# sourcedennis/wasm-pathtracer

Hardware: AMD Instinct MI355X
Metric: Mray/s (primary+shadow+bounce) at 1920x1080, 1/2/4/8 GPU; L2 vs CPU ref (higher is better)
Workload: dtype f32; 1 GPU; C3 bunny scene (scene id 2), 1920x1080, 64 spp per GPU share (64 spp frame), depth 8, NormalNEE; rays=25682600955, parallelism=single GPU

## Files before the change

include/wpt.h:

```cpp
#ifndef WPT_H
#define WPT_H

#include <stddef.h>
#include <stdint.h>

#ifdef __cplusplus
extern "C" {
#endif

#define WPT_OK 0
#define WPT_ERR_NOT_INIT (-1)
#define WPT_ERR_ALREADY_INIT (-2)
#define WPT_ERR_INVALID_SCENE (-3)
#define WPT_ERR_INVALID_ARG (-4)
#define WPT_ERR_UNSUPPORTED (-5)
#define WPT_ERR_DEVICE (-6)
#define WPT_ERR_NO_MESH (-7)

#define WPT_NO_NEE 0
#define WPT_NORMAL_NEE 1
#define WPT_PNEE 2


int wpt_init(uint32_t width, uint32_t height, uint32_t scene_id, float cam_x, float cam_y, float cam_z,
// ... 45 lines not shown

int wpt_copy_partition(void* device_dst);

typedef int (*wpt_exchange_fn)(void* user);
int wpt_set_exchange(wpt_exchange_fn fn, void* user, void* local_dev, void* gathered_dev, uint64_t slot);
int64_t wpt_exchange_slot(void);

int wpt_comm_unique_id(void* out128);
int wpt_set_comm(uint32_t rank, uint32_t nranks, uint32_t tile, const void* unique_id128);
int wpt_gather_frame(uint32_t root);
int wpt_comm_destroy(void);
#define WPT_XFER_GATHER 0
#define WPT_XFER_ALLGATHER 1
typedef int (*wpt_transport_fn)(void* user, int32_t op, uint32_t root);
int wpt_set_transport(wpt_transport_fn fn, void* user, void* send_dev, void* recv_dev, uint64_t slot);
int64_t wpt_gather_plan(uint32_t rank, uint32_t nranks, uint32_t root, uint64_t slot, uint64_t* out);
float wpt_seq_sum(const float* v, uint64_t n);
float wpt_seq_sum_chunks(const float* v, uint64_t n);
int wpt_seq_sum_device(const float* v, uint64_t n, float* out);

int wpt_stats(uint64_t* out, size_t n);
int wpt_kernel_times(double* out, size_t n);
int wpt_set_counting(int on);
int wpt_set_profiling(int on);
int wpt_set_lanes(int32_t n);
#define WPT_OPT_DEFAULTS 0
#define WPT_OPT_TRAVERSAL 1
#define WPT_OPT_TRAVERSAL_SH 2
#define WPT_OPT_FUSED 3
#define WPT_OPT_FUSED_BELOW 4
#define WPT_OPT_SMALL_LANES 5
#define WPT_OPT_PIXEL_TILE 6
#define WPT_OPT_GRID_PCT 7
#define WPT_OPT_REFILL 8
#define WPT_OPT_REFILL_SH 9
#define WPT_OPT_TREELET 10
#define WPT_OPT_BVH_BUILD 11
#define WPT_OPT_LANES 12
#define WPT_OPT_FINISH_BELOW 13
#define WPT_OPT_TRACE_GRID_PCT 14
#define WPT_OPT_FINISH_EVERY 20
#define WPT_OPT_PROBE 22
#define WPT_OPT_STOCK 23
#define WPT_OPT_STOCK_LANES 24
#define WPT_OPT_FILL 25
#define WPT_OPT_ASYNC_PRIO 26
#define WPT_OPT_ASYNC_GRID_PCT 27
#define WPT_OPT_STOCK_AHEAD 30
#define WPT_OPT_STOCK_EVERY 32
#define WPT_OPT_STOCK_EXTRA 33
#define WPT_OPT_ASYNC_ONESHOT 31
#define WPT_OPT_STOCK_PREFILL 35
#define WPT_OPT_ASYNC_FUSED_BELOW 36
#define WPT_OPT_LOG 34
#define WPT_OPT_SCENE_TRAVERSAL 28
#define WPT_OPT_SCENE_TRI_ONLY 29
int wpt_set_option(int32_t option, int64_t value);
int64_t wpt_probe_read(uint32_t* meta, uint32_t* rec, uint64_t* rec_entries, double* ticks_per_us);
int wpt_get_option(int32_t option, int64_t* value);
int wpt_scene_build_info(double* out);
int wpt_clear_stats(void);
int wpt_sync(void);
int wpt_bvh_depth(void);

int wpt_trace_rays(size_t n, const float* rays, float* t_out, int32_t* id_out);
int wpt_shadow_rays(size_t n, const float* pq, const int32_t* light, uint8_t* occluded);

int wpt_shutdown(void);

void* wpt_debug_scene_new(int32_t scene_id, const float* mesh_vertices, size_t num_vertices);
int wpt_debug_scene_info(void* h, uint64_t* out);
int wpt_debug_scene_nodes4(void* h, uint32_t* out);
int wpt_debug_scene_nodes(void* h, uint32_t* out);
int wpt_debug_scene_shapes(void* h, float* out);
int wpt_debug_scene_lights(void* h, uint32_t* out);
void wpt_debug_scene_free(void* h);
void* wpt_debug_scene_new_gpu(int32_t scene_id, const float* mesh_vertices, size_t num_vertices);
int wpt_debug_scene_build_info(void* h, double* out);

#ifdef __cplusplus
}
#endif

#endif
```

wasm-pathtracer_amd/_lib.py:

```python
import ctypes
import os

HERE = os.path.dirname(os.path.abspath(__file__))
_VARIANT = os.environ.get("WPT_LIB_VARIANT", "")
LIB_PATH = os.path.join(HERE, f"libwpt_{_VARIANT}.so" if _VARIANT else "libwpt.so")

_lib = None

c_u32, c_i32, c_f32, c_sz = ctypes.c_uint32, ctypes.c_int32, ctypes.c_float, ctypes.c_size_t
c_p = ctypes.c_void_p

_SIGS = {
    "wpt_init": (ctypes.c_int, [c_u32, c_u32, c_u32, c_f32, c_f32, c_f32, c_f32, c_f32]),
    "wpt_results": (ctypes.POINTER(ctypes.c_uint8), [c_u32]),
    "wpt_update_scene": (ctypes.c_int, [c_u32]),
    "wpt_update_settings": (ctypes.c_int, [c_u32, c_u32, c_u32, c_u32, c_u32]),
    "wpt_update_viewport": (ctypes.c_int, [c_u32, c_u32]),
    "wpt_update_camera": (ctypes.c_int, [c_f32, c_f32, c_f32, c_f32, c_f32]),
    "wpt_allocate_mesh": (ctypes.c_int, [c_u32, c_u32]),
    "wpt_mesh_vertices": (ctypes.POINTER(ctypes.c_float), [c_u32]),
    "wpt_notify_mesh_loaded": (ctypes.c_int, [c_u32]),
    "wpt_load_obj": (ctypes.c_int, [c_u32, ctypes.c_char_p, c_sz, c_p, c_p]),
    "wpt_parse_obj": (ctypes.c_int, [ctypes.c_char_p, c_sz, c_p, c_p, ctypes.c_uint64, c_p]),
    "wpt_allocate_texture": (ctypes.POINTER(ctypes.c_uint8), [c_u32, c_u32, c_u32]),
    "wpt_notify_texture_loaded": (ctypes.c_int, [c_u32]),
    "wpt_compute": (ctypes.c_int, [c_sz]),
    "wpt_last_error": (ctypes.c_char_p, []),
    "wpt_set_device": (ctypes.c_int, [ctypes.c_int]),
    "wpt_set_render_options": (ctypes.c_int, [c_i32, c_u32, ctypes.c_uint64]),
    "wpt_set_partition": (ctypes.c_int, [c_u32, c_u32, c_u32]),
    "wpt_partition_pixels": (ctypes.c_int64, [c_p]),
    "wpt_tile_partition": (ctypes.c_int64, [c_u32, c_u32, c_u32, c_u32, c_u32, c_p]),
    "wpt_photon_tree": (ctypes.c_int64, [c_p, c_p, c_p]),
    "wpt_read_radiance": (ctypes.c_int, [c_p, c_p]),
    "wpt_copy_partition": (ctypes.c_int, [c_p]),
    "wpt_set_exchange": (ctypes.c_int, [c_p, c_p, c_p, c_p, ctypes.c_uint64]),
    "wpt_exchange_slot": (ctypes.c_int64, []),
    "wpt_stats": (ctypes.c_int, [c_p, c_sz]),
    "wpt_kernel_times": (ctypes.c_int, [c_p, c_sz]),
    "wpt_set_counting": (ctypes.c_int, [ctypes.c_int]),
    "wpt_set_profiling": (ctypes.c_int, [ctypes.c_int]),
    "wpt_set_lanes": (ctypes.c_int, [ctypes.c_int32]),
    "wpt_set_option": (ctypes.c_int, [ctypes.c_int32, ctypes.c_int64]),
    "wpt_get_option": (ctypes.c_int, [ctypes.c_int32, c_p]),
    "wpt_probe_read": (ctypes.c_int64, [c_p, c_p, c_p, c_p]),
    "wpt_scene_build_info": (ctypes.c_int, [c_p]),
    "wpt_clear_stats": (ctypes.c_int, []),
    "wpt_sync": (ctypes.c_int, []),
    "wpt_bvh_depth": (ctypes.c_int, []),
    "wpt_trace_rays": (ctypes.c_int, [c_sz, c_p, c_p, c_p]),
    "wpt_shadow_rays": (ctypes.c_int, [c_sz, c_p, c_p, c_p]),
    "wpt_shutdown": (ctypes.c_int, []),
    "wpt_debug_scene_new": (c_p, [c_i32, c_p, c_sz]),
    "wpt_debug_scene_info": (ctypes.c_int, [c_p, c_p]),
    "wpt_debug_scene_nodes": (ctypes.c_int, [c_p, c_p]),
    "wpt_debug_scene_shapes": (ctypes.c_int, [c_p, c_p]),
    "wpt_debug_scene_nodes4": (ctypes.c_int, [c_p, c_p]),
    "wpt_comm_unique_id": (ctypes.c_int, [c_p]),
    "wpt_set_comm": (ctypes.c_int, [c_u32, c_u32, c_u32, c_p]),
    "wpt_gather_frame": (ctypes.c_int, [c_u32]),
    "wpt_comm_destroy": (ctypes.c_int, []),
    "wpt_set_transport": (ctypes.c_int, [c_p, c_p, c_p, c_p, ctypes.c_uint64]),
    "wpt_gather_plan": (ctypes.c_int64, [c_u32, c_u32, c_u32, ctypes.c_uint64, c_p]),
    "wpt_seq_sum": (ctypes.c_float, [c_p, ctypes.c_uint64]),
    "wpt_seq_sum_chunks": (ctypes.c_float, [c_p, ctypes.c_uint64]),
    "wpt_seq_sum_device": (ctypes.c_int, [c_p, ctypes.c_uint64, c_p]),
    "wpt_debug_scene_lights": (ctypes.c_int, [c_p, c_p]),
    "wpt_debug_scene_free": (None, [c_p]),
    "wpt_debug_scene_new_gpu": (c_p, [c_i32, c_p, c_sz]),
    "wpt_debug_scene_build_info": (ctypes.c_int, [c_p, c_p]),
}

EXPORTED = tuple(_SIGS)


def header_symbols():
    import re
    hdr = os.path.join(os.path.dirname(HERE), "include", "wpt.h")
    txt = open(hdr).read()
    return sorted(set(re.findall(r"\b(wpt_[a-z_0-9]+)\s*\(", txt)))


def lib():
    global _lib
    if _lib is not None:
        return _lib
    try:
        import torch
    except ImportError:
        pass
    if not os.path.exists(LIB_PATH):
        raise RuntimeError(f"{LIB_PATH} is missing: run __graft_entry__.build() (make -C wasm-pathtracer_amd/csrc)")
    L = ctypes.CDLL(LIB_PATH)
    for name, (res, args) in _SIGS.items():
        f = getattr(L, name)
        f.restype = res
        f.argtypes = args
    _lib = L
    return L
```

wasm-pathtracer_amd/csrc/wpt_api.cpp:

```cpp
#include <cstring>
#include <map>
#include <memory>
#include <string>
#include <vector>

#include "../../include/wpt.h"
#include "wpt_bvh_gpu.h"
#include "wpt_comm.h"
#include "wpt_obj.h"
#include "wpt_partition.h"
#include "wpt_render.h"
#include "wpt_seqsum.h"

using namespace wpt;

namespace {

struct Session {
  std::map<uint32_t, std::vector<float>> preload;
  std::map<uint32_t, std::vector<float>> meshes;
  std::map<uint32_t, std::vector<uint8_t>> textures;
  uint32_t scene_id = 0;
  HostScene scene;
  Renderer renderer;
// ... 441 lines not shown
  if (slot < s.renderer.exchange_slot() || slot < s.renderer.part_pixels())
    return fail(WPT_ERR_INVALID_ARG, "transport slot smaller than the largest partition");
  s.drop_comm();
  s.xfer = fn;
  s.xfer_user = user;
  s.xfer_send = (float4*)send_dev;
  s.xfer_recv = (float4*)recv_dev;
  s.xfer_slot = slot;
  s.renderer.set_exchange(xfer_exchange, &s, send_dev, recv_dev, slot);
  return WPT_OK;
}

int64_t wpt_gather_plan(uint32_t rank, uint32_t nranks, uint32_t root, uint64_t slot, uint64_t* out) {
  if (nranks == 0 || rank >= nranks || root >= nranks) return fail(WPT_ERR_INVALID_ARG, "bad rank");
  std::vector<XferOp> ops;
  gather_plan(rank, nranks, root, slot, ops);
  if (out)
    for (size_t i = 0; i < ops.size(); i++) {
      out[4 * i] = ops[i].peer;
      out[4 * i + 1] = ops[i].offset;
      out[4 * i + 2] = ops[i].count;
      out[4 * i + 3] = ops[i].recv ? 1u : 0u;
    }
  return (int64_t)ops.size();
}

float wpt_seq_sum(const float* v, uint64_t n) { return wpt::seq_sum_f32(v, (size_t)n); }

float wpt_seq_sum_chunks(const float* v, uint64_t n) {
  std::vector<wpt::ChunkEff> eff(2 * ((size_t)n / wpt::kSumChunk + 1));
  wpt::seq_sum_effects(v, (size_t)n, eff.data());
  return wpt::seq_sum_walk(v, (size_t)n, eff.data());
}

int wpt_seq_sum_device(const float* v, uint64_t n, float* out) {
  if (!g_session) return fail(WPT_ERR_NOT_INIT, "init not called");
  if (!out || (n && !v)) return fail(WPT_ERR_INVALID_ARG, "null pointer");
  std::string err;
  if (!g_session->renderer.seq_sum_device(v, n, *out, err)) return fail(WPT_ERR_DEVICE, err);
  return WPT_OK;
}

int wpt_comm_destroy(void) {
  if (!g_session) return fail(WPT_ERR_NOT_INIT, "init not called");
  g_session->drop_comm();
  return WPT_OK;
}

int wpt_stats(uint64_t* out, size_t n) {
  if (!g_session) return fail(WPT_ERR_NOT_INIT, "init not called");
  std::string err;
  if (!g_session->renderer.flush_counts(err)) return fail(WPT_ERR_DEVICE, err);
  const Stats& st = g_session->renderer.stats();
  uint64_t v[40] = {st.paths,          st.rays,           st.shadow_rays,    st.node_visits,  st.prim_tests,
                    st.bounces,        st.ext_visits,     st.ext_tests,      st.ext_node_bytes, st.sh_visits,
                    st.sh_tests,       st.sh_node_bytes,  st.fallback_ext,   st.fallback_sh,  st.ext_lane_iters,
                    st.ext_live_iters, st.sh_lane_iters,  st.sh_live_iters,  st.photon_rays,  st.photons,
                    st.sum_chunks,     st.sum_resummed,   st.sum_fetched,    st.stock_consumed, st.fill_paths,
                    st.trace_bytes,    st.finish_paths,   st.finish_max_bounces, st.max_ray_visits,
                    st.ex_body_lanes,  st.ex_bodies,      st.lf_body_lanes,  st.lf_bodies,    st.stock_traced,
                    st.stock_deficit,  st.stock_waits,    st.plan_us,        st.stock_us,
                    st.stock_rays,     st.stock_rays_used};
  for (size_t i = 0; i < n && i < 40; i++) out[i] = v[i];
  return WPT_OK;
}

int wpt_kernel_times(double* out, size_t n) {
  if (!g_session) return fail(WPT_ERR_NOT_INIT, "init not called");
  const KernelTimes& t = g_session->renderer.times();
  double v[28] = {t.generate, (double)t.n_generate, t.extend, (double)t.n_extend, t.shade, (double)t.n_shade,
                  t.shadow, (double)t.n_shadow, t.accumulate, (double)t.n_accumulate, t.trace, (double)t.n_trace};
  for (int k = 0; k < 6; k++) {
    v[12 + 2 * k] = t.busy[k];
    v[13 + 2 * k] = (double)t.logical[k];
  }
  v[24] = t.retrace;
  v[25] = (double)t.n_retrace;
  v[26] = t.busy[6];
  v[27] = (double)t.logical[6];
  for (size_t i = 0; i < n && i < 28; i++) out[i] = v[i];
  return WPT_OK;
}

int wpt_set_counting(int on) {
  if (!g_session) return fail(WPT_ERR_NOT_INIT, "init not called");
  g_session->renderer.set_counting(on != 0);
  return WPT_OK;
}

int wpt_scene_build_info(double* out) {
  if (!g_session) return fail(WPT_ERR_NOT_INIT, "init not called");
  if (!out) return fail(WPT_ERR_INVALID_ARG, "null argument");
  out[0] = g_session->scene.bvh_ms;
  out[1] = g_session->scene.bvh_on_gpu ? 1.0 : 0.0;
  return WPT_OK;
}

int wpt_set_lanes(int32_t n) {
  if (!g_session) return fail(WPT_ERR_NOT_INIT, "init not called");
  if (!g_session->renderer.set_lanes(n)) return fail(WPT_ERR_INVALID_ARG, "lanes out of range");
  return WPT_OK;
}

int wpt_set_option(int32_t option, int64_t value) {
  if (option == WPT_OPT_BVH_BUILD) {
    if (value < 0 || value > 2) return fail(WPT_ERR_INVALID_ARG, "option value out of range");
    g_bvh_build = (int)value;
    return WPT_OK;
  }
  std::string err;
  if (!g_session) {
    if (option == WPT_OPT_DEFAULTS) {
      g_default_opts.clear();
      g_bvh_build = 0;
      return WPT_OK;
    }
// ... 46 lines not shown
  std::memcpy(meta, s.probe_meta.data(), s.probe_meta.size() * sizeof(uint32_t));
  std::memcpy(rec, s.probe_rec.data(), s.probe_rec.size() * sizeof(uint4));
  *rec_entries = s.probe_rec.size();
  if (ticks_per_us) *ticks_per_us = s.probe_tpu;
  const int64_t n = (int64_t)(s.probe_meta.size() / 5);
  s.probe_meta.clear();
  s.probe_rec.clear();
  s.probe_taken = false;
  return n;
}

int wpt_get_option(int32_t option, int64_t* value) {
  if (!value) return fail(WPT_ERR_INVALID_ARG, "null argument");
  if (option == WPT_OPT_BVH_BUILD) { *value = g_bvh_build; return WPT_OK; }
  if (!g_session) {
    auto it = g_default_opts.find(option);
    if (it != g_default_opts.end()) { *value = it->second; return WPT_OK; }
    Renderer probe;
    if (!probe.get_option(option, *value)) return fail(WPT_ERR_INVALID_ARG, "unknown option");
    return WPT_OK;
  }
  if (!g_session->renderer.get_option(option, *value)) return fail(WPT_ERR_INVALID_ARG, "unknown option");
  return WPT_OK;
}

int wpt_set_profiling(int on) {
  if (!g_session) return fail(WPT_ERR_NOT_INIT, "init not called");
  g_session->renderer.set_profiling(on != 0);
  return WPT_OK;
}

int wpt_clear_stats(void) {
  if (!g_session) return fail(WPT_ERR_NOT_INIT, "init not called");
  g_session->renderer.clear_stats();
  return WPT_OK;
}

int wpt_sync(void) {
  if (!g_session) return fail(WPT_ERR_NOT_INIT, "init not called");
  std::string err;
  if (!g_session->renderer.sync(err)) return fail(WPT_ERR_DEVICE, err);
  return WPT_OK;
}

int wpt_bvh_depth(void) {
  if (!g_session) return fail(WPT_ERR_NOT_INIT, "init not called");
  return (int)g_session->renderer.bvh_depth();
}

int wpt_trace_rays(size_t n, const float* rays, float* t_out, int32_t* id_out) {
  if (!g_session) return fail(WPT_ERR_NOT_INIT, "init not called");
  std::string err;
  if (!g_session->renderer.trace_rays(n, rays, t_out, id_out, err)) return fail(WPT_ERR_DEVICE, err);
  return WPT_OK;
}

int wpt_shadow_rays(size_t n, const float* pq, const int32_t* light, uint8_t* occluded) {
  if (!g_session) return fail(WPT_ERR_NOT_INIT, "init not called");
  std::string err;
  if (!g_session->renderer.shadow_rays(n, pq, light, occluded, err)) return fail(WPT_ERR_INVALID_ARG, err);
  return WPT_OK;
}

int wpt_shutdown(void) {
  if (!g_session) return fail(WPT_ERR_NOT_INIT, "init not called");
  delete g_session;
  g_session = nullptr;
  return WPT_OK;
}

void* wpt_debug_scene_new(int32_t scene_id, const float* mesh_vertices, size_t num_vertices) {
  std::vector<float> mesh;
  if (mesh_vertices && num_vertices) mesh.assign(mesh_vertices, mesh_vertices + ((num_vertices / 3) * 9));
  HostScene* sc = new HostScene();
  std::string err;
  if (!build_scene(scene_id, mesh, *sc, err)) {
    delete sc;
    fail(WPT_ERR_INVALID_SCENE, err);
    return nullptr;
  }
  return sc;
}

void* wpt_debug_scene_new_gpu(int32_t scene_id, const float* mesh_vertices, size_t num_vertices) {
  static BvhGpu* gpu = nullptr;
  const hipError_t he = hipSetDevice(g_device);
  if (he != hipSuccess) {
    fail(WPT_ERR_DEVICE, std::string("hipSetDevice failed: ") + hipGetErrorString(he));
    return nullptr;
  }
  if (!gpu) gpu = new BvhGpu();
  gpu->min_shapes = 0;
  std::vector<float> mesh;
  if (mesh_vertices && num_vertices) mesh.assign(mesh_vertices, mesh_vertices + ((num_vertices / 3) * 9));
  HostScene* sc = new HostScene();
  std::string err;
  if (!build_scene(scene_id, mesh, *sc, err, gpu)) {
    delete sc;
    fail(err.rfind("HIP error", 0) == 0 || err.rfind("GPU BVH", 0) == 0 ? WPT_ERR_DEVICE : WPT_ERR_INVALID_SCENE,
         err);
    return nullptr;
  }
  return sc;
}

int wpt_debug_scene_build_info(void* h, double* out) {
// ... 30 lines not shown
  const HostScene* sc = (const HostScene*)h;
  if (!sc) return fail(WPT_ERR_INVALID_ARG, "null scene");
  for (size_t i = 0; i < sc->nodes4.size(); i++) {
    const Node4& n = sc->nodes4[i];
    uint32_t* o = out + 37 * i;
    memset(o, 0, 37 * sizeof(uint32_t));
    for (int k = 0; k < 4; k++) {
      const uint32_t c = n.child[k];
      if (c == kChildEmpty) continue;
      o[0]++;
      uint32_t* e = o + 1 + 9 * k;
      if (!(c & 0x80000000u)) {
        e[0] = 1;
        e[1] = c;
      } else {
        e[0] = 2;
        if ((c & 0xC0000000u) == 0xC0000000u) {
          e[1] = sc->leaf_table[2 * (c & 0x3FFFFFFFu)];
          e[2] = sc->leaf_table[2 * (c & 0x3FFFFFFFu) + 1];
        } else {
          e[1] = c & 0xFFFFFFu;
          e[2] = (c >> 24) & 0x3Fu;
        }
      }
      const float b[6] = {n.xmin[k], n.ymin[k], n.zmin[k], n.xmax[k], n.ymax[k], n.zmax[k]};
      memcpy(e + 3, b, sizeof b);
    }
  }
  return WPT_OK;
}

int wpt_debug_scene_shapes(void* h, float* out) {
  const HostScene* sc = (const HostScene*)h;
  if (!sc) return fail(WPT_ERR_INVALID_ARG, "null scene");
  for (size_t i = 0; i < sc->shapes.size(); i++) {
    const Shape& s = sc->shapes[i];
    float* o = out + 16 * i;
    memcpy(o, s.g, sizeof s.g);
    o[12] = (float)s.kind;
    o[13] = s.emissive ? 1.0f : 0.0f;
    o[14] = 0.0f;
    o[15] = 0.0f;
  }
  return WPT_OK;
}

int wpt_debug_scene_lights(void* h, uint32_t* out) {
  const HostScene* sc = (const HostScene*)h;
  if (!sc) return fail(WPT_ERR_INVALID_ARG, "null scene");
  for (size_t i = 0; i < sc->lights.size(); i++) out[i] = sc->lights[i];
  return WPT_OK;
}

void wpt_debug_scene_free(void* h) { delete (HostScene*)h; }

}
```

wasm-pathtracer_amd/csrc/wpt_render.h:

```cpp
#pragma once
#include <hip/hip_runtime.h>
#include <stdint.h>
#include <string>
#include <algorithm>
#include <deque>
#include <vector>

#include "wpt_scene.h"
#include "wpt_seqsum.h"

namespace wpt {

constexpr int kMaxInf = 16;
constexpr int kMaxBvhDepth = 4096;
constexpr int kMaxBounces = 512;

struct DevScene {
  const float4* nodes;
  const float4* tree;
  uint32_t tree_pairs, tree_root_lf;
  const float4* prims;
  const uint32_t* kinds;
  const float4* all;
  const uint32_t* all_kinds;
  const float4* mats;
  const float4* lights;
  const float4* nodes4;
  const uint32_t* leaf_table;
  uint32_t num_inf, num_finite, num_shapes, num_lights;
  uint32_t use_bvh, tri_only;
  uint32_t refill_lanes;
  uint32_t refill_lanes_sh;
  int stack_cap;
  uint32_t* overflow;
  const uint32_t* oct_child;
  const float* oct_cum;
  const uint32_t* oct_corners;
  uint32_t oct_nodes;
  uint32_t oct_lds_words;
  float bg[3];
  float4 planes[kMaxInf];
  uint4* probe;
};

struct Stats {
  uint64_t paths = 0;
  uint64_t rays = 0;
  uint64_t shadow_rays = 0;
  uint64_t node_visits = 0;
  uint64_t prim_tests = 0;
  uint64_t bounces = 0;
  uint64_t ext_visits = 0, ext_tests = 0, ext_node_bytes = 0;
  uint64_t sh_visits = 0, sh_tests = 0, sh_node_bytes = 0;
  uint64_t fallback_ext = 0, fallback_sh = 0;
  uint64_t ex_body_lanes = 0, ex_bodies = 0, lf_body_lanes = 0, lf_bodies = 0;
  uint64_t ext_lane_iters = 0, ext_live_iters = 0, sh_lane_iters = 0, sh_live_iters = 0;
  uint64_t photon_rays = 0, photons = 0;
  uint64_t trace_bytes = 0;
  uint64_t max_ray_visits = 0;
  uint64_t sum_chunks = 0, sum_resummed = 0, sum_fetched = 0;
  uint64_t finish_paths = 0, finish_max_bounces = 0;
  uint64_t stock_traced = 0, stock_consumed = 0, fill_paths = 0;
  uint64_t stock_deficit = 0, stock_waits = 0, plan_us = 0, stock_us = 0;
  uint64_t stock_rays = 0;
  uint64_t stock_rays_used = 0;
};

constexpr int kTimedKernels = 7;
struct KernelTimes {
  double generate = 0, extend = 0, shade = 0, shadow = 0, accumulate = 0, trace = 0, retrace = 0;
  uint64_t n_extend = 0, n_shadow = 0, n_shade = 0, n_generate = 0, n_accumulate = 0, n_trace = 0, n_retrace = 0;
  double busy[kTimedKernels] = {0, 0, 0, 0, 0, 0, 0};
  uint64_t logical[kTimedKernels] = {0, 0, 0, 0, 0, 0, 0};
};

constexpr int kMaxLanes = 8;
constexpr uint64_t kMinLanePaths = 1024;
constexpr size_t kFinishWord = 2 + 2 * (size_t)kMaxBounces;
constexpr size_t kCountWords = kFinishWord + 4;
constexpr uint32_t kWorkWords = 16;
constexpr uint32_t kWorkCopies = 64;
struct PathSet {
  hipStream_t stream = nullptr;
  hipStream_t lo = nullptr;
  hipEvent_t done = nullptr;
  uint64_t cap = 0;
  uint32_t* pixel = nullptr;
  float4* col = nullptr;
  float4* ro[2] = {nullptr, nullptr};
  float4* rd[2] = {nullptr, nullptr};
  float4* thr[2] = {nullptr, nullptr};
  float* t = nullptr;
  int32_t* id = nullptr;
  float4 *so = nullptr, *sd = nullptr, *sc = nullptr;
  uint32_t* counts = nullptr;
  uint32_t* h_counts = nullptr;
  uint2* spill = nullptr;
  size_t spill_cap = 0;
};

constexpr int kAsyncLane0 = 2;
struct Batch {
  enum State { kNew, kBouncing, kCountWait, kIssued };
  uint64_t k0 = 0, n = 0;
  int half = -1;
  const uint32_t* part = nullptr;
  uint32_t npix = 0;
  const uint32_t* moff = nullptr;
  const uint32_t* mbase = nullptr;
  const uint32_t* mlist = nullptr;
  uint32_t nent = 0;
  bool stock = false;
  bool async = false;
  int queue = 0;
  int lane0 = 0, nl = 1;
  uint64_t off[kMaxLanes + 1] = {};
  bool fused = false, pnee = false;
  int maxb = 0, b = 0;
  bool finished = false;
  State state = kNew;
  hipEvent_t done[kMaxLanes] = {};
  hipEvent_t live[kMaxLanes] = {};
  uint32_t* hc = nullptr;
  uint32_t* hl = nullptr;
};

class Renderer {
 public:
  Renderer();
  ~Renderer();
  bool set_device(int dev, std::string& err);
  bool upload_scene(const HostScene& sc, std::string& err);
  bool set_viewport(uint32_t w, uint32_t h, std::string& err);
  void set_camera(const float cam[5]);
  void set_types(int left, int right, int debug) { left_type_ = left; right_type_ = right; debug_ = debug; }
  void set_adaptive(bool left, bool right) { adaptive_[0] = left; adaptive_[1] = right; }
  bool adaptive() const { return adaptive_[0] || adaptive_[1]; }
  bool fill_sampling_blue(std::string& err);
  bool sampling_rgba(uint8_t* out, std::string& err);
  void set_options(int max_depth, uint32_t seed, uint64_t batch) {
    if (seed != seed_) photons_ok_ = false;
    max_depth_ = max_depth; seed_ = seed; if (batch) batch_ = batch;
  }
  bool build_photons(std::string& err);
  bool photon_tree(std::vector<uint32_t>& child, std::vector<float>& cum, uint64_t& shot, uint64_t& stored,
                   std::string& err);
  bool set_partition(uint32_t rank, uint32_t nranks, uint32_t tile, std::string& err);
  bool reset(std::string& err);
  bool compute(uint64_t num_paths, std::string& err);
  bool sync(std::string& err);
  bool results_rgba(uint8_t* host_out, std::string& err);
  bool read_radiance(float* acc3, uint32_t* cnt, std::string& err);
  bool copy_partition(float* dev_dst, std::string& err);
  using ExchangeFn = int (*)(void*);
  void set_exchange(ExchangeFn fn, void* user, void* local_dev, void* gathered_dev, uint64_t slot) {
    xfn_ = fn; xuser_ = user; xlocal_ = (float4*)local_dev; xall_ = (float4*)gathered_dev; xslot_ = slot;
  }
  uint64_t exchange_slot() const { return maxpart_; }
  uint32_t rank() const { return rank_; }
  uint32_t nranks() const { return nranks_; }
  uint32_t tile() const { return tile_; }
  bool unpack_ranks(const float4* gathered, uint64_t slot, std::string& err);
  bool trace_rays(size_t n, const float* rays, float* t_out, int32_t* id_out, std::string& err);
  bool shadow_rays(size_t n, const float* pq, const int32_t* light, uint8_t* occ, std::string& err);
  bool probe_read(std::vector<uint32_t>& meta, std::vector<uint4>& rec, double& ticks_per_us, std::string& err);
  void set_counting(bool on) { counting_ = on; }
  void set_profiling(bool on) { profiling_ = on; }
  bool set_lanes(int n) {
    if (n < 1 || n > lanes_made_) return false;
    nlanes_ = n;
    return true;
  }
  int lanes() const { return nlanes_; }
  static bool scene_option(int opt) { return opt == 1 || opt == 2 || opt == 10; }
  bool set_option(int opt, int64_t v, std::string& err);
  bool get_option(int opt, int64_t& v) const;
  int wants_bvh4() const {
    return (traversal_ == 1 || traversal_sh_ == 1) ? 1 : (traversal_ == 3 || traversal_sh_ == 3) ? 2 : 0;
  }
  bool seq_sum_device(const float* v, uint64_t n, float& out, std::string& err);
  const Stats& stats() const { return stats_; }
  const KernelTimes& times() const { return times_; }
  void clear_stats() {
    std::string e;
    (void)flush_counts(e);
    stats_ = Stats();
    times_ = KernelTimes();
  }
  bool flush_counts(std::string& err);
  uint32_t width() const { return w_; }
  uint32_t height() const { return h_; }
  uint32_t part_pixels() const { return (uint32_t)part_pix_.size(); }
  const std::vector<uint32_t>& part_list() const { return part_pix_; }
  hipStream_t stream() const { return stream_; }
  uint32_t bvh_depth() const { return depth_; }

 private:
  bool ensure_paths(uint64_t n, std::string& err);
  bool ensure_lane(int i, uint64_t n, std::string& err);
  void free_lane_paths(PathSet& L);
  void bind_lane(int i);
  bool run_batch(uint64_t k0, uint64_t n, int half, std::string& err, const uint32_t* part_pix = nullptr,
                 uint32_t part_n = 0, const Batch* map = nullptr);
  bool batch_begin(Batch& B, std::string& err);
  bool batch_advance(Batch& B, bool block, std::string& err);
  bool batch_tail(Batch& B, std::string& err);
  void batch_counts(const Batch& B, const uint32_t* hc);
  bool pump(bool block, std::string& err);
  bool wait_issued(Batch* B, std::string& err);
  bool drain_async(std::string& err);
  bool host_wait(hipEvent_t e, std::string& err);
  bool host_wait_stream(hipStream_t s, std::string& err);
  hipEvent_t ev_sync_ = nullptr;
  uint64_t batch_cap() const;
  int main_lanes() const;
  bool compute_half(int h, uint64_t n, std::string& err);
// ... 38 lines not shown
  ChunkEff* h_eff_ = nullptr;
  uint32_t* d_need_ = nullptr;
  uint32_t* d_list_ = nullptr;
  float* d_fb_ = nullptr;
  uint32_t* h_list_ = nullptr;
  float* h_fb_ = nullptr;
  uint32_t stock_slots_ = 1024;
  int stock_lanes_ = 2;
  uint32_t stock_ahead_ = 40;
  uint32_t stock_extra_ = 8;
  uint32_t stock_every_ = 3;
  float4* d_stock_ = nullptr;
  uint32_t* d_stock_id_ = nullptr;
  size_t stock_bytes_[2] = {0, 0};
  uint32_t* d_front_ = nullptr;
  uint32_t* d_def_ = nullptr;
  uint32_t* d_bmax_ = nullptr;
  unsigned long long* d_rays_ = nullptr;
  uint64_t stock_cap_ = 0;
  uint32_t stock_used_slots_ = 0;
  static constexpr int kMaxRefill = 8;
  static constexpr uint64_t kStockBytes = 48ull << 30;
  static constexpr int kRefillChunks = 8;
  static constexpr uint64_t kRefillChunk = 1ull << 25;
  struct Refill {
    uint32_t id = 0;
    bool live = false;
    bool counted = false;
    uint32_t* off = nullptr;
    uint32_t* base = nullptr;
    std::deque<Batch> chunks;
  };
  Refill refills_[kMaxRefill];
  hipEvent_t refill_ev_[kMaxRefill][2 * kRefillChunks] = {};
  uint32_t* h_refill_cnt_ = nullptr;
  uint32_t refill_id_ = 0;
  int refill_lane_ = 0;
  uint32_t round_need_[2] = {0, 0};
  bool stock_redo_[2] = {false, false};
  int log_ = 0;
  bool stock_active(int h) const { return stock_slots_ != 0 && nranks_ == 1 && adaptive_[h]; }
  bool stock_alloc(std::string& err);
  void stock_drop();
  bool stock_round(int h, uint64_t left, std::string& err);
  bool stock_consume(int h, uint64_t a, uint64_t b, std::string& err);
  bool stock_flush(std::string& err);
  bool refill_count(Refill& f, bool block, std::string& err);
  uint32_t refill_scale(int h, uint32_t ahead, uint64_t after) const;
  Refill* refill_slot(std::string& err);
  void refill_plan(Refill& F, int h, uint32_t ahead, uint32_t q);
  bool refill_issue(Refill& F, int h, uint64_t wt, std::string& err);
  bool stock_prefill(int h, uint64_t budget, std::string& err);
  bool stock_prefill_ = true;
  bool pend_stock_ = false;
  std::deque<Batch*> aq_[2];
  bool fill_on_ = false;
  int async_prio_ = 0;
  int async_grid_pct_ = 100;
  uint64_t async_fused_below_ = 1ull << 26;
  bool async_launch_ = false;
  uint32_t* d_seam_pix_[2] = {nullptr, nullptr};
  uint32_t* d_rest_pix_[2] = {nullptr, nullptr};
  uint32_t seam_npix_[2] = {0, 0}, rest_npix_[2] = {0, 0};
  static constexpr int kMaxFill = 8;
  Batch fill_[kMaxFill];
  int nfill_ = 0;
  hipEvent_t fill_ev_[kMaxFill][2] = {};
  uint32_t* h_fill_cnt_ = nullptr;
  bool async_pending() const { return !aq_[0].empty() || !aq_[1].empty(); }
  int fill_lane() const { return kAsyncLane0 + stock_lanes_; }
  bool issue_fill(int h, uint64_t k0, uint64_t n, std::string& err);
  bool drain_fill(std::string& err);
  bool compute_halves(uint64_t nl, uint64_t nr, std::string& err);
  uint32_t async_grid(uint32_t g, int base_pct, uint32_t rays_per_path = 1) const {
    if (!async_launch_) return g;
    if (async_oneshot_) return std::max<uint32_t>(1u, (uint32_t)((async_paths_ * rays_per_path + 255) / 256));
    return async_grid_pct_ > 0 ? std::max<uint32_t>(1u, (uint32_t)((uint64_t)g * async_grid_pct_ / base_pct)) : g;
  }
  bool async_oneshot_ = false;
  uint64_t async_paths_ = 0;
  void bind_batch_lane(const Batch& B, int l);
  bool time_launches_ = false;
  uint8_t* d_samp_ = nullptr;
  ExchangeFn xfn_ = nullptr;
  void* xuser_ = nullptr;
  float4* xlocal_ = nullptr;
  float4* xall_ = nullptr;
  uint64_t xslot_ = 0;
  uint64_t maxpart_ = 0;
  uint32_t* d_xidx_ = nullptr;
  bool photons_ok_ = false;
  uint64_t photons_shot_ = 0, photons_stored_ = 0;
  std::vector<uint32_t> oct_child_;
  std::vector<float> oct_cum_;
  uint32_t* d_oct_child_ = nullptr;
  float* d_oct_cum_ = nullptr;
  uint32_t* d_oct_corners_ = nullptr;

  int device_ = -1;
  int ncu_ = 256;
  uint2* d_spill_ = nullptr;
  size_t spill_cap_ = 0;
  static constexpr int kTravVariants = 8;
  uint32_t grid_ext_[2 * kTravVariants] = {};
  uint32_t grid_sh_[2 * kTravVariants] = {};
  uint32_t grid_tr_[4] = {};
  uint32_t grid_shade_ = 512;
  uint32_t shade_occ_[16] = {};
  size_t shade_occ_smem_[16] = {};
  bool fused_ = false;
  uint64_t fused_below_ = 1ull << 24;
  int small_lanes_ = 2;
  int traversal_ = 3, traversal_sh_ = 3;
  int trav_ext_ = 0, trav_sh_ = 0;
  bool treelet_ = true;
  uint32_t pixel_tile_ = 8;
  int grid_pct_ = 50;
#ifndef WPT_TRACE_GRID_PCT
#define WPT_TRACE_GRID_PCT 75
#endif
  int trace_grid_pct_ = WPT_TRACE_GRID_PCT;
  uint32_t refill_ = 12, refill_sh_ = 16;
  uint64_t finish_below_ = 1u << 18;
  int finish_every_ = 4;
  int batch_lanes_ = 1;
  uint32_t probe_cap_ = 0, probe_waves_ = 0, probe_used_ = 0;
  uint4* d_probe_ = nullptr;
  std::vector<uint32_t> probe_meta_;
  int cur_bounce_ = 0;
  uint4* probe_slot(int kernel, uint32_t grid);
  uint32_t* d_fallback_ = nullptr;
  hipStream_t stream_ = nullptr;
  hipStream_t ks_ = nullptr;
  PathSet lanes_[kMaxLanes];
  int lanes_made_ = 0;
  bool stats_pending_ = false;
  int pend_nl_ = 0, pend_b_ = 0;
  int nlanes_ = 4;
  int bound_ = 0;
  hipEvent_t ev_main_ = nullptr;
  hipEvent_t ev_ref_ = nullptr;
  std::vector<void*> scene_bufs_;
  DevScene ds_{};
  uint32_t depth_ = 0;
  bool scene_ok_ = false;

  uint32_t w_ = 0, h_ = 0;
  float cam_[5] = {0, 0, 0, 0, 0};
  int left_type_ = 1, right_type_ = 1, debug_ = 0;
  int max_depth_ = 0;
  uint32_t seed_ = 0xBABABEBEu;
  uint64_t batch_ = 1ull << 27;

  uint32_t rank_ = 0, nranks_ = 1, tile_ = 16;
  std::vector<uint32_t> part_pix_;
  uint32_t* d_part_pix_ = nullptr;
  uint32_t* d_half_pix_[2] = {nullptr, nullptr};
  uint32_t* d_frame_pix_ = nullptr;
  uint32_t half_npix_[2] = {0, 0};
  uint64_t next_path_ = 0;

  float4* d_acc_ = nullptr;
  uint32_t* d_cnt_ = nullptr;
  uint8_t* d_rgba_ = nullptr;

  uint64_t cap_ = 0;
  uint32_t* p_pixel_ = nullptr;
  float4* p_col_ = nullptr;
  float4* p_ro_[2] = {nullptr, nullptr};
  float4* p_rd_[2] = {nullptr, nullptr};
  float4* p_thr_[2] = {nullptr, nullptr};
  float* p_t_ = nullptr;
  int32_t* p_id_ = nullptr;
  float4* s_o_ = nullptr;
  float4* s_d_ = nullptr;
  float4* s_c_ = nullptr;
  uint32_t* d_counts_ = nullptr;
  unsigned long long* d_work_ = nullptr;
  uint32_t* h_counts_ = nullptr;
  uint32_t* h_word_ = nullptr;
  uint32_t* ext_count(int b) const { return b == 0 ? d_counts_ : d_counts_ + 2 + 2 * (b - 1); }
  uint32_t* sh_count(int b) const { return d_counts_ + 3 + 2 * b; }
  unsigned long long* append_ctr(int b) const { return reinterpret_cast<unsigned long long*>(d_counts_ + 2 + 2 * b); }

  bool counting_ = false;
  bool profiling_ = false;
  Stats stats_;
  KernelTimes times_;
  struct PendingTiming {
    hipEvent_t a, b;
    int slot;
  };
  bool next_event(hipEvent_t* e, std::string& err);
  bool resolve_timings(std::string& err);
  std::vector<hipEvent_t> ev_pool_;
  size_t ev_used_ = 0;
  std::vector<PendingTiming> pending_;
};

}
```

wasm-pathtracer_amd/csrc/wpt_render.hip:

```cpp
#include "wpt_render.h"
#include "wpt_partition.h"
#include "wpt_photon.h"
#include "wpt_quartic.h"
#include "wpt_seqsum.h"

#include <algorithm>
#include <chrono>
#include <cstdlib>
#include <cmath>
#include <cstdio>
#include <cstring>
#include <deque>
#include <mutex>
#include <unordered_map>
#include <thread>
#include <type_traits>

#define HIP_OK(expr)                                                     \
  do {                                                                   \
    hipError_t e_ = (expr);                                              \
    if (e_ != hipSuccess) {                                              \
      err = std::string(#expr " failed: ") + hipGetErrorString(e_);      \
      return false;                                                      \
    }                                                                    \
// ... 616 lines not shown
__device__ __forceinline__ bool begin_shadow(const DevScene& S, const Hot& H, Lane& L, V3 o, V3 d, float dir_len,
                                             int32_t light, float& early, bool& occluded, uint32_t& visits,
                                             uint32_t& tests, uint32_t& nbytes) {
  L.o = o;
  L.d = d;
  L.inv = inv_dir(d);
  L.best_id = -1;
  occluded = false;
  if (!S.use_bvh) {
    L.best = 0.0f;
    linear_closest<TRI_ONLY>(S, o, d, L.best, L.best_id, tests);
    return false;
  }
  early = dir_len;
  float tl;
  bool lhit;
  uint32_t k = 0;
  if (H.lrec)
    while (k < S.num_lights && H.lid[k] != light) k++;
  if (H.lrec && k < S.num_lights) {
    lhit = tri_hit_r(H.lq(k, 0), H.lq(k, 1), H.lq(k, 2), H.lq(k, 3), o, d, tl);
  } else {
    const uint32_t lk = (uint32_t)light - S.num_inf;
    const float4* lp = S.prims + 4 * (size_t)lk;
    lhit = TRI_ONLY ? tri_hit(lp, o, d, tl) : prim_hit(S.kinds[lk], lp, o, d, tl);
  }
  if (lhit) early = fminf(tl, dir_len);
  float pt = __int_as_float(0x7f800000);
  int32_t pid = -1;
  if (planes_closest(S, o, d, pt, pid) && pt < early) {
    occluded = true;
    return false;
  }
  if (pid >= 0 && pt < dir_len) { L.best = pt; L.best_id = pid; }
  else { L.best = dir_len; L.best_id = -1; }
  if (!S.num_finite) return false;
  return FAST ? enter_root4<COUNT>(H, L, visits, nbytes) : enter_root<COUNT>(S, H, L, visits, nbytes);
}

__device__ __forceinline__ bool shadow_verdict(const Lane& L, float dir_len, int32_t light, bool occluded) {
  return occluded || (L.best_id >= 0 && L.best < dir_len && L.best_id != light);
}

struct GenParams {
  uint32_t W, H, npix;
  float w_inv, h_inv, ar;
  float cam[3];
  float cx, sx, cy, sy;
  uint32_t seed;
  uint32_t half;
  uint32_t left_type, right_type;
};

__global__ void __launch_bounds__(kBlock) k_generate(GenParams P, const uint32_t* __restrict__ part_pix, uint64_t k0,
                                                     uint32_t n, uint32_t* __restrict__ pix_out,
                                                     float4* __restrict__ thr,
                                                     float4* __restrict__ col, float4* __restrict__ ro,
                                                     float4* __restrict__ rd, uint32_t* __restrict__ count0,
                                                     const uint32_t* __restrict__ rnd_off,
                                                     const uint32_t* __restrict__ rnd_base,
                                                     const uint32_t* __restrict__ rnd_list, uint32_t stock_slots) {
  const uint32_t i = blockIdx.x * kBlock + threadIdx.x;
  if (i == 0) *count0 = n;
  if (i >= n) return;
  const uint64_t k = k0 + i;
  uint32_t pl, sample;
  if (rnd_off) {
    uint32_t lo = 0, hi = P.npix;
    while (lo + 1u < hi) {
      const uint32_t mid = (lo + hi) >> 1;
      if ((uint64_t)rnd_off[mid] <= k) lo = mid;
      else hi = mid;
    }
    pl = lo;
    sample = rnd_base[lo] + (uint32_t)(k - rnd_off[lo]);
  } else {
    pl = (uint32_t)(k % P.npix);
    sample = (uint32_t)(k / P.npix);
  }
  const uint32_t pixel = rnd_list ? rnd_list[pl] : part_pix ? part_pix[pl] : pl;
  const uint32_t x = pixel % P.W, y = pixel / P.W;
  uint32_t s = path_seed(P.seed, pixel, sample);
  const float fx = (((float)x + xs_next(s)) * P.w_inv - 0.5f) * P.ar;
  const float fy = 0.5f - ((float)y + xs_next(s)) * P.h_inv;
  V3 v = normalize(mk(fx, fy, 0.8f));
  v = mk(v.x, P.cx * v.y - P.sx * v.z, P.sx * v.y + P.cx * v.z);
  v = mk(P.cy * v.x + P.sy * v.z, v.y, (-P.sy) * v.x + P.cy * v.z);
  const uint32_t type = x < P.half ? P.left_type : P.right_type;
  pix_out[i] = stock_slots ? pixel * stock_slots + (sample & (stock_slots - 1u)) : rnd_off ? pl : pixel;
  thr[i] = make_float4(1.0f, 1.0f, 1.0f, __uint_as_float(type << kTypeShift));
  col[i] = make_float4(0.0f, 0.0f, 0.0f, 0.0f);
  ro[i] = make_float4(P.cam[0], P.cam[1], P.cam[2], __uint_as_float(s));
  rd[i] = make_float4(v.x, v.y, v.z, __uint_as_float(i));
}

template <bool TRI_ONLY>
__device__ __forceinline__ const float4* shape_rec(const DevScene& S, int32_t id, uint32_t& kind) {
  if (!S.use_bvh) { kind = S.all_kinds[id]; return S.all + 4 * (size_t)id; }
  if ((uint32_t)id < S.num_inf) { kind = kPlane; return nullptr; }
  kind = TRI_ONLY ? (uint32_t)kTri : S.kinds[id - S.num_inf];
  return S.prims + 4 * (size_t)(id - S.num_inf);
}

template <class CP, class FP>
struct OctViewT {
  CP child;
  FP cum;
};
using OctG = OctViewT<const uint32_t*, const float*>;
using OctL1 = OctViewT<const lds_u32*, const float*>;
using OctL2 = OctViewT<const lds_u32*, const lds_f32*>;

template <class OV>
__device__ uint32_t oct_find(const DevScene& S, const OV& O, V3 v, int max_depth, float b[6], int& depth) {
  b[0] = b[1] = b[2] = -kPhotonTreeSize;
  b[3] = b[4] = b[5] = kPhotonTreeSize;
  uint32_t node = 0;
  depth = 0;
  while (O.child[node] != 0u && (max_depth < 0 || depth < max_depth)) {
    float nb[6];
    const uint32_t ci = octant(b, v, nb);
    for (int k = 0; k < 6; k++) b[k] = nb[k];
    node = O.child[node] + ci;
    depth++;
  }
  return node;
}

template <class OV>
__device__ __forceinline__ float oct_bin_prob(const DevScene& S, const OV& O, uint32_t node, uint32_t i) {
  const auto c = O.cum + (size_t)node * S.num_lights;
  return i + 1u == S.num_lights ? 1.0f - c[i] : c[i + 1] - c[i];
}

template <class OV>
__device__ __forceinline__ float oct_node_prob(const DevScene& S, const OV& O, V3 v, int depth, uint32_t res) {
  float b[6];
  int d;
  return oct_bin_prob(S, O, oct_find(S, O, v, depth, b, d), res);
}

__device__ __forceinline__ void oct_axis(float v, float lo, float hi, float& w, float& wadj, float& off) {
  const float size = hi - lo;
  if (v > 0.5f * (lo + hi)) {
    const float left = (hi - (v - size * 0.5f)) / size;
    w = left;
// ... 226 lines not shown
    } else {
      const float4* L = S.lights + 5 * (size_t)li;
      L0 = L[0];
      L1 = L[1];
      L2 = L[2];
      L3 = L[3];
      L4 = L[4];
    }
    const float q1 = xs_next(s);
    const float q2 = xs_next(s);
    const float q1s = sqrtf(q1);
    const V3 pt = add(add(scale(ld3(L0), 1.0f - q1s), scale(ld3(L1), q1s * (1.0f - q2))), scale(ld3(L2), q2 * q1s));
    V3 ln = ld3(L3);
    if (xs_next(s) > 0.5f) ln = neg(ln);
    const V3 inten = ld3(L4);
    V3 tl = sub(pt, hp);
    const float d2 = dot(tl, tl);
    const float dl = sqrtf(d2);
    tl = divs(tl, dl);
    const float ci = dot(tl, nrm);
    const float co = dot(neg(tl), ln);
    if (ci > 0.0f && co > 0.0f) {
      if (P.debug) {
        const float4 c4 = col[path];
        const V3 c = add(ld3(c4), mulv(thr, inten));
        col[path] = make_float4(c.x, c.y, c.z, c4.w);
      } else {
        const float solid = (L0.w * co) / d2;
        const V3 contrib = scale(scale(scale(mulv(thr, inten), solid), ci), 1.0f / light_chance);
        const V3 sorig = add(hp, scale(tl, kEpsilon));
        R.so = make_float4(sorig.x, sorig.y, sorig.z, dl);
        R.sd = make_float4(tl.x, tl.y, tl.z, L1.w);
        R.sc = make_float4(contrib.x, contrib.y, contrib.z, d4.w);
        R.shadow = true;
      }
    }
  }
  const bool capped = P.max_depth > 0 && (int)depth >= P.max_depth;
  if (!capped && depth < (uint32_t)kMaxBounces) {
    const float keep = fmaxf(fminf(fmaxf(fmaxf(thr.x, thr.y), thr.z), 0.9f), 0.1f);
    if (xs_next(s) < keep) {
      thr = scale(thr, 1.0f / keep);
      const uint32_t nsh = (flags >> kShadowShift) + (R.shadow ? 1u : 0u);
      flags = (flags & ~((~0u) << kDepthShift)) | (depth << kDepthShift) | (nsh << kShadowShift) | kFlagBounced;
      R.ro = make_float4(no.x, no.y, no.z, __uint_as_float(s));
      R.rd = make_float4(wi.x, wi.y, wi.z, d4.w);
      R.th = make_float4(thr.x, thr.y, thr.z, __uint_as_float(flags));
      R.alive = true;
    }
  }
  if (!R.alive) end_counts((flags >> kShadowShift) + (R.shadow ? 1u : 0u));
}

template <bool TRI_ONLY, bool PNEE, int OCT, bool CR = false>
__global__ void WPT_SHADE_BOUNDS k_shade(DevScene S, ShadeParams P, RayStream in, RayStream out,
                                                       ShadowStream sh, float4* __restrict__ col,
                                                       const uint32_t* __restrict__ count, const float* __restrict__ t_in,
                                                       const int32_t* __restrict__ id_in,
                                                       unsigned long long* __restrict__ append) {
  constexpr uint32_t kWaves = kShadeBlock / 64;
  __shared__ uint32_t s_off[2][kWaves];
  __shared__ f4v s_light[5 * kShadeLights];
  const uint32_t n = *count;
  const bool lds_lights = S.num_lights <= kShadeLights;
  if (lds_lights) {
    for (uint32_t k = threadIdx.x; k < 5 * S.num_lights; k += kShadeBlock) {
      const float4 v = S.lights[k];
      s_light[k] = f4v{v.x, v.y, v.z, v.w};
    }
  }
  extern __shared__ uint32_t s_oct[];
  if (PNEE && OCT != 0) {
    const uint32_t nc = S.oct_nodes, nw = S.oct_lds_words;
    for (uint32_t k = threadIdx.x; k < nw; k += kShadeBlock)
      s_oct[k] = k < nc ? S.oct_child[k] : __float_as_uint(S.oct_cum[k - nc]);
  }
  __syncthreads();
  using OV = std::conditional_t<OCT == 2, OctL2, std::conditional_t<OCT == 1, OctL1, OctG>>;
  OV O;
  if constexpr (OCT == 2) {
    O.child = (const lds_u32*)s_oct;
    O.cum = (const lds_f32*)(s_oct + S.oct_nodes);
  } else if constexpr (OCT == 1) {
    O.child = (const lds_u32*)s_oct;
    O.cum = S.oct_cum;
  } else {
    O.child = S.oct_child;
    O.cum = S.oct_cum;
  }
  const uint32_t lane = threadIdx.x & 63u, wid = threadIdx.x >> 6;
  const uint64_t below = (1ull << lane) - 1ull;
  for (uint32_t i0 = blockIdx.x * kShadeBlock; i0 < n; i0 += gridDim.x * kShadeBlock) {
    const uint32_t i = i0 + threadIdx.x;
    ShadeOut R;
    R.alive = R.shadow = false;
    if (i < n)
      shade_path<TRI_ONLY, PNEE, OV, CR>(S, O, P, col, t_in[i], id_in[i], in.o[i], in.d[i], in.thr[i], R,
                                     lds_lights ? (const lds_f4v*)s_light : nullptr);
    const uint64_t am = __ballot(R.alive), sm = __ballot(R.shadow);
    if (lane == 0) {
      s_off[0][wid] = (uint32_t)__popcll(am);
      s_off[1][wid] = (uint32_t)__popcll(sm);
    }
    __syncthreads();
    if (wid == 0) {
      const uint32_t a = lane < kWaves ? s_off[0][lane] : 0u, b = lane < kWaves ? s_off[1][lane] : 0u;
      uint32_t ia = a, ib = b;
#pragma unroll
      for (uint32_t k = 1; k < kWaves; k <<= 1) {
        const uint32_t ya = __shfl_up(ia, k, 64), yb = __shfl_up(ib, k, 64);
        if (lane >= k) { ia += ya; ib += yb; }
      }
      unsigned long long base = 0ull;
      if (lane == kWaves - 1) base = atomicAdd(append, (unsigned long long)ia | ((unsigned long long)ib << 32));
      const uint32_t ba = (uint32_t)__shfl((int)(uint32_t)base, (int)(kWaves - 1), 64);
      const uint32_t bb = (uint32_t)__shfl((int)(uint32_t)(base >> 32), (int)(kWaves - 1), 64);
      if (lane < kWaves) {
        s_off[0][lane] = ba + ia - a;
        s_off[1][lane] = bb + ib - b;
      }
    }
    __syncthreads();
    if (R.alive) {
      const uint32_t p = s_off[0][wid] + (uint32_t)__popcll(am & below);
      st_stream(out.o + p, R.ro);
      st_stream(out.d + p, R.rd);
      st_stream(out.thr + p, R.th);
    }
    if (R.shadow) {
      const uint32_t p = s_off[1][wid] + (uint32_t)__popcll(sm & below);
      st_stream(sh.o + p, R.so);
      st_stream(sh.d + p, R.sd);
      st_stream(sh.c + p, R.sc);
    }
    __syncthreads();
  }
}

struct WaveFeed {
  uint32_t n, v, wave, nwaves;
  __device__ WaveFeed(uint32_t n_) : n(n_), v(0) {
    wave = (blockIdx.x * kTBlock + threadIdx.x) >> 6;
    nwaves = (gridDim.x * kTBlock) >> 6;
  }
  static constexpr uint32_t K = kFeedChunk;
  __device__ uint32_t pos(uint32_t k) const { return ((k / K) * nwaves + wave) * K + (k % K); }
  __device__ bool more() const { return pos(v) < n; }
  __device__ uint32_t taken() const { return taken_below(n); }
  __device__ uint32_t taken_below(uint32_t m) const {
    const uint32_t C = m / K, rem = m % K;
    const uint32_t full = C > wave ? (C - wave - 1u) / nwaves + 1u : 0u;
    const uint32_t part = (rem != 0u && C % nwaves == wave) ? rem : 0u;
    return min(v, full * K + part);
  }
  __device__ uint32_t take(uint64_t take_m) {
    const uint32_t rank = (uint32_t)__popcll(take_m & ((1ull << (threadIdx.x & 63)) - 1ull));
    const uint32_t p = pos(v + rank);
    v += (uint32_t)__popcll(take_m);
    return p;
  }
};

__global__ void __launch_bounds__(kBlock) k_photon_gen(DevScene S, uint32_t seed, uint32_t k0, uint32_t n,
                                                       float4* __restrict__ ro, float4* __restrict__ rd,
                                                       float4* __restrict__ rec) {
  const uint32_t i = blockIdx.x * kBlock + threadIdx.x;
  if (i >= n) return;
  uint32_t s = photon_seed(seed, k0 + i);
  const uint32_t li = xs_next_in_range(s, S.num_lights);
  const float4* L = S.lights + 5 * (size_t)li;
  const float4 L0 = L[0], L1 = L[1], L2 = L[2], L3 = L[3], L4 = L[4];
  const float q1 = xs_next(s);
  const float q2 = xs_next(s);
  const float q1s = sqrtf(q1);
  const V3 pt = add(add(scale(ld3(L0), 1.0f - q1s), scale(ld3(L1), q1s * (1.0f - q2))), scale(ld3(L2), q2 * q1s));
  V3 ln = ld3(L3);
  if (xs_next(s) > 0.5f) ln = neg(ln);
  float x, y, z;
  do {
    x = xs_next(s) * 2.0f - 1.0f;
// ... 357 lines not shown
  __shared__ float s_lrec[16 * kLdsLights];
  __shared__ int32_t s_lid[kLdsLights];
  __shared__ f4v s_tree[4 * kTreePairs + 1];
  const Hot H = load_hot(S, (lds_f32h*)s_lrec, (lds_i32*)s_lid, (lds_f4v*)s_tree, (const float4*)s_tree);
  const uint32_t n = *count;
  const uint32_t G = gridDim.x * kTBlock;
  const Stack stk{(lds_u32*)(s_code + threadIdx.x), (lds_f32*)(s_h + threadIdx.x),
                  spill + blockIdx.x * kTBlock + threadIdx.x, G, S.stack_cap, S.overflow};
  const OctG O{S.oct_child, S.oct_cum};
  const float inf = __int_as_float(0x7f800000);
  uint32_t nrays = 0, nshadow = 0, npaths = 0, longest = 0, dummy = 0;
  for (uint32_t i = blockIdx.x * kTBlock + threadIdx.x; i < n; i += G) {
    float4 o4 = in.o[i], d4 = in.d[i], th4 = in.thr[i];
    const uint32_t r0 = nrays;
    npaths++;
    for (;;) {
      Lane L;
      bool occ = false;
      nrays++;
      if (begin_extend<TRI_ONLY, false, false>(S, H, L, ld3(o4), ld3(d4), dummy, dummy, dummy))
        while (step<false, TRI_ONLY, false, false>(S, H, L, stk, -1, 0.0f, occ, dummy, dummy, dummy)) {
        }
      ShadeOut R;
      R.alive = R.shadow = false;
      shade_path<TRI_ONLY, PNEE, OctG, CR>(S, O, P, col, L.best_id >= 0 ? L.best : inf, L.best_id, o4, d4, th4, R);
      if (R.shadow) {
        nshadow++;
        const float dir_len = R.so.w, early0 = 0.0f;
        const int32_t light = (int32_t)__float_as_uint(R.sd.w);
        float early = early0;
        bool occluded = false;
        Lane Ls;
        if (begin_shadow<TRI_ONLY, false, false>(S, H, Ls, ld3(R.so), ld3(R.sd), dir_len, light, early, occluded,
                                                 dummy, dummy, dummy))
          while (step<true, TRI_ONLY, false, false>(S, H, Ls, stk, light, early, occluded, dummy, dummy, dummy)) {
          }
        if (!shadow_verdict(Ls, dir_len, light, occluded)) add_contribution(col, R.sc);
      }
      if (!R.alive) break;
      o4 = R.ro;
      d4 = R.rd;
      th4 = R.th;
    }
    longest = max(longest, nrays - r0);
  }
  if (nrays) atomicAdd(counters, nrays);
  if (nshadow) atomicAdd(counters + 1, nshadow);
  if (npaths) {
    atomicAdd(counters + 2, npaths);
    atomicMax(counters + 3, longest);
  }
}

__global__ void __launch_bounds__(kBlock) k_accumulate(const uint32_t* __restrict__ part_pix, uint64_t k0, uint32_t n,
                                                       uint32_t npix, const float4* __restrict__ col,
                                                       float4* __restrict__ acc, uint32_t* __restrict__ cnt) {
  const uint32_t i = blockIdx.x * kBlock + threadIdx.x;
  const uint32_t lim = n < npix ? n : npix;
  if (i >= lim) return;
  const uint32_t pl = (uint32_t)((k0 + i) % npix);
  const uint32_t pixel = part_pix ? part_pix[pl] : pl;
  float4 a = acc[pixel];
  uint32_t c = cnt[pixel];
  for (uint32_t j = i; j < n; j += npix) {
    const float4 v = col[j];
    a.x += v.x;
    a.y += v.y;
    a.z += v.z;
    c += 1;
  }
  acc[pixel] = a;
  cnt[pixel] = c;
}

__global__ void k_rgba(const float4* __restrict__ acc, const uint32_t* __restrict__ cnt, uint32_t npix,
                       uint8_t* __restrict__ out) {
  const uint32_t i = blockIdx.x * kBlock + threadIdx.x;
  if (i >= npix) return;
  const float4 a = acc[i];
  const uint32_t c = cnt[i];
  uchar4 r = make_uchar4(0, 0, 0, 255);
  if (c > 0) {
    const float fc = (float)c;
    r.x = (uint8_t)(fmaxf(fminf(a.x / fc, 1.0f), 0.0f) * 255.0f);
    r.y = (uint8_t)(fmaxf(fminf(a.y / fc, 1.0f), 0.0f) * 255.0f);
    r.z = (uint8_t)(fmaxf(fminf(a.z / fc, 1.0f), 0.0f) * 255.0f);
  }
  reinterpret_cast<uchar4*>(out)[i] = r;
}

__global__ void k_pack_partition(const uint32_t* __restrict__ part_pix, uint32_t n, const float4* __restrict__ acc,
                                 const uint32_t* __restrict__ cnt, float4* __restrict__ out) {
  const uint32_t i = blockIdx.x * kBlock + threadIdx.x;
  if (i >= n) return;
  const uint32_t p = part_pix ? part_pix[i] : i;
  float4 a = acc[p];
  a.w = __uint_as_float(cnt[p]);
  out[i] = a;
}

inline uint32_t blocks_for(uint64_t n) { return (uint32_t)((n + kBlock - 1) / kBlock); }

}

namespace {
struct RingBlock {
// ... 113 lines not shown
    if (d_rest_pix_[k]) (void)hipFree(d_rest_pix_[k]);
  }
  if (h_fill_cnt_) (void)hipHostFree(h_fill_cnt_);
  for (auto& fe : fill_ev_)
    for (hipEvent_t e : fe)
      if (e) (void)hipEventDestroy(e);
  if (ev_main_) (void)hipEventDestroy(ev_main_);
  if (ev_sync_) (void)hipEventDestroy(ev_sync_);
  if (ev_ref_) (void)hipEventDestroy(ev_ref_);
  if (h_word_) (void)hipHostFree(h_word_);
  for (auto& e : ev_pool_)
    if (e) (void)hipEventDestroy(e);
  if (stream_) (void)hipStreamDestroy(stream_);
}

bool Renderer::set_device(int dev, std::string& err) {
  if (device_ == dev && stream_) return true;
  if (stream_) {
    err = "device already selected";
    return false;
  }
  HIP_OK(hipSetDevice(dev));
  device_ = dev;
  HIP_OK(hipStreamCreateWithFlags(&stream_, hipStreamNonBlocking));
  HIP_OK(hipDeviceGetAttribute(&ncu_, hipDeviceAttributeMultiprocessorCount, dev));
  HIP_OK(hipEventCreateWithFlags(&ev_main_, hipEventDisableTiming));
  HIP_OK(hipEventCreateWithFlags(&ev_sync_, hipEventDisableTiming));
  HIP_OK(hipEventCreate(&ev_ref_));
  HIP_OK(hipHostMalloc(&h_word_, sizeof(uint32_t) * 4));
  lanes_made_ = kMaxLanes;
  for (int i = 0; i < kMaxLanes; i++) {
    PathSet& L = lanes_[i];
    if (i == 0) L.stream = stream_;
    else HIP_OK(hipStreamCreateWithFlags(&L.stream, hipStreamNonBlocking));
    HIP_OK(hipEventCreateWithFlags(&L.done, hipEventDisableTiming));
    HIP_OK(hipMalloc(&L.counts, sizeof(uint32_t) * kCountWords));
    HIP_OK(hipHostMalloc(&L.h_counts, sizeof(uint32_t) * kCountWords));
  }
  bind_lane(0);
  HIP_OK(hipMalloc(&d_work_, sizeof(unsigned long long) * kWorkWords * kWorkCopies));
  HIP_OK(hipMalloc(&d_fallback_, sizeof(uint32_t) * 4));
  HIP_OK(hipMemset(d_fallback_, 0, sizeof(uint32_t) * 4));
  HIP_OK(hipMemset(d_work_, 0, sizeof(unsigned long long) * kWorkWords * kWorkCopies));
  return true;
}

void Renderer::free_scene() {
  for (void* p : scene_bufs_) (void)hipFree(p);
  scene_bufs_.clear();
  scene_ok_ = false;
}

void Renderer::free_lane_paths(PathSet& L) {
  void* bufs[] = {L.pixel, L.col, L.ro[0], L.rd[0], L.thr[0], L.ro[1], L.rd[1], L.thr[1], L.t, L.id, L.so, L.sd, L.sc};
  for (void* p : bufs)
    if (p) (void)hipFree(p);
  L.pixel = nullptr;
  L.col = nullptr;
  for (int k = 0; k < 2; k++) L.ro[k] = L.rd[k] = L.thr[k] = nullptr;
  L.t = nullptr;
  L.id = nullptr;
  L.so = L.sd = L.sc = nullptr;
  L.cap = 0;
}

void Renderer::free_paths() {
  for (PathSet& L : lanes_) free_lane_paths(L);
  bind_lane(bound_);
}

void Renderer::bind_lane(int i) {
  const PathSet& L = lanes_[i];
  bound_ = i;
  async_launch_ = false;
  ks_ = L.stream;
  cap_ = L.cap;
  p_pixel_ = L.pixel;
  p_col_ = L.col;
  for (int k = 0; k < 2; k++) {
    p_ro_[k] = L.ro[k];
    p_rd_[k] = L.rd[k];
    p_thr_[k] = L.thr[k];
  }
  p_t_ = L.t; p_id_ = L.id;
  s_o_ = L.so; s_d_ = L.sd; s_c_ = L.sc;
  d_counts_ = L.counts; h_counts_ = L.h_counts;
  d_spill_ = L.spill; spill_cap_ = L.spill_cap;
}

bool Renderer::upload_scene(const HostScene& sc, std::string& err) {
  if (!stream_) { err = "no device"; return false; }
  if (!drain_async(err)) return false;
  stock_drop();
  HIP_OK(hipStreamSynchronize(stream_));
  free_photons();
  free_scene();
  if (sc.num_inf > (uint32_t)kMaxInf && sc.use_bvh) { err = "too many infinite shapes"; return false; }
  if (sc.use_bvh && sc.depth >= (uint32_t)kMaxBvhDepth) { err = "BVH deeper than supported"; return false; }
  const size_t ns = sc.shapes.size();
  const size_t nf = ns - sc.num_inf;
  auto rec = [](const Shape& s, float4* out) {
    memset(out, 0, 4 * sizeof(float4));
    const float* g = s.g;
    if (s.kind == kTri) {
      V3 v0 = mk(g[0], g[1], g[2]), v1 = mk(g[3], g[4], g[5]), v2 = mk(g[6], g[7], g[8]);
      V3 n = cross(sub(v1, v0), sub(v2, v0));
      V3 nn = normalize(n);
      float od = dot(n, v0);
      out[0] = make_float4(v0.x, v0.y, v0.z, n.x);
      out[1] = make_float4(v1.x, v1.y, v1.z, n.y);
      out[2] = make_float4(v2.x, v2.y, v2.z, n.z);
      out[3] = make_float4(nn.x, nn.y, nn.z, od);
    } else if (s.kind == kPlane) {
      V3 loc = mk(g[0], g[1], g[2]), n = mk(g[3], g[4], g[5]);
      out[0] = make_float4(n.x, n.y, n.z, dot(n, loc));
      out[1] = make_float4(loc.x, loc.y, loc.z, 0.0f);
    } else if (s.kind == kSphere) {
      out[0] = make_float4(g[0], g[1], g[2], g[3]);
    } else if (s.kind == kTorus) {
      out[0] = make_float4(g[0], g[1], g[2], g[3]);
      out[1] = make_float4(g[4], 0.0f, 0.0f, 0.0f);
    } else {
      out[0] = make_float4(g[0], g[1], g[2], g[3]);
      out[1] = make_float4(g[4], g[5], 0.0f, 0.0f);
    }
  };
  std::vector<float4> prims(4 * std::max<size_t>(nf, 1)), all(4 * std::max<size_t>(ns, 1));
  std::vector<uint32_t> kinds(std::max<size_t>(nf, 1)), all_kinds(std::max<size_t>(ns, 1));
  std::vector<float4> mats(std::max<size_t>(ns, 1));
  for (size_t i = 0; i < ns; i++) {
    const Shape& s = sc.shapes[i];
    rec(s, &all[4 * i]);
    all_kinds[i] = s.kind;
    if (i >= sc.num_inf) {
      rec(s, &prims[4 * (i - sc.num_inf)]);
      kinds[i - sc.num_inf] = s.kind;
    }
// ... 62 lines not shown
          const Node2& n = tree_nodes[order[t] + c];
          auto it = tix.find(n.left_first);
          if (n.count == 0 && it != tix.end()) tree[4 * t + 2 * c + 1].z = u2f(kTreeFlag | it->second);
        }
      }
      if (!order.empty() && order[0] == tree_nodes[root].left_first) root_lf = kTreeFlag;
      else tree.clear();
    }
    ds.tree_pairs = (uint32_t)(tree.size() / 4);
    ds.tree_root_lf = root_lf;
    if (tree.empty()) tree.push_back(make_float4(0.f, 0.f, 0.f, 0.f));
    if (!up(tree.data(), tree.size() * sizeof(float4), &p)) return false;
    ds.tree = (const float4*)p;
  }
  if (!up(prims.data(), prims.size() * sizeof(float4), &p)) return false;
  ds.prims = (const float4*)p;
  if (!up(kinds.data(), kinds.size() * sizeof(uint32_t), &p)) return false;
  ds.kinds = (const uint32_t*)p;
  if (!up(all.data(), all.size() * sizeof(float4), &p)) return false;
  ds.all = (const float4*)p;
  if (!up(all_kinds.data(), all_kinds.size() * sizeof(uint32_t), &p)) return false;
  ds.all_kinds = (const uint32_t*)p;
  if (!up(mats.data(), mats.size() * sizeof(float4), &p)) return false;
  ds.mats = (const float4*)p;
  if (!up(lights.data(), lights.size() * sizeof(float4), &p)) return false;
  ds.lights = (const float4*)p;
  {
    const size_t n4 = std::max<size_t>(sc.nodes4.size(), 1);
    std::vector<Node4> n4v(n4);
    if (!sc.nodes4.empty()) memcpy(n4v.data(), sc.nodes4.data(), sizeof(Node4) * sc.nodes4.size());
    if (!up(n4v.data(), sizeof(Node4) * n4, &p)) return false;
    ds.nodes4 = (const float4*)p;
    std::vector<uint32_t> lt(std::max<size_t>(sc.leaf_table.size(), 2), 0u);
    std::copy(sc.leaf_table.begin(), sc.leaf_table.end(), lt.begin());
    if (!up(lt.data(), sizeof(uint32_t) * lt.size(), &p)) return false;
    ds.leaf_table = (const uint32_t*)p;
    auto mode = [&](int want) {
      const bool b4 = want == 1 || (want == 3 && !sc.tri_only && sc.use_bvh);
      return (b4 && !sc.nodes4.empty()) ? 1 : 0;
    };
    trav_ext_ = mode(traversal_);
    trav_sh_ = mode(traversal_sh_);
  }
  ds.num_inf = sc.num_inf;
  ds.num_finite = (uint32_t)nf;
  ds.num_shapes = (uint32_t)ns;
  ds.num_lights = (uint32_t)sc.lights.size();
  ds.use_bvh = sc.use_bvh ? 1u : 0u;
  ds.tri_only = sc.tri_only ? 1u : 0u;
  ds.refill_lanes = refill_;
  ds.refill_lanes_sh = refill_sh_;
  for (int k = 0; k < 3; k++) ds.bg[k] = sc.background[k];
  for (uint32_t i = 0; i < sc.num_inf && i < (uint32_t)kMaxInf; i++) ds.planes[i] = all[4 * i];
  ds_ = ds;
  depth_ = sc.depth;
  ds_.stack_cap = (int)std::max<uint32_t>(sc.depth + 2, 3 * sc.depth4 + 4);
  ds_.overflow = d_fallback_ + 2;
  if (!size_grids(err)) return false;
  scene_ok_ = true;
  return true;
}

bool Renderer::set_option(int opt, int64_t v, std::string& err) {
  auto range = [&](int64_t lo, int64_t hi) {
    if (v < lo || v > hi) {
      err = "option value out of range";
      return false;
    }
    return true;
  };
  switch (opt) {
    case 1:
    case 2:
      if (!range(0, 3) || v == 2) { err = "traversal: 0 (bvh2), 1 (bvh4) or 3 (auto)"; return false; }
      (opt == 1 ? traversal_ : traversal_sh_) = (int)v;
      return true;
    case 3: if (!range(0, 1)) return false; fused_ = v != 0; return true;
    case 4: if (!range(0, (int64_t)1 << 40)) return false; fused_below_ = (uint64_t)v; return true;
    case 5: if (!range(1, kMaxLanes)) return false; small_lanes_ = (int)v; return true;
    case 6: if (!range(0, 4096)) return false; pixel_tile_ = (uint32_t)v; return true;
    case 7:
      if (!range(1, 100)) return false;
      grid_pct_ = (int)v;
      return !stream_ || size_grids(err);
    case 8: if (!range(1, 64)) return false; refill_ = (uint32_t)v; ds_.refill_lanes = refill_; return true;
    case 9: if (!range(1, 64)) return false; refill_sh_ = (uint32_t)v; ds_.refill_lanes_sh = refill_sh_; return true;
    case 10: if (!range(0, 1)) return false; treelet_ = v != 0; return true;
    case 12:
      if (!set_lanes((int)v)) { err = "lanes out of range"; return false; }
      return true;
    case 13: if (!range(0, (int64_t)1 << 32)) return false; finish_below_ = (uint64_t)v; return true;
    case 14:
      if (!range(1, 100)) return false;
      trace_grid_pct_ = (int)v;
      return !stream_ || size_grids(err);
    case 20: if (!range(1, 64)) return false; finish_every_ = (int)v; return true;
    case 23:
      if (v != 0 && (v < 64 || v > 4096 || (v & (v - 1)) != 0)) { err = "stock: 0 or a power of two 64..4096"; return false; }
      if (!drain_async(err)) return false;
      stock_drop();
      stock_slots_ = (uint32_t)v;
      return true;
    case 25: if (!range(0, 1)) return false; fill_on_ = v != 0; return true;
    case 30: if (!range(0, 64)) return false; stock_ahead_ = (uint32_t)v; return true;
    case 32: if (!range(1, 1024)) return false; stock_every_ = (uint32_t)v; return true;
    case 33: if (!range(0, 64)) return false; stock_extra_ = (uint32_t)v; return true;
    case 31: if (!range(0, 1)) return false; async_oneshot_ = v != 0; return true;
    case 34: if (!range(0, 1)) return false; log_ = (int)v; return true;
    case 35: if (!range(0, 1)) return false; stock_prefill_ = v != 0; return true;
    case 36: if (!range(0, (int64_t)1 << 40)) return false; async_fused_below_ = (uint64_t)v; return true;
    case 26:
      if (!range(0, 1)) return false;
      if (!drain_async(err)) return false;
      async_prio_ = (int)v;
      return true;
    case 27: if (!range(0, 100)) return false; async_grid_pct_ = (int)v; return true;
    case 28:
    case 29: err = "read-only option"; return false;
    case 24:
      if (!range(1, kMaxLanes - kAsyncLane0 - 1)) return false;
      if (!drain_async(err)) return false;
      stock_lanes_ = (int)v;
      refill_lane_ = 0;
      return true;
    case 22:
      if (!range(0, 1 << 20)) return false;
      probe_cap_ = (uint32_t)v;
      probe_used_ = 0;
      probe_meta_.clear();
      if (d_probe_) { (void)hipFree(d_probe_); d_probe_ = nullptr; }
      return true;
    default: err = "unknown option"; return false;
  }
}

bool Renderer::get_option(int opt, int64_t& v) const {
  switch (opt) {
    case 1: v = traversal_; return true;
    case 2: v = traversal_sh_; return true;
    case 3: v = fused_ ? 1 : 0; return true;
    case 4: v = (int64_t)fused_below_; return true;
    case 5: v = small_lanes_; return true;
    case 6: v = pixel_tile_; return true;
    case 7: v = grid_pct_; return true;
    case 8: v = refill_; return true;
    case 9: v = refill_sh_; return true;
    case 10: v = treelet_ ? 1 : 0; return true;
    case 12: v = nlanes_; return true;
    case 13: v = (int64_t)finish_below_; return true;
    case 14: v = trace_grid_pct_; return true;
    case 20: v = finish_every_; return true;
    case 22: v = probe_cap_; return true;
    case 23: v = stock_slots_; return true;
    case 25: v = fill_on_ ? 1 : 0; return true;
    case 30: v = stock_ahead_; return true;
    case 32: v = stock_every_; return true;
    case 33: v = stock_extra_; return true;
    case 31: v = async_oneshot_ ? 1 : 0; return true;
    case 34: v = log_; return true;
    case 35: v = stock_prefill_ ? 1 : 0; return true;
    case 36: v = (int64_t)async_fused_below_; return true;
    case 26: v = async_prio_; return true;
    case 27: v = async_grid_pct_; return true;
    case 28: v = !scene_ok_ ? -1 : !ds_.use_bvh ? 2 : trav_ext_; return true;
    case 29: v = !scene_ok_ ? -1 : ds_.tri_only ? 1 : 0; return true;
    case 24: v = stock_lanes_; return true;
    default: return false;
  }
}

bool Renderer::set_viewport(uint32_t w, uint32_t h, std::string& err) {
  if (!stream_) { err = "no device"; return false; }
  if (w == 0 || h == 0) { err = "empty viewport"; return false; }
  if (!drain_async(err)) return false;
  stock_drop();
  HIP_OK(hipStreamSynchronize(stream_));
  w_ = w;
  h_ = h;
  free_rounds();
  if (d_acc_) (void)hipFree(d_acc_);
  if (d_cnt_) (void)hipFree(d_cnt_);
  if (d_rgba_) (void)hipFree(d_rgba_);
  if (d_samp_) (void)hipFree(d_samp_);
  d_acc_ = nullptr; d_cnt_ = nullptr; d_rgba_ = nullptr; d_samp_ = nullptr;
  HIP_OK(hipMalloc(&d_acc_, sizeof(float4) * (size_t)w * h));
  HIP_OK(hipMalloc(&d_cnt_, sizeof(uint32_t) * (size_t)w * h));
  HIP_OK(hipMalloc(&d_rgba_, 4 * (size_t)w * h));
  HIP_OK(hipMalloc(&d_samp_, 4 * (size_t)w * h));
  return set_partition(rank_, nranks_, tile_, err);
}

void Renderer::set_camera(const float cam[5]) { memcpy(cam_, cam, sizeof cam_); }

bool Renderer::set_partition(uint32_t rank, uint32_t nranks, uint32_t tile, std::string& err) {
  if (nranks == 0 || rank >= nranks || tile == 0) { err = "bad partition"; return false; }
  if (!drain_async(err)) return false;
  stock_drop();
  HIP_OK(hipStreamSynchronize(stream_));
  rank_ = rank; nranks_ = nranks; tile_ = tile;
  part_pix_.clear();
  if (d_part_pix_) { (void)hipFree(d_part_pix_); d_part_pix_ = nullptr; }
  for (uint32_t*& p : d_half_pix_)
    if (p) { (void)hipFree(p); p = nullptr; }
  for (int k = 0; k < 2; k++) {
    if (d_seam_pix_[k]) { (void)hipFree(d_seam_pix_[k]); d_seam_pix_[k] = nullptr; }
    if (d_rest_pix_[k]) { (void)hipFree(d_rest_pix_[k]); d_rest_pix_[k] = nullptr; }
    seam_npix_[k] = rest_npix_[k] = 0;
  }
  if (d_frame_pix_) { (void)hipFree(d_frame_pix_); d_frame_pix_ = nullptr; }
  half_npix_[0] = half_npix_[1] = 0;
  if (d_xidx_) { (void)hipFree(d_xidx_); d_xidx_ = nullptr; }
  maxpart_ = 0;
  if (w_ && h_ && nranks > 1) {
    tile_partition(w_, h_, rank, nranks, tile, part_pix_);
// ... 122 lines not shown
    ev_pool_.push_back(x);
  }
  *e = ev_pool_[ev_used_++];
  return true;
}

bool Renderer::resolve_timings(std::string& err) {
  std::vector<std::pair<float, float>> iv[kTimedKernels];
  for (const PendingTiming& p : pending_) {
    float ms = 0, t0 = 0, t1 = 0;
    HIP_OK(hipEventElapsedTime(&ms, p.a, p.b));
    HIP_OK(hipEventElapsedTime(&t0, ev_ref_, p.a));
    HIP_OK(hipEventElapsedTime(&t1, ev_ref_, p.b));
    double* acc[kTimedKernels] = {&times_.generate, &times_.extend,     &times_.shade,  &times_.shadow,
                                  &times_.accumulate, &times_.trace, &times_.retrace};
    uint64_t* n[kTimedKernels] = {&times_.n_generate,   &times_.n_extend, &times_.n_shade,  &times_.n_shadow,
                                  &times_.n_accumulate, &times_.n_trace,  &times_.n_retrace};
    *acc[p.slot] += ms;
    *n[p.slot] += 1;
    iv[p.slot].push_back({t0, t1});
  }
  for (int k = 0; k < kTimedKernels; k++) {
    std::sort(iv[k].begin(), iv[k].end());
    double busy = 0, lo = 0, hi = -1e30;
    for (const auto& x : iv[k]) {
      if (x.first > hi) {
        if (hi > lo) busy += hi - lo;
        lo = x.first;
        hi = x.second;
      } else {
        hi = std::max<double>(hi, x.second);
      }
    }
    if (hi > lo) busy += hi - lo;
    times_.busy[k] += busy;
  }
  pending_.clear();
  ev_used_ = 0;
  return true;
}

uint64_t Renderer::batch_cap() const {
  const int nl = main_lanes();
  uint64_t c = lanes_[0].cap;
  for (int i = 1; i < nl; i++) c = std::min(c, lanes_[i].cap);
  return c * (uint64_t)nl;
}

int Renderer::main_lanes() const {
  const bool async = (stock_slots_ || fill_on_) && nranks_ == 1 && (adaptive_[0] || adaptive_[1]);
  return async ? std::min(nlanes_, kAsyncLane0) : nlanes_;
}

static void add_counts(Stats& st, const uint32_t* hc, int b, bool stock) {
  uint64_t& r = stock ? st.stock_rays : st.rays;
  uint64_t& sr = stock ? st.stock_rays : st.shadow_rays;
  for (int i = 0; i < b; i++) {
    r += i == 0 ? hc[0] : hc[2 + 2 * (i - 1)];
    sr += hc[3 + 2 * i];
  }
  r += hc[kFinishWord];
  sr += hc[kFinishWord + 1];
  st.finish_paths += hc[kFinishWord + 2];
  st.finish_max_bounces = std::max<uint64_t>(st.finish_max_bounces, hc[kFinishWord + 3]);
}

bool Renderer::flush_counts(std::string& err) {
  if (!stats_pending_) return true;
  for (int l = 0; l < pend_nl_; l++)
    if (!host_wait(lanes_[l].done, err)) return false;
  for (int l = 0; l < pend_nl_; l++) add_counts(stats_, lanes_[l].h_counts, pend_b_, pend_stock_);
  stats_pending_ = false;
  return true;
}

void Renderer::batch_counts(const Batch& B, const uint32_t* hc) {
  for (int i = 0; i < B.nl; i++) add_counts(stats_, hc + (size_t)i * kCountWords, B.b, B.stock);
  stats_.bounces += (uint64_t)B.b;
}

bool Renderer::batch_begin(Batch& B, std::string& err) {
  time_launches_ = profiling_ && !B.async;
  const bool round = B.half >= 0 && !B.moff;
  const uint32_t* rnd_off = B.moff ? B.moff : round ? rounds_[B.half].rc : nullptr;
  const uint32_t* rnd_base = B.moff ? B.mbase : round ? rounds_[B.half].rbase : nullptr;
  const uint32_t npix = B.moff ? B.nent : B.part ? B.npix : (uint32_t)part_pix_.size();
  const uint32_t* part = B.part ? B.part : (nranks_ > 1 ? d_part_pix_ : nullptr);
  GenParams G;
  G.W = w_; G.H = h_; G.npix = npix;
  const float fw = (float)w_, fh = (float)h_;
  G.w_inv = 1.0f / fw; G.h_inv = 1.0f / fh; G.ar = fw / fh;
  G.cam[0] = cam_[0]; G.cam[1] = cam_[1]; G.cam[2] = cam_[2];
  G.cx = mcos(cam_[3]); G.sx = msin(cam_[3]);
  G.cy = mcos(cam_[4]); G.sy = msin(cam_[4]);
  G.seed = seed_;
  G.half = w_ / 2;
  G.left_type = (uint32_t)left_type_; G.right_type = (uint32_t)right_type_;
  const uint32_t slots = B.stock ? stock_used_slots_ : 0u;
  for (int i = 0; i <= B.nl; i++) B.off[i] = B.n * (uint64_t)i / (uint64_t)B.nl;
  if (time_launches_) HIP_OK(hipEventRecord(ev_ref_, stream_));
  HIP_OK(hipEventRecord(ev_main_, stream_));
  batch_lanes_ = B.nl;
  for (int i = 0; i < B.nl; i++) {
    const int l = B.lane0 + i;
    bind_batch_lane(B, l);
    if (B.off[i + 1] - B.off[i] > cap_) { bind_lane(0); err = "batch exceeds lane capacity"; return false; }
    if (l != 0) HIP_OK(hipStreamWaitEvent(ks_, ev_main_, 0));
    if (ks_ != lanes_[l].stream) HIP_OK(hipStreamWaitEvent(ks_, lanes_[l].done, 0));
    const uint32_t nn = (uint32_t)(B.off[i + 1] - B.off[i]);
    HIP_OK(hipMemsetAsync(d_counts_, 0, sizeof(uint32_t) * kCountWords, ks_));
    LAUNCH_TIMED(0, generate, n_generate,
                 k_generate<<<blocks_for(nn), kBlock, 0, ks_>>>(G, part, B.k0 + B.off[i], nn, p_pixel_, p_thr_[0],
                                                              p_col_, p_ro_[0], p_rd_[0], d_counts_, rnd_off, rnd_base,
                                                              B.mlist, slots));
  }
  B.maxb = max_depth_ > 0 ? std::min(max_depth_, kMaxBounces) : kMaxBounces;
  B.fused = (fused_ || B.n < (B.async && async_fused_below_ ? async_fused_below_ : fused_below_)) && trav_ext_ != 1 &&
            trav_sh_ != 1;
  B.pnee = left_type_ == 2 || right_type_ == 2;
  B.b = 0;
  B.finished = false;
  B.state = Batch::kBouncing;
  bind_lane(0);
  return true;
}

bool Renderer::batch_advance(Batch& B, bool block, std::string& err) {
  const ShadeParams SP{max_depth_, debug_};
  auto launch_finish = [&](const RayStream& rin, int bb, uint32_t g, bool pn) -> bool {
#define WPT_FIN(T, PN, CR) \
  k_finish<T, PN, CR><<<g, kTBlock, 0, ks_>>>(ds_, SP, rin, ext_count(bb + 1), p_col_, d_spill_, d_counts_ + kFinishWord)
#define WPT_FIN2(T, PN) \
  if (B.stock) WPT_FIN(T, PN, true); \
  else WPT_FIN(T, PN, false)
    if (ds_.tri_only) {
      if (pn) WPT_FIN2(true, true);
      else WPT_FIN2(true, false);
    } else {
      if (pn) WPT_FIN2(false, true);
      else WPT_FIN2(false, false);
    }
#undef WPT_FIN2
#undef WPT_FIN
    HIP_OK(hipGetLastError());
    return true;
  };
  while (B.state == Batch::kBouncing || B.state == Batch::kCountWait) {
    time_launches_ = profiling_ && !B.async;
    batch_lanes_ = B.nl;
    if (B.state == Batch::kCountWait) {
      const int b = B.b - 1;
      uint32_t live[kMaxLanes];
      uint64_t left = 0;
      if (B.async) {
        for (int i = 0; i < B.nl; i++) {
          if (!block) {
            const hipError_t q = hipEventQuery(B.live[i]);
            if (q == hipErrorNotReady) return true;
            HIP_OK(q);
          }
          HIP_OK(hipEventSynchronize(B.live[i]));
        }
        for (int i = 0; i < B.nl; i++) live[i] = B.hl[i];
      } else {
        if (async_pending() && !pump(false, err)) return false;
        time_launches_ = profiling_;
        batch_lanes_ = B.nl;
        for (int i = 0; i < B.nl; i++)
          if (!host_wait_stream(lanes_[B.lane0 + i].stream, err)) return false;
        time_launches_ = profiling_;
        batch_lanes_ = B.nl;
        for (int i = 0; i < B.nl; i++) live[i] = lanes_[B.lane0 + i].h_counts[0];
      }
      for (int i = 0; i < B.nl; i++) left += live[i];
      B.state = Batch::kBouncing;
      if (left == 0) break;
      if (left <= finish_below_ && b + 1 < B.maxb) {
        for (int i = 0; i < B.nl; i++) {
          bind_batch_lane(B, B.lane0 + i);
          if (B.fused && !launch_shadow(sh_count(b), nullptr, err)) { bind_lane(0); return false; }
          if (live[i] == 0) continue;
          const RayStream rin{p_ro_[(b + 1) & 1], p_rd_[(b + 1) & 1], p_thr_[(b + 1) & 1]};
          const uint32_t g =
              (uint32_t)std::min<uint64_t>((live[i] + kTBlock - 1) / kTBlock,
                                           std::min(async_grid(grid_tr_[ds_.tri_only ? 1 : 0], trace_grid_pct_),
                                                    spill_grid()));
          if (!launch_finish(rin, b, g, B.pnee)) { bind_lane(0); return false; }
        }
        B.finished = true;
        break;
      }
      continue;
    }
    if (B.b >= B.maxb) break;
    const int b = B.b;
    cur_bounce_ = b;
    for (int i = 0; i < B.nl; i++) {
      bind_batch_lane(B, B.lane0 + i);
      const uint32_t nn = (uint32_t)(B.off[i + 1] - B.off[i]);
      if (B.fused && b > 0) {
        if (!launch_trace(b, err)) { bind_lane(0); return false; }
      } else if (!launch_extend(p_ro_[b & 1], p_rd_[b & 1], ext_count(b), err)) {
        bind_lane(0);
        return false;
      }
      {
        const RayStream in{p_ro_[b & 1], p_rd_[b & 1], p_thr_[b & 1]};
        const RayStream out{p_ro_[(b + 1) & 1], p_rd_[(b + 1) & 1], p_thr_[(b + 1) & 1]};
        const ShadowStream sh{s_o_, s_d_, s_c_};
        [[maybe_unused]] const uint32_t sgrid =
            std::max<uint32_t>(1, std::min<uint32_t>((nn + kShadeBlock - 1) / kShadeBlock, grid_shade_));
#if WPT_SHADE_GRID_VAR
#define WPT_SHADE_GRID(T, PN, OC, CR)                                                                           \
  const int vi = (CR ? 8 : 0) + (T ? 4 : 0) + (PN ? 1 + OC : 0);                                                \
  const size_t smem = OC ? 4 * (size_t)ds_.oct_lds_words : 0;                                                   \
  if (shade_occ_[vi] == 0 || shade_occ_smem_[vi] != smem) {                                                     \
    int bpc = 0;                                                                                                \
    HIP_OK(hipOccupancyMaxActiveBlocksPerMultiprocessor(&bpc, k_shade<T, PN, OC, CR>, (int)kShadeBlock, smem));  \
    shade_occ_[vi] = (uint32_t)std::max(bpc, 1);                                                                \
    shade_occ_smem_[vi] = smem;                                                                                 \
  }                                                                                                             \
  const uint32_t sg = std::max<uint32_t>(1, std::min<uint32_t>((nn + kShadeBlock - 1) / kShadeBlock,            \
                                                               (uint32_t)ncu_ * shade_occ_[vi]));
#else
#define WPT_SHADE_GRID(T, PN, OC, CR) const uint32_t sg = sgrid;
#endif
#define WPT_SHADE1(T, PN, OC, CR)                                                                                   \
  do {                                                                                                              \
    WPT_SHADE_GRID(T, PN, OC, CR)                                                                                   \
    const uint32_t sgo = async_launch_ && async_oneshot_ ? std::max<uint32_t>(1, (nn + kShadeBlock - 1) / kShadeBlock) \
                                                         : sg;                                                      \
    LAUNCH_TIMED(2, shade, n_shade,                                                                                 \
                 k_shade<T, PN, OC, CR><<<sgo, kShadeBlock, OC ? 4 * ds_.oct_lds_words : 0, ks_>>>(                 \
                     ds_, SP, in, out, sh, p_col_, ext_count(b), p_t_, p_id_, append_ctr(b)));                      \
  } while (0)
#define WPT_SHADE(T, PN, OC)              \
  do {                                    \
    if (B.stock) WPT_SHADE1(T, PN, OC, true); \
    else WPT_SHADE1(T, PN, OC, false);    \
  } while (0)
        const int oc = !B.pnee || ds_.oct_lds_words == 0 ? 0 : (ds_.oct_lds_words > ds_.oct_nodes ? 2 : 1);
        if (ds_.tri_only) {
          if (!B.pnee) WPT_SHADE(true, false, 0);
          else if (oc == 2) WPT_SHADE(true, true, 2);
          else if (oc == 1) WPT_SHADE(true, true, 1);
          else WPT_SHADE(true, true, 0);
        } else {
          if (!B.pnee) WPT_SHADE(false, false, 0);
          else if (oc == 2) WPT_SHADE(false, true, 2);
          else if (oc == 1) WPT_SHADE(false, true, 1);
          else WPT_SHADE(false, true, 0);
        }
#undef WPT_SHADE
#undef WPT_SHADE1
#undef WPT_SHADE_GRID
      }
      if (!B.fused && !launch_shadow(sh_count(b), nullptr, err)) { bind_lane(0); return false; }
    }
    B.b = b + 1;
    if (max_depth_ <= 0 && (b % finish_every_) == finish_every_ - 1) {
      for (int i = 0; i < B.nl; i++) {
        bind_batch_lane(B, B.lane0 + i);
        if (B.async) {
          HIP_OK(hipMemcpyAsync(B.hl + i, ext_count(b + 1), sizeof(uint32_t), hipMemcpyDeviceToHost, ks_));
          HIP_OK(hipEventRecord(B.live[i], ks_));
        } else {
          HIP_OK(hipMemcpyAsync(h_counts_, ext_count(b + 1), sizeof(uint32_t), hipMemcpyDeviceToHost, ks_));
        }
      }
      B.state = Batch::kCountWait;
    }
  }
  bind_lane(0);
  return batch_tail(B, err);
}

bool Renderer::batch_tail(Batch& B, std::string& err) {
  time_launches_ = profiling_ && !B.async;
  batch_lanes_ = B.nl;
  cur_bounce_ = B.b;
  if (B.fused && B.b > 0 && !B.finished) {
    for (int i = 0; i < B.nl; i++) {
      bind_batch_lane(B, B.lane0 + i);
      if (!launch_shadow(sh_count(B.b - 1), nullptr, err)) { bind_lane(0); return false; }
    }
  }
  const bool round = B.half >= 0 && !B.moff;
  const uint32_t npix = B.part ? B.npix : (uint32_t)part_pix_.size();
  const uint32_t* part = B.part ? B.part : (nranks_ > 1 ? d_part_pix_ : nullptr);
  for (int i = 0; i < B.nl; i++) {
    const int l = B.lane0 + i;
    bind_batch_lane(B, l);
    const uint32_t nn = (uint32_t)(B.off[i + 1] - B.off[i]);
    if (i > 0 && !B.stock) HIP_OK(hipStreamWaitEvent(ks_, B.async ? B.done[i - 1] : lanes_[l - 1].done, 0));
    if (B.stock)
      k_stock_store<<<blocks_for(nn), kBlock, 0, ks_>>>(p_pixel_, nn, p_col_, d_stock_);
    else if (round)
      LAUNCH_TIMED(4, accumulate, n_accumulate,
                   k_accumulate_round<<<blocks_for(nn), kBlock, 0, ks_>>>(part, nn, p_pixel_, p_col_, d_acc_, d_cnt_));
    else
      LAUNCH_TIMED(4, accumulate, n_accumulate,
                   k_accumulate<<<blocks_for(std::min<uint64_t>(nn, npix)), kBlock, 0, ks_>>>(
                       part, B.k0 + B.off[i], nn, npix, p_col_, d_acc_, d_cnt_));
    HIP_OK(hipGetLastError());
    uint32_t* hc = B.async ? B.hc + (size_t)i * kCountWords : h_counts_;
    HIP_OK(hipMemcpyAsync(hc, d_counts_, sizeof(uint32_t) * kCountWords, hipMemcpyDeviceToHost, ks_));
    HIP_OK(hipEventRecord(B.async ? B.done[i] : lanes_[l].done, ks_));
  }
  bind_lane(0);
  if (!B.async) {
    for (int i = 1; i < B.nl; i++) HIP_OK(hipStreamWaitEvent(stream_, lanes_[B.lane0 + i].done, 0));
    pend_nl_ = B.nl;
    pend_b_ = B.b;
    pend_stock_ = B.stock;
    stats_pending_ = true;
  }
  B.state = Batch::kIssued;
  return true;
}

bool Renderer::host_wait(hipEvent_t e, std::string& err) {
  for (;;) {
    const hipError_t q = hipEventQuery(e);
    if (q == hipSuccess) return true;
    if (q != hipErrorNotReady) HIP_OK(q);
    if (!async_pending()) {
      HIP_OK(hipEventSynchronize(e));
      return true;
    }
    if (!pump(false, err)) return false;
    std::this_thread::sleep_for(std::chrono::microseconds(20));
  }
}

bool Renderer::host_wait_stream(hipStream_t s, std::string& err) {
  if (!async_pending()) {
    HIP_OK(hipStreamSynchronize(s));
    return true;
  }
  HIP_OK(hipEventRecord(ev_sync_, s));
  return host_wait(ev_sync_, err);
}

bool Renderer::pump(bool block, std::string& err) {
  for (auto& q : aq_) {
    while (!q.empty()) {
      Batch& B = *q.front();
      if (B.state == Batch::kNew && !batch_begin(B, err)) return false;
      if (B.state != Batch::kIssued && !batch_advance(B, block, err)) return false;
      if (B.state != Batch::kIssued) break;
      q.pop_front();
    }
  }
  bind_lane(0);
  return true;
}

bool Renderer::wait_issued(Batch* B, std::string& err) {
  std::deque<Batch*>& q0 = aq_[B->queue];
  if (B->state == Batch::kNew && std::find(q0.begin(), q0.end(), B) == q0.end()) q0.push_back(B);
  while (B->state != Batch::kIssued) {
    std::deque<Batch*>& q = aq_[B->queue];
    if (q.empty()) { err = "async batch lost"; return false; }
    Batch& H = *q.front();
    if (H.state == Batch::kNew && !batch_begin(H, err)) return false;
    if (!batch_advance(H, true, err)) return false;
    q.pop_front();
// ... 570 lines not shown
    stats_.ex_bodies += w[11];
    stats_.lf_body_lanes += w[12];
    stats_.lf_bodies += w[13];
  }
  return true;
}

bool Renderer::sync(std::string& err) {
  if (!drain_async(err)) return false;
  for (Refill& f : refills_)
    if (f.live && !refill_count(f, true, err)) return false;
  if (stream_) HIP_OK(hipStreamSynchronize(stream_));
  return flush_counts(err);
}

bool Renderer::results_rgba(uint8_t* out, std::string& err) {
  const uint32_t np = w_ * h_;
  k_rgba<<<blocks_for(np), kBlock, 0, stream_>>>(d_acc_, d_cnt_, np, d_rgba_);
  HIP_OK(hipGetLastError());
  HIP_OK(hipMemcpyAsync(out, d_rgba_, 4 * (size_t)np, hipMemcpyDeviceToHost, stream_));
  HIP_OK(hipStreamSynchronize(stream_));
  return true;
}

bool Renderer::read_radiance(float* acc3, uint32_t* cnt, std::string& err) {
  const size_t np = (size_t)w_ * h_;
  std::vector<float4> a(np);
  HIP_OK(hipMemcpyAsync(a.data(), d_acc_, sizeof(float4) * np, hipMemcpyDeviceToHost, stream_));
  if (cnt) HIP_OK(hipMemcpyAsync(cnt, d_cnt_, sizeof(uint32_t) * np, hipMemcpyDeviceToHost, stream_));
  HIP_OK(hipStreamSynchronize(stream_));
  for (size_t i = 0; i < np; i++) {
    acc3[3 * i] = a[i].x;
    acc3[3 * i + 1] = a[i].y;
    acc3[3 * i + 2] = a[i].z;
  }
  return true;
}

bool Renderer::copy_partition(float* dev_dst, std::string& err) {
  const uint32_t n = (uint32_t)part_pix_.size();
  k_pack_partition<<<blocks_for(n), kBlock, 0, stream_>>>(nranks_ > 1 ? d_part_pix_ : nullptr, n, d_acc_, d_cnt_,
                                                          (float4*)dev_dst);
  HIP_OK(hipGetLastError());
  HIP_OK(hipStreamSynchronize(stream_));
  return true;
}

bool Renderer::launch_extend(const float4* ro, const float4* rd, const uint32_t* cnt, std::string& err) {
  const int v = (ds_.tri_only ? 1 : 0) | (counting_ ? 2 : 0) | (trav_ext_ << 2);
  const int full = batch_lanes_ == 1 ? kTravVariants : 0;
  const uint32_t g = std::min(async_grid(grid_ext_[v + full], 100), spill_grid());
  ds_.probe = probe_slot(1, g);
#define WPT_EXT(T, C, F) \
  k_extend<T, C, F><<<g, kTBlock, 0, ks_>>>(ds_, ro, rd, cnt, p_t_, p_id_, d_spill_, d_work_, d_fallback_)
  switch (v) {
    case 0: LAUNCH_TIMED(1, extend, n_extend, WPT_EXT(false, false, 0)); break;
    case 1: LAUNCH_TIMED(1, extend, n_extend, WPT_EXT(true, false, 0)); break;
    case 2: LAUNCH_TIMED(1, extend, n_extend, WPT_EXT(false, true, 0)); break;
    case 3: LAUNCH_TIMED(1, extend, n_extend, WPT_EXT(true, true, 0)); break;
    case 4: LAUNCH_TIMED(1, extend, n_extend, WPT_EXT(false, false, 1)); break;
    case 5: LAUNCH_TIMED(1, extend, n_extend, WPT_EXT(true, false, 1)); break;
    case 6: LAUNCH_TIMED(1, extend, n_extend, WPT_EXT(false, true, 1)); break;
    default: LAUNCH_TIMED(1, extend, n_extend, WPT_EXT(true, true, 1)); break;
  }
#undef WPT_EXT
  ds_.probe = nullptr;
  return true;
}

bool Renderer::launch_shadow(const uint32_t* cnt, uint8_t* occ_out, std::string& err) {
  const int v = (ds_.tri_only ? 1 : 0) | (counting_ ? 2 : 0) | (trav_sh_ << 2);
  const int full = batch_lanes_ == 1 ? kTravVariants : 0;
  const uint32_t g = std::min(async_grid(grid_sh_[v + full], 100), spill_grid());
  ds_.probe = probe_slot(3, g);
#define WPT_SH(T, C, F)                                                                                        \
  k_shadow<T, C, F><<<g, kTBlock, 0, ks_>>>(ds_, cnt, s_o_, s_d_, s_c_, p_col_, occ_out, d_spill_, d_work_, \
                                           d_fallback_)
  switch (v) {
    case 0: LAUNCH_TIMED(3, shadow, n_shadow, WPT_SH(false, false, 0)); break;
    case 1: LAUNCH_TIMED(3, shadow, n_shadow, WPT_SH(true, false, 0)); break;
    case 2: LAUNCH_TIMED(3, shadow, n_shadow, WPT_SH(false, true, 0)); break;
    case 3: LAUNCH_TIMED(3, shadow, n_shadow, WPT_SH(true, true, 0)); break;
    case 4: LAUNCH_TIMED(3, shadow, n_shadow, WPT_SH(false, false, 1)); break;
    case 5: LAUNCH_TIMED(3, shadow, n_shadow, WPT_SH(true, false, 1)); break;
    case 6: LAUNCH_TIMED(3, shadow, n_shadow, WPT_SH(false, true, 1)); break;
    default: LAUNCH_TIMED(3, shadow, n_shadow, WPT_SH(true, true, 1)); break;
  }
#undef WPT_SH
  ds_.probe = nullptr;
  return true;
}

bool Renderer::launch_trace(int b, std::string& err) {
  const int v = (ds_.tri_only ? 1 : 0) | (counting_ ? 2 : 0);
  const uint32_t g = std::min(async_grid(grid_tr_[v], trace_grid_pct_, 2), spill_grid());
  const float4* ro = p_ro_[b & 1];
  const float4* rd = p_rd_[b & 1];
  const uint32_t* ce = ext_count(b);
  const uint32_t* cs = sh_count(b - 1);
  ds_.probe = probe_slot(5, g);
#define WPT_TR(T, C) \
  k_trace<T, C><<<g, kTBlock, 0, ks_>>>(ds_, ro, rd, ce, p_t_, p_id_, cs, s_o_, s_d_, s_c_, p_col_, d_spill_, d_work_)
  switch (v) {
    case 0: LAUNCH_TIMED(5, trace, n_trace, WPT_TR(false, false)); break;
    case 1: LAUNCH_TIMED(5, trace, n_trace, WPT_TR(true, false)); break;
    case 2: LAUNCH_TIMED(5, trace, n_trace, WPT_TR(false, true)); break;
    default: LAUNCH_TIMED(5, trace, n_trace, WPT_TR(true, true)); break;
  }
#undef WPT_TR
  ds_.probe = nullptr;
  (void)err;
  return true;
}

uint4* Renderer::probe_slot(int kernel, uint32_t grid) {
  if (probe_used_ >= probe_cap_) return nullptr;
  const uint32_t waves = grid * (kTBlock / 64);
  if (!d_probe_) {
    probe_waves_ = max_grid() * (kTBlock / 64);
    const uint64_t cap_max = (1ull << 28) / std::max<uint32_t>(probe_waves_, 1);
    probe_cap_ = (uint32_t)std::min<uint64_t>(probe_cap_, cap_max);
    if (hipMalloc(&d_probe_, sizeof(uint4) * (size_t)probe_waves_ * probe_cap_) != hipSuccess) {
      d_probe_ = nullptr;
      probe_cap_ = 0;
      return nullptr;
    }
  }
  if (waves > probe_waves_) return nullptr;
  const uint32_t first = probe_used_ * probe_waves_;
  probe_meta_.insert(probe_meta_.end(), {(uint32_t)kernel, (uint32_t)bound_, (uint32_t)cur_bounce_, waves, first});
  probe_used_++;
  return d_probe_ + first;
}

bool Renderer::probe_read(std::vector<uint32_t>& meta, std::vector<uint4>& rec, double& ticks_per_us,
                          std::string& err) {
  HIP_OK(hipDeviceSynchronize());
  int khz = 0;
  HIP_OK(hipDeviceGetAttribute(&khz, hipDeviceAttributeWallClockRate, device_ < 0 ? 0 : device_));
  ticks_per_us = khz / 1000.0;
  meta = probe_meta_;
  rec.assign((size_t)probe_used_ * probe_waves_, make_uint4(0, 0, 0, 0));
  if (probe_used_) HIP_OK(hipMemcpy(rec.data(), d_probe_, sizeof(uint4) * rec.size(), hipMemcpyDeviceToHost));
  probe_used_ = 0;
  probe_meta_.clear();
  return true;
}

size_t Renderer::spill_slots() const {
  return (size_t)ds_.stack_cap > (size_t)kLdsSlots ? (size_t)ds_.stack_cap - kLdsSlots : 1;
}

uint32_t Renderer::spill_grid() const {
  return (uint32_t)std::min<size_t>(spill_cap_ / (spill_slots() * kTBlock), 0xFFFFFFFFu);
}

bool Renderer::ensure_spill(int l, uint32_t grid, std::string& err) {
  PathSet& L = lanes_[l];
  const size_t need = spill_slots() * (size_t)grid * kTBlock;
  if (need <= L.spill_cap) return true;
  HIP_OK(hipStreamSynchronize(L.stream));
  if (L.lo) HIP_OK(hipStreamSynchronize(L.lo));
// ... 467 lines not shown
          row[c] = walk((c & 4u) ? ax : it.kx, (c & 2u) ? ay : it.ky, (c & 1u) ? az : it.kz, it.d);
      }
    }
    HIP_OK(hipMalloc(&d_oct_corners_, sizeof(uint32_t) * corners.size()));
    HIP_OK(hipMemcpy(d_oct_corners_, corners.data(), sizeof(uint32_t) * corners.size(), hipMemcpyHostToDevice));
    ds_.oct_corners = d_oct_corners_;
  }
  {
    const size_t nodes = oct_child_.size(), all = nodes + oct_cum_.size();
    ds_.oct_lds_words = all <= kOctLdsWords ? (uint32_t)all : nodes <= kOctLdsWords ? (uint32_t)nodes : 0u;
  }
  photons_ok_ = true;
  return true;
}

bool Renderer::photon_tree(std::vector<uint32_t>& child, std::vector<float>& cum, uint64_t& shot, uint64_t& stored,
                           std::string& err) {
  if (!scene_ok_) { err = "no scene"; return false; }
  if (!build_photons(err)) return false;
  child = oct_child_;
  cum = oct_cum_;
  shot = photons_shot_;
  stored = photons_stored_;
  return true;
}

bool Renderer::trace_rays(size_t n, const float* rays, float* t_out, int32_t* id_out, std::string& err) {
  batch_lanes_ = 1;
  if (!scene_ok_) { err = "no scene"; return false; }
  if (n == 0) return true;
  if (n > 0xFFFFFFFFull) { err = "too many rays"; return false; }
  if (!ensure_paths(n, err)) return false;
  std::vector<float4> o(n), d(n);
  for (size_t i = 0; i < n; i++) {
    const float* r = rays + 6 * i;
    o[i] = make_float4(r[0], r[1], r[2], 0.0f);
    d[i] = make_float4(r[3], r[4], r[5], 0.0f);
  }
  const uint32_t nn = (uint32_t)n;
  HIP_OK(hipMemcpyAsync(p_ro_[0], o.data(), 16 * n, hipMemcpyHostToDevice, stream_));
  HIP_OK(hipMemcpyAsync(p_rd_[0], d.data(), 16 * n, hipMemcpyHostToDevice, stream_));
  HIP_OK(hipMemcpyAsync(d_counts_, &nn, 4, hipMemcpyHostToDevice, stream_));
  const bool prof = profiling_;
  profiling_ = false;
  const bool ok = launch_extend(p_ro_[0], p_rd_[0], d_counts_, err);
  profiling_ = prof;
  if (!ok) return false;
  HIP_OK(hipMemcpyAsync(t_out, p_t_, 4 * n, hipMemcpyDeviceToHost, stream_));
  HIP_OK(hipMemcpyAsync(id_out, p_id_, 4 * n, hipMemcpyDeviceToHost, stream_));
  HIP_OK(hipStreamSynchronize(stream_));
  return true;
}

bool Renderer::shadow_rays(size_t n, const float* pq, const int32_t* light, uint8_t* occ, std::string& err) {
  batch_lanes_ = 1;
  if (!scene_ok_) { err = "no scene"; return false; }
  if (n == 0) return true;
  if (n > 0xFFFFFFFFull) { err = "too many rays"; return false; }
  for (size_t i = 0; i < n; i++)
    if (light[i] < (int32_t)ds_.num_inf || light[i] >= (int32_t)ds_.num_shapes) { err = "light id out of range"; return false; }
  if (!ensure_paths(n, err)) return false;
  std::vector<float4> o(n), d(n);
  for (size_t i = 0; i < n; i++) {
    const float* r = pq + 6 * i;
    const V3 p = mk(r[0], r[1], r[2]), q = mk(r[3], r[4], r[5]);
    V3 dir = sub(q, p);
    const float dl = len(dir);
    dir = divs(dir, dl);
    const V3 org = add(p, scale(dir, kEpsilon));
    o[i] = make_float4(org.x, org.y, org.z, dl);
    d[i] = make_float4(dir.x, dir.y, dir.z, u2f((uint32_t)light[i]));
  }
  uint8_t* dq = nullptr;
  HIP_OK(hipMalloc(&dq, n));
  const uint32_t nn = (uint32_t)n;
  HIP_OK(hipMemcpyAsync(s_o_, o.data(), 16 * n, hipMemcpyHostToDevice, stream_));
  HIP_OK(hipMemcpyAsync(s_d_, d.data(), 16 * n, hipMemcpyHostToDevice, stream_));
  HIP_OK(hipMemcpyAsync(d_counts_, &nn, 4, hipMemcpyHostToDevice, stream_));
  const bool prof = profiling_;
  profiling_ = false;
  const bool ok = launch_shadow(d_counts_, dq, err);
  profiling_ = prof;
  if (ok) {
    HIP_OK(hipMemcpyAsync(occ, dq, n, hipMemcpyDeviceToHost, stream_));
    HIP_OK(hipStreamSynchronize(stream_));
  }
  (void)hipFree(dq);
  return ok;
}

}
```

wasm-pathtracer_amd/csrc/wpt_scene.cpp:

```cpp
#include "wpt_scene.h"

#include <algorithm>
#include <chrono>
#include <cmath>
#include <cstring>

namespace wpt {

namespace {

struct Box {
  float x0, y0, z0, x1, y1, z1;
};
inline Box join(const Box& a, const Box& o) {
  return Box{fminf(a.x0, o.x0), fminf(a.y0, o.y0), fminf(a.z0, o.z0),
             fmaxf(a.x1, o.x1), fmaxf(a.y1, o.y1), fmaxf(a.z1, o.z1)};
}
inline float surface(const Box& b) {
  float xs = b.x1 - b.x0, ys = b.y1 - b.y0, zs = b.z1 - b.z0;
  return 2.0f * (xs * ys + xs * zs + ys * zs);
}

bool shape_bounds(const Shape& s, Box* b, V3* loc) {
  switch (s.kind) {
// ... 254 lines not shown
    sc.nodes4.push_back(Node4{});
    const uint32_t l = sc.nodes[n].left_first, r = l + 1;
    const uint32_t i = pick_i(l, r, 4);
    std::vector<Entry> kids;
    cut(l, i, kids, level + 1);
    cut(r, 4 - i, kids, level + 1);
    fill(idx, kids);
    return idx;
  }
  void fill(uint32_t idx, const std::vector<Entry>& kids) {
    Node4& o = sc.nodes4[idx];
    for (int k = 0; k < 4; k++) {
      if (k < (int)kids.size()) {
        const float* b = kids[k].b;
        o.xmin[k] = b[0]; o.ymin[k] = b[1]; o.zmin[k] = b[2];
        o.xmax[k] = b[3]; o.ymax[k] = b[4]; o.zmax[k] = b[5];
        o.child[k] = kids[k].code;
      } else {
        o.xmin[k] = o.ymin[k] = o.zmin[k] = 0.0f;
        o.xmax[k] = o.ymax[k] = o.zmax[k] = 0.0f;
        o.child[k] = kChildEmpty;
      }
      o.pad[k] = 0;
    }
  }
  static void hull_of(const Node4& k, float* b) {
    b[0] = k.xmin[0]; b[1] = k.ymin[0]; b[2] = k.zmin[0];
    b[3] = k.xmax[0]; b[4] = k.ymax[0]; b[5] = k.zmax[0];
    for (int c = 1; c < 4 && k.child[c] != kChildEmpty; c++) {
      b[0] = fminf(b[0], k.xmin[c]); b[1] = fminf(b[1], k.ymin[c]); b[2] = fminf(b[2], k.zmin[c]);
      b[3] = fmaxf(b[3], k.xmax[c]); b[4] = fmaxf(b[4], k.ymax[c]); b[5] = fmaxf(b[5], k.zmax[c]);
    }
  }
};
}

void build_bvh4(HostScene& sc) {
  sc.nodes4.clear();
  sc.leaf_table.clear();
  sc.depth4 = 0;
  if (sc.shapes.size() <= sc.num_inf) return;
  Collapse4 c(sc);
  c.costs();
  if (!c.leaf(0) && c.pick_t(0, 4) == 1) {
    c.make_node(0, 0);
    return;
  }
  sc.nodes4.push_back(Node4{});
  std::vector<Collapse4::Entry> kids;
  c.cut(0, 4, kids, 1);
  c.fill(0, kids);
}

bool scene_init(HostScene& sc, std::vector<Shape> shapes, const float bg[3], Bvh2Builder* gpu, std::string* err) {
  sc.background[0] = bg[0]; sc.background[1] = bg[1]; sc.background[2] = bg[2];
  sc.use_bvh = true;
  sc.nodes.clear();
  Builder b(sc.nodes);
  std::vector<Shape> finite;
  finite.reserve(shapes.size());
  b.loc.reserve(shapes.size());
  b.box.reserve(shapes.size());
  uint32_t num_inf = 0;
  for (size_t i = 0; i < shapes.size(); i++) {
    Box bx;
    V3 lc;
    if (shape_bounds(shapes[i], &bx, &lc)) {
      b.loc.push_back(lc);
      b.box.push_back(bx);
      finite.push_back(shapes[i]);
    } else {
      std::swap(shapes[num_inf], shapes[i]);
      num_inf++;
    }
  }
  sc.num_inf = num_inf;
  sc.nodes.push_back(Node2{});
  sc.nodes.push_back(Node2{});
  sc.depth = 0;
  sc.shapes.reserve(shapes.size());
  sc.shapes.assign(shapes.begin(), shapes.begin() + num_inf);
  sc.bvh_on_gpu = false;
  sc.bvh_ms = 0.0;
  if (!finite.empty() && gpu && finite.size() >= gpu->min_shapes) {
    static_assert(sizeof(Box) == 6 * sizeof(float) && sizeof(V3) == 3 * sizeof(float), "packed boxes");
    std::string e;
    if (!gpu->build(&b.box[0].x0, &b.loc[0].x, finite.size(), sc.nodes, b.ord, sc.depth, sc.bvh_ms, e)) {
      if (err) *err = e;
      return false;
    }
    sc.bvh_on_gpu = true;
    for (uint32_t i : b.ord) sc.shapes.push_back(finite[i]);
  } else if (!finite.empty()) {
    const auto t0 = std::chrono::steady_clock::now();
    b.ord.resize(finite.size());
    for (size_t i = 0; i < finite.size(); i++) b.ord[i] = (uint32_t)i;
    for (auto& bn : b.bins) bn.reserve(finite.size());
    Box all;
    b.hull(b.ord.data(), b.ord.size(), &all);
    uint32_t maxd = 0;
    Node2 root = b.subdivide(0, finite.size(), all, 0, &maxd);
    sc.nodes[0] = root;
    sc.depth = maxd;
    sc.bvh_ms = std::chrono::duration<double, std::milli>(std::chrono::steady_clock::now() - t0).count();
    for (uint32_t i : b.ord) sc.shapes.push_back(finite[i]);
  }
  sc.tri_only = true;
  for (size_t i = num_inf; i < sc.shapes.size(); i++)
    if (sc.shapes[i].kind != kTri) sc.tri_only = false;
  sc.lights.clear();
  for (size_t i = 0; i < sc.shapes.size(); i++)
    if (sc.shapes[i].emissive) sc.lights.push_back((uint32_t)i);
  sc.nodes4.clear();
  sc.leaf_table.clear();
  sc.depth4 = 0;
  if (sc.want_bvh4 == 1 || (sc.want_bvh4 == 2 && !sc.tri_only && sc.use_bvh)) build_bvh4(sc);
  return true;
}

namespace {
V3 clamp_color(float r, float g, float b) { return mk(clamp01(r), clamp01(g), clamp01(b)); }

void museum_lights(std::vector<Shape>& s, float x, float y, V3 color) {
  V3 lc1 = mk(x - 1.0f, 0.0f, y + 2.8f), lc2 = mk(x + 1.0f, 0.0f, y + 2.8f);
  V3 lc3 = mk(x + 1.0f, 1.0f, y + 2.5f), lc4 = mk(x - 1.0f, 1.0f, y + 2.5f);
  s.push_back(make_triangle(lc3, lc2, lc1, true, color));
  s.push_back(make_triangle(lc4, lc3, lc1, true, color));
  lc1 = mk(x - 1.0f, 0.0f, y - 2.8f); lc2 = mk(x + 1.0f, 0.0f, y - 2.8f);
  lc3 = mk(x + 1.0f, 1.0f, y - 2.5f); lc4 = mk(x - 1.0f, 1.0f, y - 2.5f);
  s.push_back(make_triangle(lc3, lc2, lc1, true, color));
  s.push_back(make_triangle(lc4, lc3, lc1, true, color));
}

void push_bunny_light(std::vector<Shape>& s) {
  V3 lc1 = mk(-1.0f, 7.0f, 0.0f), lc2 = mk(1.0f, 7.0f, 0.0f), lc3 = mk(1.0f, 7.0f, 2.0f), lc4 = mk(-1.0f, 7.0f, 2.0f);
  s.push_back(make_triangle(lc3, lc2, lc1, true, mk(16.0f, 16.0f, 16.0f)));
  s.push_back(make_triangle(lc4, lc3, lc1, true, mk(16.0f, 16.0f, 16.0f)));
}
}

bool build_scene(int scene_id, const std::vector<float>& mesh, HostScene& sc, std::string& err, Bvh2Builder* gpu) {
  std::vector<Shape> s;
  const float black[3] = {0, 0, 0};
  if (scene_id == 2) {
    s.push_back(make_plane(mk(0.0f, -1.0f, 0.0f), mk(0.0f, 1.0f, 0.0f), false, clamp_color(1.0f, 1.0f, 1.0f)));
    s.push_back(make_plane(mk(0.0f, 0.0f, 13.0f), mk(0.0f, 0.0f, -1.0f), false, clamp_color(0.8f, 1.0f, 0.8f)));
    size_t nt = mesh.size() / 9;
    V3 mat = clamp_color(1.0f, 0.4f, 0.4f);
    for (size_t i = 0; i < nt; i++) {
      const float* a = mesh.data() + 9 * i;
      V3 tr = mk(0.0f, 0.0f, 5.0f);
      V3 p0 = add(scale(mk(a[0], a[1], a[2]), 0.5f), tr);
      V3 p1 = add(scale(mk(a[3], a[4], a[5]), 0.5f), tr);
      V3 p2 = add(scale(mk(a[6], a[7], a[8]), 0.5f), tr);
      s.push_back(make_triangle(p0, p1, p2, false, mat));
    }
    push_bunny_light(s);
    if (!scene_init(sc, std::move(s), black, gpu, &err)) return false;
    return true;
  }
  if (scene_id == 100) {
    V3 white = clamp_color(0.8f, 0.8f, 0.8f);
    s.push_back(make_plane(mk(0.0f, -1.0f, 0.0f), mk(0.0f, 1.0f, 0.0f), false, white));
    s.push_back(make_plane(mk(0.0f, 3.0f, 0.0f), mk(0.0f, -1.0f, 0.0f), false, white));
    s.push_back(make_plane(mk(0.0f, 0.0f, 4.0f), mk(0.0f, 0.0f, -1.0f), false, white));
    s.push_back(make_plane(mk(-2.0f, 0.0f, 0.0f), mk(1.0f, 0.0f, 0.0f), false, clamp_color(0.75f, 0.25f, 0.25f)));
    s.push_back(make_plane(mk(2.0f, 0.0f, 0.0f), mk(-1.0f, 0.0f, 0.0f), false, clamp_color(0.25f, 0.75f, 0.25f)));
    s.push_back(make_aarect(-1.2f, -0.2f, -1.0f, 0.8f, 1.8f, 2.8f, false, white));
    s.push_back(make_aarect(0.3f, 1.3f, -1.0f, -0.2f, 0.6f, 1.6f, false, white));
// ... 58 lines not shown
```

wasm-pathtracer_amd/csrc/wpt_scene.h:

```cpp
#pragma once
#include <stdint.h>
#include <string>
#include <vector>

#include "wpt_math.h"

namespace wpt {

enum ShapeKind : uint32_t { kTri = 0, kPlane = 1, kSphere = 2, kAARect = 3, kTorus = 4 };

struct Shape {
  uint32_t kind;
  float g[12];
  bool emissive;
  float m[3];
};

struct Node2 {
  float bmin[3];
  float bmax[3];
  uint32_t left_first;
  uint32_t count;
};
static_assert(sizeof(Node2) == 32, "BVHNode is 32 bytes");

struct Node4 {
  float xmin[4], xmax[4], ymin[4], ymax[4], zmin[4], zmax[4];
  uint32_t child[4];
  uint32_t pad[4];
};
static_assert(sizeof(Node4) == 128, "Node4 is 128 bytes");
constexpr uint32_t kChildEmpty = 0xFFFFFFFFu;

struct HostScene {
  std::vector<Shape> shapes;
  uint32_t num_inf = 0;
  std::vector<Node2> nodes;
  std::vector<uint32_t> lights;
  bool use_bvh = true;
  float background[3] = {0, 0, 0};
  uint32_t depth = 0;
  bool tri_only = true;
  std::vector<Node4> nodes4;
  std::vector<uint32_t> leaf_table;
  uint32_t depth4 = 0;
  int want_bvh4 = 1;
  bool bvh_on_gpu = false;
  double bvh_ms = 0.0;
};

struct Bvh2Builder {
  virtual ~Bvh2Builder() = default;
  virtual bool build(const float* box, const float* loc, size_t n, std::vector<Node2>& nodes,
                     std::vector<uint32_t>& ord, uint32_t& depth, double& ms, std::string& err) = 0;
  size_t min_shapes = 0;
};

void build_bvh4(HostScene& sc);

Shape make_triangle(V3 a, V3 b, V3 c, bool emissive, V3 m);
Shape make_plane(V3 loc, V3 normal, bool emissive, V3 m);
Shape make_sphere(V3 c, float r, bool emissive, V3 m);
Shape make_aarect(float x0, float x1, float y0, float y1, float z0, float z1, bool emissive, V3 m);
Shape make_torus(V3 loc, float big_r, float small_r, bool emissive, V3 m);

bool scene_init(HostScene& sc, std::vector<Shape> shapes, const float bg[3], Bvh2Builder* gpu = nullptr,
                std::string* err = nullptr);

bool build_scene(int scene_id, const std::vector<float>& mesh, HostScene& sc, std::string& err,
                 Bvh2Builder* gpu = nullptr);

}
```

wasm-pathtracer_amd/interface.py:

```python
import ctypes

import numpy as np

from ._lib import lib

OK = 0
ERR_NOT_INIT, ERR_ALREADY_INIT, ERR_INVALID_SCENE, ERR_INVALID_ARG = -1, -2, -3, -4
ERR_UNSUPPORTED, ERR_DEVICE, ERR_NO_MESH = -5, -6, -7
NO_NEE, NORMAL_NEE, PNEE = 0, 1, 2


class WptError(RuntimeError):
    def __init__(self, code, msg):
        super().__init__(f"[{code}] {msg}")
        self.code = code


def _check(rc):
    if rc < 0:
        raise WptError(rc, lib().wpt_last_error().decode())
    return rc


def init(width, height, scene_id, cam_x, cam_y, cam_z, cam_rot_x, cam_rot_y):
# ... 112 lines not shown
def photon_tree(num_lights):
    n = _check(lib().wpt_photon_tree(None, None, None))
    child = np.empty(n, dtype=np.uint32)
    cum = np.empty(n * max(num_lights, 1), dtype=np.float32)
    ss = np.empty(2, dtype=np.uint64)
    _check(lib().wpt_photon_tree(child.ctypes.data, cum.ctypes.data, ss.ctypes.data))
    return child, cum[: n * num_lights].reshape(n, num_lights), int(ss[0]), int(ss[1])


def read_radiance(width, height):
    acc = np.empty(width * height * 3, dtype=np.float32)
    cnt = np.empty(width * height, dtype=np.uint32)
    _check(lib().wpt_read_radiance(acc.ctypes.data, cnt.ctypes.data))
    return acc.reshape(height, width, 3), cnt.reshape(height, width)


def comm_unique_id():
    buf = ctypes.create_string_buffer(128)
    _check(lib().wpt_comm_unique_id(buf))
    return buf.raw


def set_comm(rank, nranks, tile, unique_id):
    uid = ctypes.create_string_buffer(bytes(unique_id), 128)
    _check(lib().wpt_set_comm(rank, nranks, tile, uid))


def gather_frame(root=0):
    _check(lib().wpt_gather_frame(root))


def gather_plan(rank, nranks, root, slot):
    n = _check(lib().wpt_gather_plan(rank, nranks, root, slot, None))
    out = np.zeros(4 * max(n, 1), dtype=np.uint64)
    _check(lib().wpt_gather_plan(rank, nranks, root, slot, out.ctypes.data))
    return [(int(a), int(b), int(c), bool(d)) for a, b, c, d in out[: 4 * n].reshape(-1, 4)]


def comm_destroy():
    _check(lib().wpt_comm_destroy())


def copy_partition(device_ptr):
    _check(lib().wpt_copy_partition(ctypes.c_void_p(device_ptr)))


def stats():
    keys = ("paths", "rays", "shadow_rays", "node_visits", "prim_tests", "bounces", "ext_visits", "ext_tests",
            "ext_node_bytes", "sh_visits", "sh_tests", "sh_node_bytes", "fallback_ext", "fallback_sh",
            "ext_lane_iters", "ext_live_iters", "sh_lane_iters", "sh_live_iters", "photon_rays", "photons",
            "sum_chunks", "sum_resummed", "sum_fetched", "stock_consumed", "fill_paths", "trace_bytes",
            "finish_paths", "finish_max_bounces", "max_ray_visits", "ex_body_lanes", "ex_bodies", "lf_body_lanes",
            "lf_bodies", "stock_traced", "stock_deficit", "stock_waits", "plan_us", "stock_us",
            "stock_rays", "stock_rays_used")
    out = (ctypes.c_uint64 * len(keys))()
    _check(lib().wpt_stats(ctypes.addressof(out), len(keys)))
    return dict(zip(keys, list(out)))


def kernel_times():
    out = (ctypes.c_double * 28)()
    _check(lib().wpt_kernel_times(ctypes.addressof(out), 28))
    names = ("generate", "extend", "shade", "shadow", "accumulate", "trace")
    kt = {n: {"ms": out[2 * i], "launches": int(out[2 * i + 1]), "busy_ms": out[12 + 2 * i],
              "logical_launches": int(out[13 + 2 * i])} for i, n in enumerate(names)}
    return kt


def set_counting(on):
    _check(lib().wpt_set_counting(1 if on else 0))


def set_profiling(on):
    _check(lib().wpt_set_profiling(1 if on else 0))


def scene_build_info():
    out = (ctypes.c_double * 2)()
    _check(lib().wpt_scene_build_info(ctypes.addressof(out)))
    return float(out[0]), bool(out[1])


def set_lanes(n):
    _check(lib().wpt_set_lanes(int(n)))


OPTIONS = {"defaults": 0, "traversal": 1, "traversal_sh": 2, "fused": 3, "fused_below": 4, "small_lanes": 5, "pixel_tile": 6,
           "grid_pct": 7, "refill": 8, "refill_sh": 9, "treelet": 10, "bvh_build": 11, "lanes": 12,
           "finish_below": 13, "trace_grid_pct": 14, "finish_every": 20, "probe": 22, "stock": 23, "stock_lanes": 24,
           "fill": 25, "async_prio": 26, "async_grid_pct": 27, "scene_traversal": 28, "scene_tri_only": 29,
           "stock_ahead": 30, "async_oneshot": 31, "stock_every": 32, "stock_extra": 33,
           "log": 34, "stock_prefill": 35, "async_fused_below": 36}
TRAVERSALS = {"bvh2": 0, "bvh4": 1, "auto": 3}
OPTION_VALUES = {"traversal": TRAVERSALS, "traversal_sh": TRAVERSALS,
                 "bvh_build": {"auto": 0, "host": 1, "gpu": 2}}


def set_option(name, value):
    if isinstance(value, str) and not value.lstrip("-").isdigit():
        value = OPTION_VALUES[name][value]
    _check(lib().wpt_set_option(OPTIONS[name], int(value)))


def get_option(name):
    v = ctypes.c_int64(0)
    _check(lib().wpt_get_option(OPTIONS[name], ctypes.addressof(v)))
    return v.value


def probe_read():
    L = lib()
    ent = ctypes.c_uint64(0)
    tpu = ctypes.c_double(0.0)
    n = L.wpt_probe_read(None, None, ctypes.addressof(ent), ctypes.addressof(tpu))
    if n < 0:
        raise WptError(int(n), L.wpt_last_error().decode())
    meta = np.zeros((n, 5), np.uint32)
    rec = np.zeros((ent.value, 4), np.uint32)
    if n:
        ent.value = rec.shape[0]
        _check(L.wpt_probe_read(meta.ctypes.data, rec.ctypes.data, ctypes.addressof(ent), ctypes.addressof(tpu)))
    return meta, rec, tpu.value


def clear_stats():
    _check(lib().wpt_clear_stats())


def sync():
    _check(lib().wpt_sync())


def bvh_depth():
    return _check(lib().wpt_bvh_depth())


def trace_rays(rays):
    r = np.ascontiguousarray(rays, dtype=np.float32).reshape(-1, 6)
    n = r.shape[0]
    t = np.empty(n, dtype=np.float32)
    ids = np.empty(n, dtype=np.int32)
    _check(lib().wpt_trace_rays(n, r.ctypes.data, t.ctypes.data, ids.ctypes.data))
    return t, ids


def shadow_rays(pq, light_ids):
    p = np.ascontiguousarray(pq, dtype=np.float32).reshape(-1, 6)
    li = np.ascontiguousarray(light_ids, dtype=np.int32)
    occ = np.empty(p.shape[0], dtype=np.uint8)
    _check(lib().wpt_shadow_rays(p.shape[0], p.ctypes.data, li.ctypes.data, occ.ctypes.data))
    return occ.astype(bool)


def shutdown():
    _check(lib().wpt_shutdown())


class DebugScene:

    def __init__(self, scene_id, mesh=None, gpu=False):
        L = lib()
        m = None if mesh is None else np.ascontiguousarray(mesh, dtype=np.float32)
        new = L.wpt_debug_scene_new_gpu if gpu else L.wpt_debug_scene_new
        self.h = new(scene_id, None if m is None else m.ctypes.data, 0 if m is None else m.size // 3)
        if not self.h:
            raise WptError(ERR_INVALID_SCENE, L.wpt_last_error().decode())
        bi = np.zeros(2, dtype=np.float64)
        _check(L.wpt_debug_scene_build_info(self.h, bi.ctypes.data))
        self.bvh_ms, self.bvh_on_gpu = float(bi[0]), bool(bi[1])
        info = np.zeros(8, dtype=np.uint64)
        L.wpt_debug_scene_info(self.h, info.ctypes.data)
        (self.num_shapes, self.num_inf, self.num_nodes, self.num_lights, self.depth, self.use_bvh,
         self.tri_only, self.num_nodes4) = (int(x) for x in info)

    def nodes(self):
        out = np.empty((self.num_nodes, 8), dtype=np.uint32)
        lib().wpt_debug_scene_nodes(self.h, out.ctypes.data)
        return out

    def nodes4(self):
        out = np.empty((self.num_nodes4, 37), dtype=np.uint32)
        if self.num_nodes4:
            lib().wpt_debug_scene_nodes4(self.h, out.ctypes.data)
        return out

    def shapes(self):
        out = np.empty((self.num_shapes, 16), dtype=np.float32)
        lib().wpt_debug_scene_shapes(self.h, out.ctypes.data)
        return out

    def lights(self):
        out = np.empty(self.num_lights, dtype=np.uint32)
        lib().wpt_debug_scene_lights(self.h, out.ctypes.data)
        return out

    def __del__(self):
        try:
            if getattr(self, "h", None):
                lib().wpt_debug_scene_free(self.h)
                self.h = None
        except Exception:
            pass
```

Measured before the change: 8462 Mray/s.

## Presolve primary rays against guard boxes and planes to skip BVH traversal

Adds a presolve pass run during primary-ray generation. Each camera ray is tested against the infinite planes and a few guard boxes, built on the host by splitting BVH leaves along gaps. Rays that provably miss all the finite geometry get their hit resolved directly and are compacted apart from the rays that still need full BVH traversal. This is meant to cut traversal work for primary rays that only see the floor or background, at the cost of extra per-ray slab tests, a second hit buffer and compaction bookkeeping.

New measurement: 9123 Mray/s (median of 6 runs). 7.8% higher.

```diff
diff --git a/include/wpt.h b/include/wpt.h
--- a/include/wpt.h
+++ b/include/wpt.h
@@ -121,6 +121,7 @@
 #define WPT_OPT_ASYNC_ONESHOT 31
 #define WPT_OPT_STOCK_PREFILL 35
 #define WPT_OPT_ASYNC_FUSED_BELOW 36
+#define WPT_OPT_PRESOLVE 37
 #define WPT_OPT_LOG 34
 #define WPT_OPT_SCENE_TRAVERSAL 28
 #define WPT_OPT_SCENE_TRI_ONLY 29
@@ -134,6 +135,7 @@
 
 int wpt_trace_rays(size_t n, const float* rays, float* t_out, int32_t* id_out);
 int wpt_shadow_rays(size_t n, const float* pq, const int32_t* light, uint8_t* occluded);
+int wpt_presolve_rays(size_t n, const float* rays, uint8_t* resolved, float* t_out, int32_t* id_out);
 
 int wpt_shutdown(void);
 
@@ -143,6 +145,8 @@
 int wpt_debug_scene_nodes(void* h, uint32_t* out);
 int wpt_debug_scene_shapes(void* h, float* out);
 int wpt_debug_scene_lights(void* h, uint32_t* out);
+int wpt_debug_scene_presolve(void* h, size_t n, const float* rays, uint8_t* resolved, float* t_out, int32_t* id_out);
+int wpt_debug_scene_guards(void* h, uint32_t* num_guards, float* boxes, uint32_t* leaf_guard);
 void wpt_debug_scene_free(void* h);
 void* wpt_debug_scene_new_gpu(int32_t scene_id, const float* mesh_vertices, size_t num_vertices);
 int wpt_debug_scene_build_info(void* h, double* out);
diff --git a/wasm-pathtracer_amd/_lib.py b/wasm-pathtracer_amd/_lib.py
--- a/wasm-pathtracer_amd/_lib.py
+++ b/wasm-pathtracer_amd/_lib.py
@@ -50,6 +50,9 @@
     "wpt_bvh_depth": (ctypes.c_int, []),
     "wpt_trace_rays": (ctypes.c_int, [c_sz, c_p, c_p, c_p]),
     "wpt_shadow_rays": (ctypes.c_int, [c_sz, c_p, c_p, c_p]),
+    "wpt_presolve_rays": (ctypes.c_int, [c_sz, c_p, c_p, c_p, c_p]),
+    "wpt_debug_scene_presolve": (ctypes.c_int, [c_p, c_sz, c_p, c_p, c_p, c_p]),
+    "wpt_debug_scene_guards": (ctypes.c_int, [c_p, c_p, c_p, c_p]),
     "wpt_shutdown": (ctypes.c_int, []),
     "wpt_debug_scene_new": (c_p, [c_i32, c_p, c_sz]),
     "wpt_debug_scene_info": (ctypes.c_int, [c_p, c_p]),
diff --git a/wasm-pathtracer_amd/csrc/wpt_api.cpp b/wasm-pathtracer_amd/csrc/wpt_api.cpp
--- a/wasm-pathtracer_amd/csrc/wpt_api.cpp
+++ b/wasm-pathtracer_amd/csrc/wpt_api.cpp
@@ -517,7 +517,7 @@
   std::string err;
   if (!g_session->renderer.flush_counts(err)) return fail(WPT_ERR_DEVICE, err);
   const Stats& st = g_session->renderer.stats();
-  uint64_t v[40] = {st.paths,          st.rays,           st.shadow_rays,    st.node_visits,  st.prim_tests,
+  uint64_t v[41] = {st.paths,          st.rays,           st.shadow_rays,    st.node_visits,  st.prim_tests,
                     st.bounces,        st.ext_visits,     st.ext_tests,      st.ext_node_bytes, st.sh_visits,
                     st.sh_tests,       st.sh_node_bytes,  st.fallback_ext,   st.fallback_sh,  st.ext_lane_iters,
                     st.ext_live_iters, st.sh_lane_iters,  st.sh_live_iters,  st.photon_rays,  st.photons,
@@ -525,8 +525,8 @@
                     st.trace_bytes,    st.finish_paths,   st.finish_max_bounces, st.max_ray_visits,
                     st.ex_body_lanes,  st.ex_bodies,      st.lf_body_lanes,  st.lf_bodies,    st.stock_traced,
                     st.stock_deficit,  st.stock_waits,    st.plan_us,        st.stock_us,
-                    st.stock_rays,     st.stock_rays_used};
-  for (size_t i = 0; i < n && i < 40; i++) out[i] = v[i];
+                    st.stock_rays,     st.stock_rays_used, st.presolved_rays};
+  for (size_t i = 0; i < n && i < 41; i++) out[i] = v[i];
   return WPT_OK;
 }
 
@@ -679,6 +679,14 @@
   if (!g_session) return fail(WPT_ERR_NOT_INIT, "init not called");
   std::string err;
   if (!g_session->renderer.trace_rays(n, rays, t_out, id_out, err)) return fail(WPT_ERR_DEVICE, err);
+  return WPT_OK;
+}
+
+int wpt_presolve_rays(size_t n, const float* rays, uint8_t* resolved, float* t_out, int32_t* id_out) {
+  if (!g_session) return fail(WPT_ERR_NOT_INIT, "init not called");
+  if (n && (!rays || !resolved || !t_out || !id_out)) return fail(WPT_ERR_INVALID_ARG, "null argument");
+  std::string err;
+  if (!g_session->renderer.presolve_rays(n, rays, resolved, t_out, id_out, err)) return fail(WPT_ERR_DEVICE, err);
   return WPT_OK;
 }
 
@@ -815,6 +823,41 @@
   return WPT_OK;
 }
 
+int wpt_debug_scene_presolve(void* h, size_t n, const float* rays, uint8_t* resolved, float* t_out, int32_t* id_out) {
+  const HostScene* sc = (const HostScene*)h;
+  if (!sc || (n && (!rays || !resolved || !t_out || !id_out))) return fail(WPT_ERR_INVALID_ARG, "null argument");
+  HostPlanes hp{};
+  hp.num_inf = 0;
+  PresolveBoxes pre{};
+  if (sc->use_bvh && sc->shapes.size() > sc->num_inf && sc->num_inf <= 16) {
+    pre = sc->pre;
+    hp.num_inf = sc->num_inf;
+    for (uint32_t i = 0; i < sc->num_inf; i++) {
+      const float* g = sc->shapes[i].g;
+      const V3 loc = mk(g[0], g[1], g[2]), nrm = mk(g[3], g[4], g[5]);
+      hp.planes[i] = HostPlanes::P4{nrm.x, nrm.y, nrm.z, dot(nrm, loc)};
+    }
+  }
+  for (size_t i = 0; i < n; i++) {
+    const float* r = rays + 6 * i;
+    resolved[i] = presolve_ray(hp, pre, mk(r[0], r[1], r[2]), mk(r[3], r[4], r[5]), t_out[i], id_out[i]) ? 1 : 0;
+  }
+  return WPT_OK;
+}
+
+int wpt_debug_scene_guards(void* h, uint32_t* num_guards, float* boxes, uint32_t* leaf_guard) {
+  const HostScene* sc = (const HostScene*)h;
+  if (!sc || !num_guards) return fail(WPT_ERR_INVALID_ARG, "null argument");
+  *num_guards = sc->pre.num_guards;
+  if (boxes) {
+    memcpy(boxes, sc->pre.root, 6 * sizeof(float));
+    memcpy(boxes + 6, sc->pre.guard, 6 * kMaxGuards * sizeof(float));
+  }
+  if (leaf_guard)
+    for (size_t i = 0; i < sc->nodes.size(); i++) leaf_guard[i] = i < sc->leaf_guard.size() ? sc->leaf_guard[i] : ~0u;
+  return WPT_OK;
+}
+
 void wpt_debug_scene_free(void* h) { delete (HostScene*)h; }
 
 }
diff --git a/wasm-pathtracer_amd/csrc/wpt_presolve.h b/wasm-pathtracer_amd/csrc/wpt_presolve.h
--- /dev/null
+++ b/wasm-pathtracer_amd/csrc/wpt_presolve.h
@@ -0,0 +1,86 @@
+#pragma once
+#include "wpt_math.h"
+
+namespace wpt {
+
+constexpr int kMaxGuards = 4;
+
+struct PresolveBoxes {
+  uint32_t num_guards;
+  float root[6];
+  float guard[kMaxGuards][6];
+};
+
+WPT_HD void presolve_slab(const float* b, V3 o, V3 inv, float& hh, float& tmax) {
+  const float tx1 = (b[0] - o.x) * inv.x;
+  const float tx2 = (b[3] - o.x) * inv.x;
+  const float ty1 = (b[1] - o.y) * inv.y;
+  const float ty2 = (b[4] - o.y) * inv.y;
+  const float tz1 = (b[2] - o.z) * inv.z;
+  const float tz2 = (b[5] - o.z) * inv.z;
+  const float tmin = fmaxf(fmaxf(fminf(tx1, tx2), fminf(ty1, ty2)), fminf(tz1, tz2));
+  tmax = fminf(fminf(fmaxf(tx1, tx2), fmaxf(ty1, ty2)), fmaxf(tz1, tz2));
+  hh = fmaxf(tmin, 0.0f);
+}
+
+WPT_HD float presolve_inf() {
+#if defined(__HIP_DEVICE_COMPILE__)
+  float v;
+  asm volatile("v_mov_b32 %0, 0x7f800000" : "=v"(v));
+  return v;
+#else
+  return u2f(0x7f800000u);
+#endif
+}
+
+template <class SC>
+WPT_HD bool presolve_ray(const SC& S, const PresolveBoxes& B, V3 o, V3 d, float& t, int32_t& id) {
+  t = 0.0f;
+  id = -1;
+  if (B.num_guards == 0u) return false;
+  if (d.x == 0.0f || d.y == 0.0f || d.z == 0.0f) return false;
+  const V3 inv = mk(1.0f / d.x, 1.0f / d.y, 1.0f / d.z);
+  const float inf = presolve_inf();
+  if (!(fabsf(inv.x) < inf) || !(fabsf(inv.y) < inf) || !(fabsf(inv.z) < inf)) return false;
+  float best = inf;
+  int32_t best_id = -1;
+  bool found = false;
+  for (uint32_t i = 0; i < S.num_inf; i++) {
+    const V3 n = mk(S.planes[i].x, S.planes[i].y, S.planes[i].z);
+    const float n_dot_dir = dot(n, d);
+    if (n_dot_dir == 0.0f) continue;
+    const float tt = (S.planes[i].w - dot(n, o)) / n_dot_dir;
+    if (tt <= 0.0f) continue;
+    if (!found || (0.0f < tt && tt < best)) {
+      found = true;
+      best = tt;
+      best_id = (int32_t)i;
+    }
+  }
+  float hh, tmax;
+  presolve_slab(B.root, o, inv, hh, tmax);
+  if ((hh <= tmax) & (hh < best)) {
+    bool clear = true;
+#if defined(__HIP_DEVICE_COMPILE__)
+#pragma unroll
+#endif
+    for (int g = 0; g < kMaxGuards; g++) {
+      if ((uint32_t)g < B.num_guards) {
+        presolve_slab(B.guard[g], o, inv, hh, tmax);
+        clear = clear && (!(hh <= tmax) || best < hh);
+      }
+    }
+    if (!clear) return false;
+  }
+  t = best_id >= 0 ? best : inf;
+  id = best_id;
+  return true;
+}
+
+struct HostPlanes {
+  struct P4 { float x, y, z, w; };
+  P4 planes[16];
+  uint32_t num_inf;
+};
+
+}
diff --git a/wasm-pathtracer_amd/csrc/wpt_render.h b/wasm-pathtracer_amd/csrc/wpt_render.h
--- a/wasm-pathtracer_amd/csrc/wpt_render.h
+++ b/wasm-pathtracer_amd/csrc/wpt_render.h
@@ -41,6 +41,7 @@
   float bg[3];
   float4 planes[kMaxInf];
   uint4* probe;
+  const PresolveBoxes* pre;
 };
 
 struct Stats {
@@ -64,6 +65,7 @@
   uint64_t stock_deficit = 0, stock_waits = 0, plan_us = 0, stock_us = 0;
   uint64_t stock_rays = 0;
   uint64_t stock_rays_used = 0;
+  uint64_t presolved_rays = 0;
 };
 
 constexpr int kTimedKernels = 7;
@@ -77,7 +79,9 @@
 constexpr int kMaxLanes = 8;
 constexpr uint64_t kMinLanePaths = 1024;
 constexpr size_t kFinishWord = 2 + 2 * (size_t)kMaxBounces;
-constexpr size_t kCountWords = kFinishWord + 4;
+constexpr size_t kResWord = kFinishWord + 4;
+constexpr size_t kCountWords = kResWord + 2 * ((size_t)kMaxBounces + 1);
+static_assert(kResWord % 2 == 0, "the presolved counts are 64-bit slots");
 constexpr uint32_t kWorkWords = 16;
 constexpr uint32_t kWorkCopies = 64;
 struct PathSet {
@@ -92,6 +96,8 @@
   float4* thr[2] = {nullptr, nullptr};
   float* t = nullptr;
   int32_t* id = nullptr;
+  float* t1 = nullptr;
+  int32_t* id1 = nullptr;
   float4 *so = nullptr, *sd = nullptr, *sc = nullptr;
   uint32_t* counts = nullptr;
   uint32_t* h_counts = nullptr;
@@ -116,6 +122,7 @@
   int lane0 = 0, nl = 1;
   uint64_t off[kMaxLanes + 1] = {};
   bool fused = false, pnee = false;
+  bool presolve = false;
   int maxb = 0, b = 0;
   bool finished = false;
   State state = kNew;
@@ -162,6 +169,7 @@
   uint32_t tile() const { return tile_; }
   bool unpack_ranks(const float4* gathered, uint64_t slot, std::string& err);
   bool trace_rays(size_t n, const float* rays, float* t_out, int32_t* id_out, std::string& err);
+  bool presolve_rays(size_t n, const float* rays, uint8_t* resolved, float* t_out, int32_t* id_out, std::string& err);
   bool shadow_rays(size_t n, const float* pq, const int32_t* light, uint8_t* occ, std::string& err);
   bool probe_read(std::vector<uint32_t>& meta, std::vector<uint4>& rec, double& ticks_per_us, std::string& err);
   void set_counting(bool on) { counting_ = on; }
@@ -306,6 +314,7 @@
   bool refill_issue(Refill& F, int h, uint64_t wt, std::string& err);
   bool stock_prefill(int h, uint64_t budget, std::string& err);
   bool stock_prefill_ = true;
+  bool pend_presolve_ = false;
   bool pend_stock_ = false;
   std::deque<Batch*> aq_[2];
   bool fill_on_ = false;
@@ -360,8 +369,8 @@
   uint32_t grid_sh_[2 * kTravVariants] = {};
   uint32_t grid_tr_[4] = {};
   uint32_t grid_shade_ = 512;
-  uint32_t shade_occ_[16] = {};
-  size_t shade_occ_smem_[16] = {};
+  uint32_t shade_occ_[32] = {};
+  size_t shade_occ_smem_[32] = {};
   bool fused_ = false;
   uint64_t fused_below_ = 1ull << 24;
   int small_lanes_ = 2;
@@ -377,6 +386,10 @@
   uint32_t refill_ = 12, refill_sh_ = 16;
   uint64_t finish_below_ = 1u << 18;
   int finish_every_ = 4;
+  uint32_t num_guards_ = 0;
+  bool presolve_ = true;
+  const uint32_t* probe_res_ = nullptr;
+  int hit_sel_ = 0;
   int batch_lanes_ = 1;
   uint32_t probe_cap_ = 0, probe_waves_ = 0, probe_used_ = 0;
   uint4* d_probe_ = nullptr;
@@ -426,6 +439,10 @@
   float4* p_thr_[2] = {nullptr, nullptr};
   float* p_t_ = nullptr;
   int32_t* p_id_ = nullptr;
+  float* p_t1_ = nullptr;
+  int32_t* p_id1_ = nullptr;
+  float* hit_t(int k) const { return k ? p_t1_ : p_t_; }
+  int32_t* hit_id(int k) const { return k ? p_id1_ : p_id_; }
   float4* s_o_ = nullptr;
   float4* s_d_ = nullptr;
   float4* s_c_ = nullptr;
@@ -436,6 +453,7 @@
   uint32_t* ext_count(int b) const { return b == 0 ? d_counts_ : d_counts_ + 2 + 2 * (b - 1); }
   uint32_t* sh_count(int b) const { return d_counts_ + 3 + 2 * b; }
   unsigned long long* append_ctr(int b) const { return reinterpret_cast<unsigned long long*>(d_counts_ + 2 + 2 * b); }
+  unsigned long long* res_ctr(int b) const { return reinterpret_cast<unsigned long long*>(d_counts_ + kResWord + 2 * b); }
 
   bool counting_ = false;
   bool profiling_ = false;
diff --git a/wasm-pathtracer_amd/csrc/wpt_render.hip b/wasm-pathtracer_amd/csrc/wpt_render.hip
--- a/wasm-pathtracer_amd/csrc/wpt_render.hip
+++ b/wasm-pathtracer_amd/csrc/wpt_render.hip
@@ -692,6 +692,42 @@
   uint32_t left_type, right_type;
 };
 
+struct GenPath {
+  uint32_t pl, sample, pixel, s, type;
+  V3 v;
+};
+__device__ __forceinline__ GenPath gen_path(const GenParams& P, const uint32_t* __restrict__ part_pix, uint64_t k,
+                                            const uint32_t* __restrict__ rnd_off,
+                                            const uint32_t* __restrict__ rnd_base,
+                                            const uint32_t* __restrict__ rnd_list) {
+  GenPath g;
+  if (rnd_off) {
+    uint32_t lo = 0, hi = P.npix;
+    while (lo + 1u < hi) {
+      const uint32_t mid = (lo + hi) >> 1;
+      if ((uint64_t)rnd_off[mid] <= k) lo = mid;
+      else hi = mid;
+    }
+    g.pl = lo;
+    g.sample = rnd_base[lo] + (uint32_t)(k - rnd_off[lo]);
+  } else {
+    g.pl = (uint32_t)(k % P.npix);
+    g.sample = (uint32_t)(k / P.npix);
+  }
+  g.pixel = rnd_list ? rnd_list[g.pl] : part_pix ? part_pix[g.pl] : g.pl;
+  const uint32_t x = g.pixel % P.W, y = g.pixel / P.W;
+  uint32_t s = path_seed(P.seed, g.pixel, g.sample);
+  const float fx = (((float)x + xs_next(s)) * P.w_inv - 0.5f) * P.ar;
+  const float fy = 0.5f - ((float)y + xs_next(s)) * P.h_inv;
+  V3 v = normalize(mk(fx, fy, 0.8f));
+  v = mk(v.x, P.cx * v.y - P.sx * v.z, P.sx * v.y + P.cx * v.z);
+  v = mk(P.cy * v.x + P.sy * v.z, v.y, (-P.sy) * v.x + P.cy * v.z);
+  g.s = s;
+  g.v = v;
+  g.type = x < P.half ? P.left_type : P.right_type;
+  return g;
+}
+
 __global__ void __launch_bounds__(kBlock) k_generate(GenParams P, const uint32_t* __restrict__ part_pix, uint64_t k0,
                                                      uint32_t n, uint32_t* __restrict__ pix_out,
                                                      float4* __restrict__ thr,
@@ -703,35 +739,73 @@
   const uint32_t i = blockIdx.x * kBlock + threadIdx.x;
   if (i == 0) *count0 = n;
   if (i >= n) return;
-  const uint64_t k = k0 + i;
-  uint32_t pl, sample;
-  if (rnd_off) {
-    uint32_t lo = 0, hi = P.npix;
-    while (lo + 1u < hi) {
-      const uint32_t mid = (lo + hi) >> 1;
-      if ((uint64_t)rnd_off[mid] <= k) lo = mid;
-      else hi = mid;
-    }
-    pl = lo;
-    sample = rnd_base[lo] + (uint32_t)(k - rnd_off[lo]);
+  const GenPath g = gen_path(P, part_pix, k0 + i, rnd_off, rnd_base, rnd_list);
+  pix_out[i] = stock_slots ? g.pixel * stock_slots + (g.sample & (stock_slots - 1u)) : rnd_off ? g.pl : g.pixel;
+  thr[i] = make_float4(1.0f, 1.0f, 1.0f, __uint_as_float(g.type << kTypeShift));
+  col[i] = make_float4(0.0f, 0.0f, 0.0f, 0.0f);
+  ro[i] = make_float4(P.cam[0], P.cam[1], P.cam[2], __uint_as_float(g.s));
+  rd[i] = make_float4(g.v.x, g.v.y, g.v.z, __uint_as_float(i));
+}
+
+__global__ void __launch_bounds__(kBlock) k_generate_ps(GenParams P, const uint32_t* __restrict__ part_pix, uint64_t k0,
+                                                        uint32_t n, uint32_t* __restrict__ pix_out,
+                                                        float4* __restrict__ thr,
+                                                        float4* __restrict__ col, float4* __restrict__ ro,
+                                                        float4* __restrict__ rd, uint32_t* __restrict__ count0,
+                                                        const uint32_t* __restrict__ rnd_off,
+                                                        const uint32_t* __restrict__ rnd_base,
+                                                        const uint32_t* __restrict__ rnd_list, uint32_t stock_slots,
+                                                        DevScene S, float* __restrict__ t_out,
+                                                        int32_t* __restrict__ id_out, uint32_t* __restrict__ res0) {
+  const uint32_t i = blockIdx.x * kBlock + threadIdx.x;
+  constexpr uint32_t kWaves = kBlock / 64;
+  __shared__ uint32_t s_off[2][kWaves];
+  const bool valid = i < n;
+  const GenPath g = gen_path(P, part_pix, k0 + (valid ? i : 0u), rnd_off, rnd_base, rnd_list);
+  float pt;
+  int32_t pid;
+  const bool res = valid && presolve_ray(S, *S.pre, mk(P.cam[0], P.cam[1], P.cam[2]), g.v, pt, pid);
+  const uint32_t lane = threadIdx.x & 63u, wid = threadIdx.x >> 6;
+  const uint64_t below = (1ull << lane) - 1ull;
+  const uint64_t hm = __ballot(valid && !res), rm = __ballot(res);
+  if (lane == 0) {
+    s_off[0][wid] = (uint32_t)__popcll(hm);
+    s_off[1][wid] = (uint32_t)__popcll(rm);
+  }
+  __syncthreads();
+  if (wid == 0) {
+    const uint32_t a = lane < kWaves ? s_off[0][lane] : 0u, b = lane < kWaves ? s_off[1][lane] : 0u;
+    uint32_t ia = a, ib = b;
+#pragma unroll
+    for (uint32_t q = 1; q < kWaves; q <<= 1) {
+      const uint32_t ya = __shfl_up(ia, q, 64), yb = __shfl_up(ib, q, 64);
+      if (lane >= q) { ia += ya; ib += yb; }
+    }
+    const uint32_t tb = (uint32_t)__shfl((int)ib, (int)(kWaves - 1), 64);
+    uint32_t base = 0u;
+    if (lane == kWaves - 1 || lane == kWaves) base = atomicAdd(lane == kWaves - 1 ? count0 : res0, lane == kWaves - 1 ? ia : tb);
+    const uint32_t ba = (uint32_t)__shfl((int)base, (int)(kWaves - 1), 64);
+    const uint32_t bb = (uint32_t)__shfl((int)base, (int)kWaves, 64);
+    if (lane < kWaves) {
+      s_off[0][lane] = ba + ia - a;
+      s_off[1][lane] = bb + ib - b;
+    }
+  }
+  __syncthreads();
+  if (!valid) return;
+  uint32_t p;
+  if (res) {
+    p = n - 1u - (s_off[1][wid] + (uint32_t)__popcll(rm & below));
+    t_out[p] = pt;
+    id_out[p] = pid;
   } else {
-    pl = (uint32_t)(k % P.npix);
-    sample = (uint32_t)(k / P.npix);
-  }
-  const uint32_t pixel = rnd_list ? rnd_list[pl] : part_pix ? part_pix[pl] : pl;
-  const uint32_t x = pixel % P.W, y = pixel / P.W;
-  uint32_t s = path_seed(P.seed, pixel, sample);
-  const float fx = (((float)x + xs_next(s)) * P.w_inv - 0.5f) * P.ar;
-  const float fy = 0.5f - ((float)y + xs_next(s)) * P.h_inv;
-  V3 v = normalize(mk(fx, fy, 0.8f));
-  v = mk(v.x, P.cx * v.y - P.sx * v.z, P.sx * v.y + P.cx * v.z);
-  v = mk(P.cy * v.x + P.sy * v.z, v.y, (-P.sy) * v.x + P.cy * v.z);
-  const uint32_t type = x < P.half ? P.left_type : P.right_type;
-  pix_out[i] = stock_slots ? pixel * stock_slots + (sample & (stock_slots - 1u)) : rnd_off ? pl : pixel;
-  thr[i] = make_float4(1.0f, 1.0f, 1.0f, __uint_as_float(type << kTypeShift));
+    p = s_off[0][wid] + (uint32_t)__popcll(hm & below);
+  }
+  pix_out[i] = stock_slots ? g.pixel * stock_slots + (g.sample & (stock_slots - 1u)) : rnd_off ? g.pl : g.pixel;
   col[i] = make_float4(0.0f, 0.0f, 0.0f, 0.0f);
-  ro[i] = make_float4(P.cam[0], P.cam[1], P.cam[2], __uint_as_float(s));
-  rd[i] = make_float4(v.x, v.y, v.z, __uint_as_float(i));
+  thr[p] = make_float4(1.0f, 1.0f, 1.0f, __uint_as_float(g.type << kTypeShift));
+  ro[p] = make_float4(P.cam[0], P.cam[1], P.cam[2], __uint_as_float(g.s));
+  rd[p] = make_float4(g.v.x, g.v.y, g.v.z, __uint_as_float(i));
 }
 
 template <bool TRI_ONLY>
@@ -1064,16 +1138,20 @@
   if (!R.alive) end_counts((flags >> kShadowShift) + (R.shadow ? 1u : 0u));
 }
 
-template <bool TRI_ONLY, bool PNEE, int OCT, bool CR = false>
+template <bool TRI_ONLY, bool PNEE, int OCT, bool CR = false, bool PS = false>
 __global__ void WPT_SHADE_BOUNDS k_shade(DevScene S, ShadeParams P, RayStream in, RayStream out,
                                                        ShadowStream sh, float4* __restrict__ col,
                                                        const uint32_t* __restrict__ count, const float* __restrict__ t_in,
                                                        const int32_t* __restrict__ id_in,
-                                                       unsigned long long* __restrict__ append) {
+                                                       unsigned long long* __restrict__ append,
+                                                       float* __restrict__ t_nx, int32_t* __restrict__ id_nx,
+                                                       uint32_t end) {
   constexpr uint32_t kWaves = kShadeBlock / 64;
-  __shared__ uint32_t s_off[2][kWaves];
+  static_assert(kWaves < 64, "the scan's totals and the second atomic lane sit in one wave");
+  __shared__ uint32_t s_off[PS ? 3 : 2][kWaves];
   __shared__ f4v s_light[5 * kShadeLights];
-  const uint32_t n = *count;
+  const uint32_t nh = *count;
+  const uint32_t n = PS ? nh + reinterpret_cast<const uint32_t*>(append)[kResWord - 2] : nh;
   const bool lds_lights = S.num_lights <= kShadeLights;
   if (lds_lights) {
     for (uint32_t k = threadIdx.x; k < 5 * S.num_lights; k += kShadeBlock) {
@@ -1106,38 +1184,83 @@
     const uint32_t i = i0 + threadIdx.x;
     ShadeOut R;
     R.alive = R.shadow = false;
-    if (i < n)
-      shade_path<TRI_ONLY, PNEE, OV, CR>(S, O, P, col, t_in[i], id_in[i], in.o[i], in.d[i], in.thr[i], R,
+    if (i < n) {
+      const uint32_t q = !PS || i < nh ? i : end - 1u - (i - nh);
+      shade_path<TRI_ONLY, PNEE, OV, CR>(S, O, P, col, t_in[q], id_in[q], in.o[q], in.d[q], in.thr[q], R,
                                      lds_lights ? (const lds_f4v*)s_light : nullptr);
-    const uint64_t am = __ballot(R.alive), sm = __ballot(R.shadow);
+    }
+    bool res = false;
+    float pt = 0.0f;
+    int32_t pid = -1;
+    if constexpr (PS) {
+      if (R.alive) res = presolve_ray(S, *S.pre, ld3(R.ro), ld3(R.rd), pt, pid);
+    }
+    const uint64_t am = __ballot(R.alive && !res), sm = __ballot(R.shadow), rm = PS ? __ballot(res) : 0ull;
     if (lane == 0) {
       s_off[0][wid] = (uint32_t)__popcll(am);
       s_off[1][wid] = (uint32_t)__popcll(sm);
+      if constexpr (PS) s_off[2][wid] = (uint32_t)__popcll(rm);
     }
     __syncthreads();
-    if (wid == 0) {
+    if constexpr (!PS) {
+      if (wid == 0) {
+        const uint32_t a = lane < kWaves ? s_off[0][lane] : 0u, b = lane < kWaves ? s_off[1][lane] : 0u;
+        uint32_t ia = a, ib = b;
+#pragma unroll
+        for (uint32_t k = 1; k < kWaves; k <<= 1) {
+          const uint32_t ya = __shfl_up(ia, k, 64), yb = __shfl_up(ib, k, 64);
+          if (lane >= k) { ia += ya; ib += yb; }
+        }
+        unsigned long long base = 0ull;
+        if (lane == kWaves - 1) base = atomicAdd(append, (unsigned long long)ia | ((unsigned long long)ib << 32));
+        const uint32_t ba = (uint32_t)__shfl((int)(uint32_t)base, (int)(kWaves - 1), 64);
+        const uint32_t bb = (uint32_t)__shfl((int)(uint32_t)(base >> 32), (int)(kWaves - 1), 64);
+        if (lane < kWaves) {
+          s_off[0][lane] = ba + ia - a;
+          s_off[1][lane] = bb + ib - b;
+        }
+      }
+    } else if (wid == 0) {
       const uint32_t a = lane < kWaves ? s_off[0][lane] : 0u, b = lane < kWaves ? s_off[1][lane] : 0u;
-      uint32_t ia = a, ib = b;
+      const uint32_t c = lane < kWaves ? s_off[2][lane] : 0u;
+      uint32_t ia = a, ib = b, ic = c;
 #pragma unroll
       for (uint32_t k = 1; k < kWaves; k <<= 1) {
-        const uint32_t ya = __shfl_up(ia, k, 64), yb = __shfl_up(ib, k, 64);
-        if (lane >= k) { ia += ya; ib += yb; }
+        const uint32_t ya = __shfl_up(ia, k, 64), yb = __shfl_up(ib, k, 64), yc = __shfl_up(ic, k, 64);
+        if (lane >= k) { ia += ya; ib += yb; ic += yc; }
       }
+      const uint32_t tc = (uint32_t)__shfl((int)ic, (int)(kWaves - 1), 64);
       unsigned long long base = 0ull;
-      if (lane == kWaves - 1) base = atomicAdd(append, (unsigned long long)ia | ((unsigned long long)ib << 32));
+      uint32_t off;
+      asm volatile("v_mov_b32 %0, %1" : "=v"(off) : "i"((uint32_t)(kResWord / 2)));
+      if (lane == kWaves - 1 || lane == kWaves)
+        base = atomicAdd(append + (lane == kWaves - 1 ? 0u : off),
+                         lane == kWaves - 1 ? ((unsigned long long)ia | ((unsigned long long)ib << 32))
+                                            : (unsigned long long)tc);
       const uint32_t ba = (uint32_t)__shfl((int)(uint32_t)base, (int)(kWaves - 1), 64);
       const uint32_t bb = (uint32_t)__shfl((int)(uint32_t)(base >> 32), (int)(kWaves - 1), 64);
+      const uint32_t bc = (uint32_t)__shfl((int)(uint32_t)base, (int)kWaves, 64);
       if (lane < kWaves) {
         s_off[0][lane] = ba + ia - a;
         s_off[1][lane] = bb + ib - b;
+        s_off[2][lane] = bc + ic - c;
       }
     }
     __syncthreads();
     if (R.alive) {
-      const uint32_t p = s_off[0][wid] + (uint32_t)__popcll(am & below);
+      uint32_t p = s_off[0][wid] + (uint32_t)__popcll(am & below);
+      if constexpr (PS) {
+        if (res) p = end - 1u - (s_off[2][wid] + (uint32_t)__popcll(rm & below));
+      }
       st_stream(out.o + p, R.ro);
       st_stream(out.d + p, R.rd);
       st_stream(out.thr + p, R.th);
+      if constexpr (PS) {
+        if (res) {
+          t_nx[p] = pt;
+          id_nx[p] = pid;
+        }
+      }
     }
     if (R.shadow) {
       const uint32_t p = s_off[1][wid] + (uint32_t)__popcll(sm & below);
@@ -1601,6 +1724,22 @@
   }
 }
 
+__global__ void k_probe_add(uint4* rec, const uint32_t* __restrict__ res) { rec[0].w += *res; }
+
+__global__ void __launch_bounds__(kBlock) k_presolve(DevScene S, uint32_t n, const float* __restrict__ rays,
+                                                     uint8_t* __restrict__ resolved, float* __restrict__ t_out,
+                                                     int32_t* __restrict__ id_out) {
+  const uint32_t i = blockIdx.x * kBlock + threadIdx.x;
+  if (i >= n) return;
+  const float* r = rays + 6 * (size_t)i;
+  float t;
+  int32_t id;
+  const bool res = presolve_ray(S, *S.pre, mk(r[0], r[1], r[2]), mk(r[3], r[4], r[5]), t, id);
+  resolved[i] = res ? 1 : 0;
+  t_out[i] = t;
+  id_out[i] = id;
+}
+
 __global__ void __launch_bounds__(kBlock) k_accumulate(const uint32_t* __restrict__ part_pix, uint64_t k0, uint32_t n,
                                                        uint32_t npix, const float4* __restrict__ col,
                                                        float4* __restrict__ acc, uint32_t* __restrict__ cnt) {
@@ -1820,14 +1959,15 @@
 }
 
 void Renderer::free_lane_paths(PathSet& L) {
-  void* bufs[] = {L.pixel, L.col, L.ro[0], L.rd[0], L.thr[0], L.ro[1], L.rd[1], L.thr[1], L.t, L.id, L.so, L.sd, L.sc};
+  void* bufs[] = {L.pixel, L.col, L.ro[0], L.rd[0], L.thr[0], L.ro[1], L.rd[1], L.thr[1], L.t, L.id, L.t1, L.id1,
+                  L.so, L.sd, L.sc};
   for (void* p : bufs)
     if (p) (void)hipFree(p);
   L.pixel = nullptr;
   L.col = nullptr;
   for (int k = 0; k < 2; k++) L.ro[k] = L.rd[k] = L.thr[k] = nullptr;
-  L.t = nullptr;
-  L.id = nullptr;
+  L.t = L.t1 = nullptr;
+  L.id = L.id1 = nullptr;
   L.so = L.sd = L.sc = nullptr;
   L.cap = 0;
 }
@@ -1851,6 +1991,7 @@
     p_thr_[k] = L.thr[k];
   }
   p_t_ = L.t; p_id_ = L.id;
+  p_t1_ = L.t1; p_id1_ = L.id1;
   s_o_ = L.so; s_d_ = L.sd; s_c_ = L.sc;
   d_counts_ = L.counts; h_counts_ = L.h_counts;
   d_spill_ = L.spill; spill_cap_ = L.spill_cap;
@@ -2019,6 +2160,13 @@
   ds.refill_lanes_sh = refill_sh_;
   for (int k = 0; k < 3; k++) ds.bg[k] = sc.background[k];
   for (uint32_t i = 0; i < sc.num_inf && i < (uint32_t)kMaxInf; i++) ds.planes[i] = all[4 * i];
+  {
+    PresolveBoxes pre{};
+    if (sc.use_bvh && nf != 0) pre = sc.pre;
+    if (!up(&pre, sizeof pre, &p)) return false;
+    ds.pre = (const PresolveBoxes*)p;
+    num_guards_ = pre.num_guards;
+  }
   ds_ = ds;
   depth_ = sc.depth;
   ds_.stack_cap = (int)std::max<uint32_t>(sc.depth + 2, 3 * sc.depth4 + 4);
@@ -2076,6 +2224,7 @@
     case 34: if (!range(0, 1)) return false; log_ = (int)v; return true;
     case 35: if (!range(0, 1)) return false; stock_prefill_ = v != 0; return true;
     case 36: if (!range(0, (int64_t)1 << 40)) return false; async_fused_below_ = (uint64_t)v; return true;
+    case 37: if (!range(0, 1)) return false; presolve_ = v != 0; return true;
     case 26:
       if (!range(0, 1)) return false;
       if (!drain_async(err)) return false;
@@ -2127,6 +2276,7 @@
     case 34: v = log_; return true;
     case 35: v = stock_prefill_ ? 1 : 0; return true;
     case 36: v = (int64_t)async_fused_below_; return true;
+    case 37: v = presolve_ ? 1 : 0; return true;
     case 26: v = async_prio_; return true;
     case 27: v = async_grid_pct_; return true;
     case 28: v = !scene_ok_ ? -1 : !ds_.use_bvh ? 2 : trav_ext_; return true;
@@ -2355,12 +2505,14 @@
   return async ? std::min(nlanes_, kAsyncLane0) : nlanes_;
 }
 
-static void add_counts(Stats& st, const uint32_t* hc, int b, bool stock) {
+static void add_counts(Stats& st, const uint32_t* hc, int b, bool stock, bool presolve) {
   uint64_t& r = stock ? st.stock_rays : st.rays;
   uint64_t& sr = stock ? st.stock_rays : st.shadow_rays;
   for (int i = 0; i < b; i++) {
-    r += i == 0 ? hc[0] : hc[2 + 2 * (i - 1)];
+    const uint32_t res = presolve ? hc[kResWord + 2 * i] : 0u;
+    r += (i == 0 ? hc[0] : hc[2 + 2 * (i - 1)]) + res;
     sr += hc[3 + 2 * i];
+    st.presolved_rays += res;
   }
   r += hc[kFinishWord];
   sr += hc[kFinishWord + 1];
@@ -2372,13 +2524,13 @@
   if (!stats_pending_) return true;
   for (int l = 0; l < pend_nl_; l++)
     if (!host_wait(lanes_[l].done, err)) return false;
-  for (int l = 0; l < pend_nl_; l++) add_counts(stats_, lanes_[l].h_counts, pend_b_, pend_stock_);
+  for (int l = 0; l < pend_nl_; l++) add_counts(stats_, lanes_[l].h_counts, pend_b_, pend_stock_, pend_presolve_);
   stats_pending_ = false;
   return true;
 }
 
 void Renderer::batch_counts(const Batch& B, const uint32_t* hc) {
-  for (int i = 0; i < B.nl; i++) add_counts(stats_, hc + (size_t)i * kCountWords, B.b, B.stock);
+  for (int i = 0; i < B.nl; i++) add_counts(stats_, hc + (size_t)i * kCountWords, B.b, B.stock, B.presolve);
   stats_.bounces += (uint64_t)B.b;
 }
 
@@ -2401,21 +2553,32 @@
   G.left_type = (uint32_t)left_type_; G.right_type = (uint32_t)right_type_;
   const uint32_t slots = B.stock ? stock_used_slots_ : 0u;
   for (int i = 0; i <= B.nl; i++) B.off[i] = B.n * (uint64_t)i / (uint64_t)B.nl;
+  B.presolve = presolve_ && max_depth_ > 0 && num_guards_ != 0;
   if (time_launches_) HIP_OK(hipEventRecord(ev_ref_, stream_));
   HIP_OK(hipEventRecord(ev_main_, stream_));
   batch_lanes_ = B.nl;
   for (int i = 0; i < B.nl; i++) {
     const int l = B.lane0 + i;
+    if (B.presolve && !lanes_[l].t1 && lanes_[l].cap) {
+      HIP_OK(hipMalloc(&lanes_[l].t1, 4 * lanes_[l].cap));
+      HIP_OK(hipMalloc(&lanes_[l].id1, 4 * lanes_[l].cap));
+    }
     bind_batch_lane(B, l);
     if (B.off[i + 1] - B.off[i] > cap_) { bind_lane(0); err = "batch exceeds lane capacity"; return false; }
     if (l != 0) HIP_OK(hipStreamWaitEvent(ks_, ev_main_, 0));
     if (ks_ != lanes_[l].stream) HIP_OK(hipStreamWaitEvent(ks_, lanes_[l].done, 0));
     const uint32_t nn = (uint32_t)(B.off[i + 1] - B.off[i]);
-    HIP_OK(hipMemsetAsync(d_counts_, 0, sizeof(uint32_t) * kCountWords, ks_));
-    LAUNCH_TIMED(0, generate, n_generate,
-                 k_generate<<<blocks_for(nn), kBlock, 0, ks_>>>(G, part, B.k0 + B.off[i], nn, p_pixel_, p_thr_[0],
-                                                              p_col_, p_ro_[0], p_rd_[0], d_counts_, rnd_off, rnd_base,
-                                                              B.mlist, slots));
+    HIP_OK(hipMemsetAsync(d_counts_, 0, sizeof(uint32_t) * (B.presolve ? kCountWords : kResWord), ks_));
+    if (B.presolve)
+      LAUNCH_TIMED(0, generate, n_generate,
+                   k_generate_ps<<<blocks_for(nn), kBlock, 0, ks_>>>(
+                       G, part, B.k0 + B.off[i], nn, p_pixel_, p_thr_[0], p_col_, p_ro_[0], p_rd_[0], d_counts_, rnd_off,
+                       rnd_base, B.mlist, slots, ds_, p_t_, p_id_, reinterpret_cast<uint32_t*>(res_ctr(0))));
+    else
+      LAUNCH_TIMED(0, generate, n_generate,
+                   k_generate<<<blocks_for(nn), kBlock, 0, ks_>>>(G, part, B.k0 + B.off[i], nn, p_pixel_, p_thr_[0],
+                                                                p_col_, p_ro_[0], p_rd_[0], d_counts_, rnd_off, rnd_base,
+                                                                B.mlist, slots));
   }
   B.maxb = max_depth_ > 0 ? std::min(max_depth_, kMaxBounces) : kMaxBounces;
   B.fused = (fused_ || B.n < (B.async && async_fused_below_ ? async_fused_below_ : fused_below_)) && trav_ext_ != 1 &&
@@ -2501,12 +2664,14 @@
     for (int i = 0; i < B.nl; i++) {
       bind_batch_lane(B, B.lane0 + i);
       const uint32_t nn = (uint32_t)(B.off[i + 1] - B.off[i]);
-      if (B.fused && b > 0) {
-        if (!launch_trace(b, err)) { bind_lane(0); return false; }
-      } else if (!launch_extend(p_ro_[b & 1], p_rd_[b & 1], ext_count(b), err)) {
-        bind_lane(0);
-        return false;
-      }
+      const int hs = B.presolve ? (b & 1) : 0;
+      hit_sel_ = hs;
+      probe_res_ = B.presolve ? reinterpret_cast<const uint32_t*>(res_ctr(b)) : nullptr;
+      const bool traced = (B.fused && b > 0) ? launch_trace(b, err)
+                                             : launch_extend(p_ro_[b & 1], p_rd_[b & 1], ext_count(b), err);
+      hit_sel_ = 0;
+      probe_res_ = nullptr;
+      if (!traced) { bind_lane(0); return false; }
       {
         const RayStream in{p_ro_[b & 1], p_rd_[b & 1], p_thr_[b & 1]};
         const RayStream out{p_ro_[(b + 1) & 1], p_rd_[(b + 1) & 1], p_thr_[(b + 1) & 1]};
@@ -2514,33 +2679,37 @@
         [[maybe_unused]] const uint32_t sgrid =
             std::max<uint32_t>(1, std::min<uint32_t>((nn + kShadeBlock - 1) / kShadeBlock, grid_shade_));
 #if WPT_SHADE_GRID_VAR
-#define WPT_SHADE_GRID(T, PN, OC, CR)                                                                           \
-  const int vi = (CR ? 8 : 0) + (T ? 4 : 0) + (PN ? 1 + OC : 0);                                                \
+#define WPT_SHADE_GRID(T, PN, OC, CR, PS)                                                                       \
+  const int vi = (PS ? 16 : 0) + (CR ? 8 : 0) + (T ? 4 : 0) + (PN ? 1 + OC : 0);                                \
   const size_t smem = OC ? 4 * (size_t)ds_.oct_lds_words : 0;                                                   \
   if (shade_occ_[vi] == 0 || shade_occ_smem_[vi] != smem) {                                                     \
     int bpc = 0;                                                                                                \
-    HIP_OK(hipOccupancyMaxActiveBlocksPerMultiprocessor(&bpc, k_shade<T, PN, OC, CR>, (int)kShadeBlock, smem));  \
+    HIP_OK(hipOccupancyMaxActiveBlocksPerMultiprocessor(&bpc, k_shade<T, PN, OC, CR, PS>, (int)kShadeBlock, smem)); \
     shade_occ_[vi] = (uint32_t)std::max(bpc, 1);                                                                \
     shade_occ_smem_[vi] = smem;                                                                                 \
   }                                                                                                             \
   const uint32_t sg = std::max<uint32_t>(1, std::min<uint32_t>((nn + kShadeBlock - 1) / kShadeBlock,            \
                                                                (uint32_t)ncu_ * shade_occ_[vi]));
 #else
-#define WPT_SHADE_GRID(T, PN, OC, CR) const uint32_t sg = sgrid;
+#define WPT_SHADE_GRID(T, PN, OC, CR, PS) const uint32_t sg = sgrid;
 #endif
-#define WPT_SHADE1(T, PN, OC, CR)                                                                                   \
+#define WPT_SHADE1(T, PN, OC, CR, PS)                                                                               \
   do {                                                                                                              \
-    WPT_SHADE_GRID(T, PN, OC, CR)                                                                                   \
+    WPT_SHADE_GRID(T, PN, OC, CR, PS)                                                                               \
     const uint32_t sgo = async_launch_ && async_oneshot_ ? std::max<uint32_t>(1, (nn + kShadeBlock - 1) / kShadeBlock) \
                                                          : sg;                                                      \
     LAUNCH_TIMED(2, shade, n_shade,                                                                                 \
-                 k_shade<T, PN, OC, CR><<<sgo, kShadeBlock, OC ? 4 * ds_.oct_lds_words : 0, ks_>>>(                 \
-                     ds_, SP, in, out, sh, p_col_, ext_count(b), p_t_, p_id_, append_ctr(b)));                      \
+                 k_shade<T, PN, OC, CR, PS><<<sgo, kShadeBlock, OC ? 4 * ds_.oct_lds_words : 0, ks_>>>(             \
+                     ds_, SP, in, out, sh, p_col_, ext_count(b), hit_t(hs), hit_id(hs), append_ctr(b),             \
+                     hit_t(hs ^ 1), hit_id(hs ^ 1), nn));                                                           \
   } while (0)
 #define WPT_SHADE(T, PN, OC)              \
   do {                                    \
-    if (B.stock) WPT_SHADE1(T, PN, OC, true); \
-    else WPT_SHADE1(T, PN, OC, false);    \
+    if (B.presolve) {                                \
+      if (B.stock) WPT_SHADE1(T, PN, OC, true, true);    \
+      else WPT_SHADE1(T, PN, OC, false, true);           \
+    } else if (B.stock) WPT_SHADE1(T, PN, OC, true, false); \
+    else WPT_SHADE1(T, PN, OC, false, false);            \
   } while (0)
         const int oc = !B.pnee || ds_.oct_lds_words == 0 ? 0 : (ds_.oct_lds_words > ds_.oct_nodes ? 2 : 1);
         if (ds_.tri_only) {
@@ -2607,7 +2776,8 @@
                        part, B.k0 + B.off[i], nn, npix, p_col_, d_acc_, d_cnt_));
     HIP_OK(hipGetLastError());
     uint32_t* hc = B.async ? B.hc + (size_t)i * kCountWords : h_counts_;
-    HIP_OK(hipMemcpyAsync(hc, d_counts_, sizeof(uint32_t) * kCountWords, hipMemcpyDeviceToHost, ks_));
+    HIP_OK(hipMemcpyAsync(hc, d_counts_, sizeof(uint32_t) * (B.presolve ? kCountWords : kResWord),
+                          hipMemcpyDeviceToHost, ks_));
     HIP_OK(hipEventRecord(B.async ? B.done[i] : lanes_[l].done, ks_));
   }
   bind_lane(0);
@@ -2616,6 +2786,7 @@
     pend_nl_ = B.nl;
     pend_b_ = B.b;
     pend_stock_ = B.stock;
+    pend_presolve_ = B.presolve;
     stats_pending_ = true;
   }
   B.state = Batch::kIssued;
@@ -3292,7 +3463,8 @@
   const uint32_t g = std::min(async_grid(grid_ext_[v + full], 100), spill_grid());
   ds_.probe = probe_slot(1, g);
 #define WPT_EXT(T, C, F) \
-  k_extend<T, C, F><<<g, kTBlock, 0, ks_>>>(ds_, ro, rd, cnt, p_t_, p_id_, d_spill_, d_work_, d_fallback_)
+  k_extend<T, C, F><<<g, kTBlock, 0, ks_>>>(ds_, ro, rd, cnt, hit_t(hit_sel_), hit_id(hit_sel_), d_spill_, d_work_, \
+                                            d_fallback_)
   switch (v) {
     case 0: LAUNCH_TIMED(1, extend, n_extend, WPT_EXT(false, false, 0)); break;
     case 1: LAUNCH_TIMED(1, extend, n_extend, WPT_EXT(true, false, 0)); break;
@@ -3304,6 +3476,10 @@
     default: LAUNCH_TIMED(1, extend, n_extend, WPT_EXT(true, true, 1)); break;
   }
 #undef WPT_EXT
+  if (ds_.probe && probe_res_) {
+    k_probe_add<<<1, 1, 0, ks_>>>(ds_.probe, probe_res_);
+    HIP_OK(hipGetLastError());
+  }
   ds_.probe = nullptr;
   return true;
 }
@@ -3340,7 +3516,8 @@
   const uint32_t* cs = sh_count(b - 1);
   ds_.probe = probe_slot(5, g);
 #define WPT_TR(T, C) \
-  k_trace<T, C><<<g, kTBlock, 0, ks_>>>(ds_, ro, rd, ce, p_t_, p_id_, cs, s_o_, s_d_, s_c_, p_col_, d_spill_, d_work_)
+  k_trace<T, C><<<g, kTBlock, 0, ks_>>>(ds_, ro, rd, ce, hit_t(hit_sel_), hit_id(hit_sel_), cs, s_o_, s_d_, s_c_, \
+                                        p_col_, d_spill_, d_work_)
   switch (v) {
     case 0: LAUNCH_TIMED(5, trace, n_trace, WPT_TR(false, false)); break;
     case 1: LAUNCH_TIMED(5, trace, n_trace, WPT_TR(true, false)); break;
@@ -3348,6 +3525,10 @@
     default: LAUNCH_TIMED(5, trace, n_trace, WPT_TR(true, true)); break;
   }
 #undef WPT_TR
+  if (ds_.probe && probe_res_) {
+    k_probe_add<<<1, 1, 0, ks_>>>(ds_.probe, probe_res_);
+    if (hipGetLastError() != hipSuccess) { err = "k_probe_add launch failed"; ds_.probe = nullptr; return false; }
+  }
   ds_.probe = nullptr;
   (void)err;
   return true;
@@ -3921,6 +4102,34 @@
   return true;
 }
 
+bool Renderer::presolve_rays(size_t n, const float* rays, uint8_t* resolved, float* t_out, int32_t* id_out,
+                             std::string& err) {
+  if (!scene_ok_) { err = "no scene"; return false; }
+  if (n == 0) return true;
+  if (n > 0xFFFFFFFFull / 8) { err = "too many rays"; return false; }
+  float* dr = nullptr;
+  float* dt = nullptr;
+  int32_t* di = nullptr;
+  uint8_t* df = nullptr;
+  bool ok = hipMalloc(&dr, 24 * n) == hipSuccess && hipMalloc(&dt, 4 * n) == hipSuccess &&
+            hipMalloc(&di, 4 * n) == hipSuccess && hipMalloc(&df, n) == hipSuccess;
+  if (ok) ok = hipMemcpyAsync(dr, rays, 24 * n, hipMemcpyHostToDevice, stream_) == hipSuccess;
+  if (ok) {
+    k_presolve<<<blocks_for((uint32_t)n), kBlock, 0, stream_>>>(ds_, (uint32_t)n, dr, df, dt, di);
+    ok = hipGetLastError() == hipSuccess &&
+         hipMemcpyAsync(resolved, df, n, hipMemcpyDeviceToHost, stream_) == hipSuccess &&
+         hipMemcpyAsync(t_out, dt, 4 * n, hipMemcpyDeviceToHost, stream_) == hipSuccess &&
+         hipMemcpyAsync(id_out, di, 4 * n, hipMemcpyDeviceToHost, stream_) == hipSuccess &&
+         hipStreamSynchronize(stream_) == hipSuccess;
+  }
+  (void)hipFree(dr);
+  (void)hipFree(dt);
+  (void)hipFree(di);
+  (void)hipFree(df);
+  if (!ok) err = "HIP error in presolve_rays";
+  return ok;
+}
+
 bool Renderer::shadow_rays(size_t n, const float* pq, const int32_t* light, uint8_t* occ, std::string& err) {
   batch_lanes_ = 1;
   if (!scene_ok_) { err = "no scene"; return false; }
diff --git a/wasm-pathtracer_amd/csrc/wpt_scene.cpp b/wasm-pathtracer_amd/csrc/wpt_scene.cpp
--- a/wasm-pathtracer_amd/csrc/wpt_scene.cpp
+++ b/wasm-pathtracer_amd/csrc/wpt_scene.cpp
@@ -330,6 +330,76 @@
   c.fill(0, kids);
 }
 
+void build_guards(HostScene& sc) {
+  sc.pre = PresolveBoxes{};
+  sc.leaf_guard.assign(sc.nodes.size(), ~0u);
+  if (sc.shapes.size() <= sc.num_inf || sc.nodes.empty()) return;
+  std::vector<uint32_t> leaves;
+  {
+    std::vector<uint32_t> todo{0u};
+    while (!todo.empty()) {
+      const uint32_t n = todo.back();
+      todo.pop_back();
+      if (sc.nodes[n].count != 0) { leaves.push_back(n); continue; }
+      todo.push_back(sc.nodes[n].left_first);
+      todo.push_back(sc.nodes[n].left_first + 1);
+    }
+  }
+  struct Group {
+    std::vector<uint32_t> leaves;
+    float b[6];
+    bool whole = false;
+  };
+  auto bounds = [&](Group& g) {
+    for (int k = 0; k < 3; k++) { g.b[k] = INFINITY; g.b[3 + k] = -INFINITY; }
+    for (uint32_t n : g.leaves)
+      for (int k = 0; k < 3; k++) {
+        g.b[k] = fminf(g.b[k], sc.nodes[n].bmin[k]);
+        g.b[3 + k] = fmaxf(g.b[3 + k], sc.nodes[n].bmax[k]);
+      }
+  };
+  auto area = [](const Group& g) {
+    const double x = (double)g.b[3] - g.b[0], y = (double)g.b[4] - g.b[1], z = (double)g.b[5] - g.b[2];
+    return x * y + y * z + z * x;
+  };
+  std::vector<Group> groups(1);
+  groups[0].leaves = leaves;
+  bounds(groups[0]);
+  while (groups.size() < (size_t)kMaxGuards) {
+    int pick = -1;
+    for (size_t i = 0; i < groups.size(); i++)
+      if (!groups[i].whole && groups[i].leaves.size() > 1 && (pick < 0 || area(groups[i]) > area(groups[pick])))
+        pick = (int)i;
+    if (pick < 0) break;
+    Group& g = groups[pick];
+    float best_gap = 0.0f, cut = 0.0f;
+    int axis = -1;
+    for (int k = 0; k < 3; k++) {
+      std::vector<uint32_t> ord = g.leaves;
+      std::sort(ord.begin(), ord.end(), [&](uint32_t a, uint32_t b) { return sc.nodes[a].bmin[k] < sc.nodes[b].bmin[k]; });
+      float hi = sc.nodes[ord[0]].bmax[k];
+      for (size_t i = 1; i < ord.size(); i++) {
+        const float lo = sc.nodes[ord[i]].bmin[k];
+        if (lo > hi && lo - hi > best_gap) { best_gap = lo - hi; cut = lo; axis = k; }
+        hi = fmaxf(hi, sc.nodes[ord[i]].bmax[k]);
+      }
+    }
+    if (axis < 0) { g.whole = true; continue; }
+    Group a, b;
+    for (uint32_t n : g.leaves) (sc.nodes[n].bmin[axis] < cut ? a : b).leaves.push_back(n);
+    bounds(a);
+    bounds(b);
+    groups[pick] = std::move(a);
+    groups.push_back(std::move(b));
+  }
+  sc.pre.num_guards = (uint32_t)groups.size();
+  for (int k = 0; k < 3; k++) { sc.pre.root[k] = sc.nodes[0].bmin[k]; sc.pre.root[3 + k] = sc.nodes[0].bmax[k]; }
+  for (size_t i = 0; i < groups.size(); i++) {
+    for (int k = 0; k < 6; k++) sc.pre.guard[i][k] = groups[i].b[k];
+    for (uint32_t n : groups[i].leaves) sc.leaf_guard[n] = (uint32_t)i;
+  }
+}
+
 bool scene_init(HostScene& sc, std::vector<Shape> shapes, const float bg[3], Bvh2Builder* gpu, std::string* err) {
   sc.background[0] = bg[0]; sc.background[1] = bg[1]; sc.background[2] = bg[2];
   sc.use_bvh = true;
@@ -393,6 +463,7 @@
   sc.leaf_table.clear();
   sc.depth4 = 0;
   if (sc.want_bvh4 == 1 || (sc.want_bvh4 == 2 && !sc.tri_only && sc.use_bvh)) build_bvh4(sc);
+  build_guards(sc);
   return true;
 }
 
diff --git a/wasm-pathtracer_amd/csrc/wpt_scene.h b/wasm-pathtracer_amd/csrc/wpt_scene.h
--- a/wasm-pathtracer_amd/csrc/wpt_scene.h
+++ b/wasm-pathtracer_amd/csrc/wpt_scene.h
@@ -4,6 +4,7 @@
 #include <vector>
 
 #include "wpt_math.h"
+#include "wpt_presolve.h"
 
 namespace wpt {
 
@@ -47,6 +48,8 @@
   int want_bvh4 = 1;
   bool bvh_on_gpu = false;
   double bvh_ms = 0.0;
+  PresolveBoxes pre{};
+  std::vector<uint32_t> leaf_guard;
 };
 
 struct Bvh2Builder {
@@ -57,6 +60,8 @@
 };
 
 void build_bvh4(HostScene& sc);
+
+void build_guards(HostScene& sc);
 
 Shape make_triangle(V3 a, V3 b, V3 c, bool emissive, V3 m);
 Shape make_plane(V3 loc, V3 normal, bool emissive, V3 m);
diff --git a/wasm-pathtracer_amd/interface.py b/wasm-pathtracer_amd/interface.py
--- a/wasm-pathtracer_amd/interface.py
+++ b/wasm-pathtracer_amd/interface.py
@@ -188,7 +188,7 @@
             "sum_chunks", "sum_resummed", "sum_fetched", "stock_consumed", "fill_paths", "trace_bytes",
             "finish_paths", "finish_max_bounces", "max_ray_visits", "ex_body_lanes", "ex_bodies", "lf_body_lanes",
             "lf_bodies", "stock_traced", "stock_deficit", "stock_waits", "plan_us", "stock_us",
-            "stock_rays", "stock_rays_used")
+            "stock_rays", "stock_rays_used", "presolved_rays")
     out = (ctypes.c_uint64 * len(keys))()
     _check(lib().wpt_stats(ctypes.addressof(out), len(keys)))
     return dict(zip(keys, list(out)))
@@ -226,7 +226,7 @@
            "finish_below": 13, "trace_grid_pct": 14, "finish_every": 20, "probe": 22, "stock": 23, "stock_lanes": 24,
            "fill": 25, "async_prio": 26, "async_grid_pct": 27, "scene_traversal": 28, "scene_tri_only": 29,
            "stock_ahead": 30, "async_oneshot": 31, "stock_every": 32, "stock_extra": 33,
-           "log": 34, "stock_prefill": 35, "async_fused_below": 36}
+           "log": 34, "stock_prefill": 35, "async_fused_below": 36, "presolve": 37}
 TRAVERSALS = {"bvh2": 0, "bvh4": 1, "auto": 3}
 OPTION_VALUES = {"traversal": TRAVERSALS, "traversal_sh": TRAVERSALS,
                  "bvh_build": {"auto": 0, "host": 1, "gpu": 2}}
@@ -286,6 +286,16 @@
     occ = np.empty(p.shape[0], dtype=np.uint8)
     _check(lib().wpt_shadow_rays(p.shape[0], p.ctypes.data, li.ctypes.data, occ.ctypes.data))
     return occ.astype(bool)
+
+
+def presolve_rays(rays):
+    r = np.ascontiguousarray(rays, dtype=np.float32).reshape(-1, 6)
+    n = r.shape[0]
+    res = np.zeros(n, dtype=np.uint8)
+    t = np.empty(n, dtype=np.float32)
+    ids = np.empty(n, dtype=np.int32)
+    _check(lib().wpt_presolve_rays(n, r.ctypes.data, res.ctypes.data, t.ctypes.data, ids.ctypes.data))
+    return res.astype(bool), t, ids
 
 
 def shutdown():
@@ -330,6 +340,23 @@
         lib().wpt_debug_scene_lights(self.h, out.ctypes.data)
         return out
 
+    def presolve(self, rays):
+        r = np.ascontiguousarray(rays, dtype=np.float32).reshape(-1, 6)
+        n = r.shape[0]
+        res = np.zeros(n, dtype=np.uint8)
+        t = np.empty(n, dtype=np.float32)
+        ids = np.empty(n, dtype=np.int32)
+        _check(lib().wpt_debug_scene_presolve(self.h, n, r.ctypes.data, res.ctypes.data, t.ctypes.data,
+                                              ids.ctypes.data))
+        return res.astype(bool), t, ids
+
+    def guards(self):
+        ng = ctypes.c_uint32(0)
+        boxes = np.zeros(30, dtype=np.float32)
+        lg = np.zeros(max(self.num_nodes, 1), dtype=np.uint32)
+        _check(lib().wpt_debug_scene_guards(self.h, ctypes.addressof(ng), boxes.ctypes.data, lg.ctypes.data))
+        return boxes[:6].copy(), boxes[6:].reshape(4, 6)[: ng.value].copy(), lg[: self.num_nodes]
+
     def __del__(self):
         try:
             if getattr(self, "h", None):
```
